# catie-aq/flashT5

Hardware: AMD Instinct MI355X
Metric: FA2+T5-bias fwd+bwd TFLOP/s (bf16, d_head=64) (higher is better)
Workload: dtype bf16; 1 GPU; encoder self-attn fwd+bwd, (B,H,S,d)=(4,12,512,64) per GPU, non-causal, 32-bucket T5 RPE bias (rpe mode), sm_scale 0.125, (B,S,H,D)-strided inputs; global_batch=4, seq_len=512, parallelism=dp1, bias_mode=rpe, launch=hipGraph replay, 16 step(s) per replay

## Files before the change

### flasht5_amd/_lib.py

```python
import ctypes
import os

import torch

_HERE = os.path.dirname(os.path.abspath(__file__))
_VAR = os.environ.get("FAT5_LIB_VARIANT", "")
LIB_PATH = os.path.join(_HERE, "lib", "libfat5" + ("_" + _VAR if _VAR else "") + ".so")

FAT5_F32, FAT5_F16, FAT5_BF16 = 0, 1, 2
FAT5_FORCED_BOS, FAT5_FORCED_EOS = 1, 2
BIAS_NONE, BIAS_DENSE, BIAS_RPE1D = 0, 1, 2
KV_NATIVE, KV_FP8_E4M3 = 0, 1
MAX_RPE_RADIUS = 1024

_DT = {torch.float32: FAT5_F32, torch.float16: FAT5_F16, torch.bfloat16: FAT5_BF16}

c_i64x3 = ctypes.c_int64 * 3


class AttnParams(ctypes.Structure):
    _fields_ = [
        ("B", ctypes.c_int32), ("H", ctypes.c_int32), ("M", ctypes.c_int32), ("N", ctypes.c_int32),
        ("D", ctypes.c_int32), ("dtype", ctypes.c_int32), ("causal", ctypes.c_int32),
        ("bias_mode", ctypes.c_int32), ("sm_scale", ctypes.c_float), ("rpe_radius", ctypes.c_int32),
# ... 82 lines not shown
    _fields_ = [
        ("B", ctypes.c_int32), ("L", ctypes.c_int32), ("H", ctypes.c_int32), ("D", ctypes.c_int32), ("dtype", ctypes.c_int32),
        ("x", ctypes.c_void_p), ("out", ctypes.c_void_p), ("scale", ctypes.c_void_p),
        ("x_stride", c_i64x3), ("out_stride", c_i64x3), ("scale_stride", c_i64x3),
    ]


class SampleParams(ctypes.Structure):
    _fields_ = [
        ("B", ctypes.c_int32), ("V", ctypes.c_int32), ("dtype", ctypes.c_int32), ("top_k", ctypes.c_int32),
        ("logits", ctypes.c_void_p), ("row_stride", ctypes.c_int64), ("temperature", ctypes.c_float), ("top_p", ctypes.c_float),
        ("seed", ctypes.c_uint64), ("offset", ctypes.c_int64), ("offsets", ctypes.c_void_p), ("uniforms", ctypes.c_void_p),
        ("tokens", ctypes.c_void_p), ("aux", ctypes.c_void_p),
    ]


class BeamParams(ctypes.Structure):
    _fields_ = [
        ("B", ctypes.c_int32), ("k", ctypes.c_int32), ("V", ctypes.c_int32), ("dtype", ctypes.c_int32),
        ("logits", ctypes.c_void_p), ("row_stride", ctypes.c_int64), ("running_scores", ctypes.c_void_p),
        ("running_seqs", ctypes.c_void_p), ("cache_row_batch", ctypes.c_void_p), ("finished_seqs", ctypes.c_void_p),
        ("finished_scores", ctypes.c_void_p), ("finished_flags", ctypes.c_void_p), ("finished_lens", ctypes.c_void_p),
        ("heuristic", ctypes.c_void_p), ("status", ctypes.c_void_p), ("tokens", ctypes.c_void_p), ("step", ctypes.c_void_p),
        ("seq_len", ctypes.c_int32), ("capacity", ctypes.c_int32), ("max_length", ctypes.c_int32), ("early_stopping", ctypes.c_int32),
        ("length_penalty", ctypes.c_float), ("workspace", ctypes.c_void_p), ("workspace_bytes", ctypes.c_size_t),
        ("logits_normalized", ctypes.c_int32),
    ]


class LogitsParams(ctypes.Structure):
    _fields_ = [
        ("rows", ctypes.c_int32), ("V", ctypes.c_int32), ("dtype", ctypes.c_int32), ("log_softmax", ctypes.c_int32),
        ("logits", ctypes.c_void_p), ("row_stride", ctypes.c_int64), ("out", ctypes.c_void_p), ("out_stride", ctypes.c_int64),
        ("sequences", ctypes.c_void_p), ("seq_stride", ctypes.c_int64), ("lengths", ctypes.c_void_p), ("seq_len", ctypes.c_int32),
        ("repetition_penalty", ctypes.c_float), ("no_repeat_ngram_size", ctypes.c_int32), ("min_length", ctypes.c_int32),
        ("eos_token_id", ctypes.c_int32), ("n_suppress", ctypes.c_int32), ("suppress_tokens", ctypes.c_void_p),
        ("encoder_repetition_penalty", ctypes.c_double), ("encoder_input_ids", ctypes.c_void_p), ("encoder_stride", ctypes.c_int64),
        ("encoder_lengths", ctypes.c_void_p), ("encoder_rows", ctypes.c_int32), ("encoder_len", ctypes.c_int32),
        ("rows_per_encoder_row", ctypes.c_int32), ("encoder_no_repeat_ngram_size", ctypes.c_int32),
        ("bad_words_ids", ctypes.c_void_p), ("bad_words_offsets", ctypes.c_void_p), ("bad_words_offsets_host", ctypes.c_void_p),
        ("n_bad_words", ctypes.c_int32), ("n_bad_word_ids", ctypes.c_int32), ("min_new_tokens", ctypes.c_int32),
        ("prompt_length", ctypes.c_int32), ("prompt_lengths", ctypes.c_void_p), ("max_new_tokens", ctypes.c_int32),
        ("forced_tokens", ctypes.c_int32), ("forced_bos_token_id", ctypes.c_int32), ("forced_eos_token_id", ctypes.c_int32),
    ]


class SpecParams(ctypes.Structure):
    _fields_ = [
        ("B", ctypes.c_int32), ("M", ctypes.c_int32), ("V", ctypes.c_int32), ("dtype", ctypes.c_int32),
        ("logits", ctypes.c_void_p), ("batch_stride", ctypes.c_int64), ("row_stride", ctypes.c_int64),
        ("draft", ctypes.c_void_p), ("draft_stride", ctypes.c_int64), ("cache_seqlens", ctypes.c_void_p),
        ("draft_seqlens", ctypes.c_void_p), ("labels", ctypes.c_void_p), ("labels_stride", ctypes.c_int64),
        ("ncols", ctypes.c_int32), ("eos_token_id", ctypes.c_int32), ("tok", ctypes.c_void_p), ("seen_eos", ctypes.c_void_p),
        ("limit", ctypes.c_void_p), ("limit_scalar", ctypes.c_int32), ("n_accepted", ctypes.c_void_p), ("n_new", ctypes.c_void_p),
        ("workspace", ctypes.c_void_p), ("workspace_bytes", ctypes.c_size_t),
    ]


class SpecSampleParams(ctypes.Structure):
    _fields_ = [
        ("spec", SpecParams), ("draft_logits", ctypes.c_void_p), ("draft_batch_stride", ctypes.c_int64),
        ("draft_row_stride", ctypes.c_int64), ("temperature", ctypes.c_float), ("top_p", ctypes.c_float),
        ("top_k", ctypes.c_int32), ("reserved", ctypes.c_int32), ("seed", ctypes.c_uint64), ("offset", ctypes.c_int64),
        ("uniforms", ctypes.c_void_p), ("sampled", ctypes.c_void_p), ("aux", ctypes.c_void_p),
    ]


class LookupParams(ctypes.Structure):
    _fields_ = [
        ("B", ctypes.c_int32), ("L_src", ctypes.c_int32), ("ncols", ctypes.c_int32), ("gamma", ctypes.c_int32),
        ("max_ngram", ctypes.c_int32), ("V", ctypes.c_int32),
        ("source", ctypes.c_void_p), ("source_stride", ctypes.c_int64), ("src_seqlens", ctypes.c_void_p),
        ("labels", ctypes.c_void_p), ("labels_stride", ctypes.c_int64), ("cache_seqlens", ctypes.c_void_p),
        ("tok", ctypes.c_void_p), ("seen_eos", ctypes.c_void_p), ("draft", ctypes.c_void_p), ("draft_stride", ctypes.c_int64),
        ("n_proposed", ctypes.c_void_p),
    ]


class PackParams(ctypes.Structure):
    _fields_ = [
        ("B", ctypes.c_int32), ("L", ctypes.c_int32), ("seg_cap", ctypes.c_int32), ("reserved", ctypes.c_int32),
        ("seg", ctypes.c_void_p), ("cu_seqlens", ctypes.c_void_p), ("index", ctypes.c_void_p), ("seg_count", ctypes.c_void_p),
        ("status", ctypes.c_void_p),
    ]


class Ul2Params(ctypes.Structure):
    _fields_ = [
        ("B", ctypes.c_int32), ("L", ctypes.c_int32), ("max_length", ctypes.c_int32), ("max_labels_length", ctypes.c_int32),
        ("num_denoisers", ctypes.c_int32), ("num_sentinels", ctypes.c_int32), ("random_chunk", ctypes.c_int32), ("reserved", ctypes.c_int32),
        ("sentinel_first_id", ctypes.c_int64), ("eos_token_id", ctypes.c_int64), ("pad_token_id", ctypes.c_int64), ("seed", ctypes.c_uint64),
        ("tokens", ctypes.c_void_p), ("tokens_stride", ctypes.c_int64), ("lengths", ctypes.c_void_p), ("step", ctypes.c_void_p),
        ("mu", ctypes.c_void_p), ("r", ctypes.c_void_p), ("max_spans", ctypes.c_void_p), ("tokens_len", ctypes.c_void_p),
        ("prefix_off", ctypes.c_void_p), ("prefix_ids", ctypes.c_void_p), ("cum_prop", ctypes.c_void_p),
        ("noise_mask", ctypes.c_void_p), ("noise_mask_stride", ctypes.c_int64), ("denoiser_in", ctypes.c_void_p),
        ("input_ids", ctypes.c_void_p), ("labels", ctypes.c_void_p), ("attention_mask", ctypes.c_void_p),
        ("decoder_attention_mask", ctypes.c_void_p), ("enc_len", ctypes.c_void_p), ("dec_len", ctypes.c_void_p),
        ("denoiser", ctypes.c_void_p), ("status", ctypes.c_void_p),
    ]


class W8QuantParams(ctypes.Structure):
    _fields_ = [
        ("N", ctypes.c_int64), ("K", ctypes.c_int32), ("dtype", ctypes.c_int32), ("w", ctypes.c_void_p), ("w_stride", ctypes.c_int64),
        ("out", ctypes.c_void_p), ("out_stride", ctypes.c_int64), ("scale", ctypes.c_void_p),
    ]


class W8LinearParams(ctypes.Structure):
    _fields_ = [
        ("R", ctypes.c_int64), ("N", ctypes.c_int64), ("K", ctypes.c_int32), ("dtype", ctypes.c_int32),
        ("x", ctypes.c_void_p), ("x_stride", ctypes.c_int64), ("w8", ctypes.c_void_p), ("w_stride", ctypes.c_int64),
        ("scale", ctypes.c_void_p), ("norm_weight", ctypes.c_void_p), ("eps", ctypes.c_float), ("reserved", ctypes.c_int32),
        ("residual", ctypes.c_void_p), ("residual_stride", ctypes.c_int64), ("y", ctypes.c_void_p), ("y_stride", ctypes.c_int64),
    ]


POOL_EOS, POOL_FIRST, POOL_LAST, POOL_MEAN = 0, 1, 2, 3


class SeqPoolParams(ctypes.Structure):
    _fields_ = [
        ("mode", ctypes.c_int32), ("dtype", ctypes.c_int32), ("nseq", ctypes.c_int32), ("L", ctypes.c_int32),
        ("total", ctypes.c_int64), ("d", ctypes.c_int64), ("eos_token_id", ctypes.c_int64),
        ("hidden", ctypes.c_void_p), ("hidden_row_stride", ctypes.c_int64), ("hidden_batch_stride", ctypes.c_int64),
        ("cu_seqlens", ctypes.c_void_p), ("seqlens", ctypes.c_void_p), ("input_ids", ctypes.c_void_p),
        ("ids_batch_stride", ctypes.c_int64), ("pooled", ctypes.c_void_p), ("pooled_stride", ctypes.c_int64),
        ("position", ctypes.c_void_p), ("found", ctypes.c_void_p), ("dpooled", ctypes.c_void_p), ("dpooled_stride", ctypes.c_int64),
        ("dhidden", ctypes.c_void_p), ("dhidden_row_stride", ctypes.c_int64), ("dhidden_batch_stride", ctypes.c_int64),
    ]


class KdParams(ctypes.Structure):
    _fields_ = [
        ("dtype", ctypes.c_int32), ("reserved", ctypes.c_int32), ("rows", ctypes.c_int64), ("n_cols", ctypes.c_int64),
        ("logits", ctypes.c_void_p), ("row_stride", ctypes.c_int64), ("teacher_logits", ctypes.c_void_p),
        ("teacher_row_stride", ctypes.c_int64), ("labels", ctypes.c_void_p), ("dlosses", ctypes.c_void_p), ("dloss_stride", ctypes.c_int64),
        ("losses", ctypes.c_void_p), ("kd_losses", ctypes.c_void_p), ("z_losses", ctypes.c_void_p), ("ce_losses", ctypes.c_void_p),
        ("lse", ctypes.c_void_p), ("lse_student_t", ctypes.c_void_p), ("lse_teacher_t", ctypes.c_void_p),
        ("dlogits", ctypes.c_void_p), ("dlogits_row_stride", ctypes.c_int64), ("ignore_index", ctypes.c_int64),
        ("alpha", ctypes.c_float), ("temperature", ctypes.c_float), ("label_smoothing", ctypes.c_float), ("logit_scale", ctypes.c_float),
        ("lse_square_scale", ctypes.c_float), ("reserved2", ctypes.c_int32),
    ]


class DropoutDesc(ctypes.Structure):
    _fields_ = [
        ("seed", ctypes.c_uint64), ("step", ctypes.c_void_p), ("elem_offset", ctypes.c_uint64), ("site", ctypes.c_uint32),
        ("p", ctypes.c_float),
    ]


EXPORTS = (
    "fat5_version", "fat5_chip_cus", "fat5_last_error", "fat5_sizeof_attn_params", "fat5_attn_fwd", "fat5_attn_bwd_workspace_bytes", "fat5_attn_bwd", "fat5_attn_bwd_launches",
    "fat5_attn_bwd_stages", "fat5_attn_describe", "fat5_rpe1d_from_table",
    "fat5_rmsnorm_fwd", "fat5_rmsnorm_bwd_workspace_bytes", "fat5_rmsnorm_bwd", "fat5_add_rmsnorm_fwd", "fat5_add_rmsnorm_bwd",
    "fat5_ce_fwd", "fat5_ce_bwd", "fat5_ce_fwd_bwd", "fat5_fold_weights", "fat5_fold_weights_bwd", "fat5_fold_weights_bwd_scratch_bytes", "fat5_rmsnorm_unit_bwd", "fat5_gated_act_fwd", "fat5_gated_act_bwd",
    "fat5_adamw_scale_step", "fat5_adamw_scale_step_clipped", "fat5_adamw_scale_step_dev", "fat5_adamw_grad_sumsq", "fat5_sizeof_adamw_tensor",
    "fat5_rope_apply", "fat5_sizeof_rope_params",
    "fat5_fire_fwd", "fat5_fire_bwd", "fat5_fire_bwd_workspace_bytes", "fat5_sizeof_fire_params",
    "fat5_attn_decode", "fat5_attn_decode_workspace_bytes", "fat5_sizeof_decode_params",
    "fat5_attn_decode_kv8", "fat5_sizeof_decode_kv8_params",
    "fat5_attn_decode_chunk", "fat5_attn_decode_chunk_workspace_bytes", "fat5_sizeof_decode_chunk_params",
    "fat5_sample_logits", "fat5_sizeof_sample_params",
    "fat5_beam_step", "fat5_beam_step_workspace_bytes", "fat5_sizeof_beam_params",
    "fat5_process_logits", "fat5_sizeof_logits_params",
    "fat5_spec_accept", "fat5_spec_accept_workspace_bytes", "fat5_sizeof_spec_params",
    "fat5_spec_accept_sampled", "fat5_spec_accept_sampled_workspace_bytes", "fat5_sizeof_spec_sample_params",
    "fat5_kv_quantize", "fat5_sizeof_kv_quant_params",
    "fat5_lookup_draft", "fat5_sizeof_lookup_params",
    "fat5_pack_plan", "fat5_sizeof_pack_params",
    "fat5_ul2_collate", "fat5_sizeof_ul2_params",
    "fat5_w8_quantize", "fat5_sizeof_w8_quant_params", "fat5_w8_linear", "fat5_sizeof_w8_linear_params",
    "fat5_dropout", "fat5_dropout_add_rmsnorm_fwd", "fat5_dropout_add_rmsnorm_bwd", "fat5_sizeof_dropout_desc",
    "fat5_seq_pool_fwd", "fat5_seq_pool_bwd", "fat5_sizeof_seq_pool_params",
    "fat5_kd_fwd", "fat5_kd_bwd", "fat5_kd_fwd_bwd", "fat5_sizeof_kd_params",
)

_lib = None


def load():
    global _lib
    if _lib is not None:
        return _lib
    if not os.path.exists(LIB_PATH):
        raise ImportError(
            f"{LIB_PATH} not found: build it with `python flasht5_amd/build.py` (hipcc, gfx950). "
            "flasht5_amd has no non-HIP fallback.")
    lib = ctypes.CDLL(LIB_PATH)
    lib.fat5_version.restype = ctypes.c_int
    lib.fat5_last_error.restype = ctypes.c_char_p
    lib.fat5_attn_fwd.restype = ctypes.c_int
    lib.fat5_attn_fwd.argtypes = [ctypes.POINTER(AttnParams), ctypes.c_void_p]
    lib.fat5_attn_bwd.restype = ctypes.c_int
    lib.fat5_attn_bwd.argtypes = [ctypes.POINTER(AttnParams), ctypes.c_void_p]
    lib.fat5_attn_bwd_stages.restype = ctypes.c_int
    lib.fat5_attn_bwd_stages.argtypes = [ctypes.POINTER(AttnParams), ctypes.c_int, ctypes.c_void_p]
    lib.fat5_attn_bwd_launches.restype = ctypes.c_int
    lib.fat5_attn_bwd_launches.argtypes = [ctypes.POINTER(AttnParams)]
    lib.fat5_attn_describe.restype = ctypes.c_int
    lib.fat5_attn_describe.argtypes = [ctypes.POINTER(AttnParams), ctypes.c_char_p, ctypes.c_size_t]
    lib.fat5_attn_bwd_workspace_bytes.restype = ctypes.c_size_t
    lib.fat5_attn_bwd_workspace_bytes.argtypes = [ctypes.POINTER(AttnParams)]
    lib.fat5_rpe1d_from_table.restype = ctypes.c_int
    lib.fat5_rpe1d_from_table.argtypes = [ctypes.c_void_p, ctypes.c_int, ctypes.c_void_p, ctypes.c_void_p, ctypes.c_int32, ctypes.c_int32,
                                          ctypes.c_int32, ctypes.c_void_p]
    i64, f32, vp, i32 = ctypes.c_int64, ctypes.c_float, ctypes.c_void_p, ctypes.c_int
    lib.fat5_rmsnorm_fwd.restype = ctypes.c_int
    lib.fat5_rmsnorm_fwd.argtypes = [vp, vp, vp, vp, i64, i64, i64, i64, f32, i32, i32, vp]
    lib.fat5_rmsnorm_bwd_workspace_bytes.restype = ctypes.c_size_t
    lib.fat5_rmsnorm_bwd_workspace_bytes.argtypes = [i64, i64]
    lib.fat5_rmsnorm_bwd.restype = ctypes.c_int
    lib.fat5_rmsnorm_bwd.argtypes = [vp, vp, vp, vp, vp, vp, i64, i64, i64, i64, i64, i32, i32, vp, ctypes.c_size_t, vp]
    lib.fat5_add_rmsnorm_fwd.restype = ctypes.c_int
    lib.fat5_add_rmsnorm_fwd.argtypes = [vp, vp, vp, vp, vp, vp, i64, i64, i64, i64, i64, i64, f32, i32, i32, vp]
    lib.fat5_add_rmsnorm_bwd.restype = ctypes.c_int
    lib.fat5_add_rmsnorm_bwd.argtypes = [vp, vp, vp, vp, vp, vp, vp, i64, i64, i64, i64, i64, i64, i32, i32, vp, ctypes.c_size_t, vp]
    lib.fat5_ce_fwd.restype = ctypes.c_int
    lib.fat5_ce_fwd.argtypes = [vp, vp, vp, vp, vp, i64, i64, i64, f32, f32, f32, i64, i32, i32, vp]
    lib.fat5_fold_weights_bwd.restype = ctypes.c_int
    lib.fat5_fold_weights_bwd.argtypes = [vp, vp, vp, vp, i64, i64, i64, i64, i64, i64, vp, vp, vp, vp, vp, i64, i32, vp, ctypes.c_size_t, vp]
    lib.fat5_fold_weights_bwd_scratch_bytes.restype = ctypes.c_size_t
    lib.fat5_gated_act_fwd.restype = ctypes.c_int
    lib.fat5_gated_act_fwd.argtypes = [vp, vp, vp, i64, i64, i64, i64, i64, i32, i32, vp]
    lib.fat5_gated_act_bwd.restype = ctypes.c_int
    lib.fat5_gated_act_bwd.argtypes = [vp, vp, vp, vp, vp, i64, i64, i64, i64, i64, i64, i64, i32, i32, vp]
    lib.fat5_fold_weights_bwd_scratch_bytes.argtypes = [i64, i64]
    lib.fat5_rmsnorm_unit_bwd.restype = ctypes.c_int
    lib.fat5_rmsnorm_unit_bwd.argtypes = [vp, vp, vp, vp, vp, i64, i64, i64, i64, i64, i64, vp, i64, i32, vp]
    lib.fat5_fold_weights.restype = ctypes.c_int
    lib.fat5_fold_weights.argtypes = [vp, vp, vp, i64, i64, i64, i64, i64, i64, vp, vp, i64, i32, vp]
    lib.fat5_ce_bwd.restype = ctypes.c_int
    lib.fat5_ce_bwd.argtypes = [vp, i64, vp, vp, vp, vp, i64, i64, i64, i64, f32, f32, f32, i64, i32, vp]
    lib.fat5_ce_fwd_bwd.restype = ctypes.c_int
    lib.fat5_ce_fwd_bwd.argtypes = [vp, vp, vp, i64, vp, vp, vp, vp, i64, i64, i64, i64, f32, f32, f32, i64, i32, vp]
    lib.fat5_adamw_scale_step.restype = ctypes.c_int
    f64 = ctypes.c_double
    lib.fat5_adamw_scale_step.argtypes = [vp, i32, i32, vp, f64, f64, f64, f64, f64, i32, i32, i32, vp]
    lib.fat5_adamw_scale_step_clipped.restype = ctypes.c_int
    lib.fat5_adamw_scale_step_dev.restype = ctypes.c_int
    lib.fat5_adamw_scale_step_dev.argtypes = [vp, i32, i32, vp, vp, f64, f64, f64, i32, i32, i32, vp, vp]
    lib.fat5_adamw_scale_step_clipped.argtypes = [vp, i32, i32, vp, f64, f64, f64, f64, f64, i32, i32, i32, vp, vp]
    lib.fat5_adamw_grad_sumsq.restype = ctypes.c_int
    lib.fat5_adamw_grad_sumsq.argtypes = [vp, i32, i32, vp, i32, vp]
    lib.fat5_sizeof_adamw_tensor.restype = ctypes.c_size_t
    lib.fat5_rope_apply.restype = ctypes.c_int
    lib.fat5_rope_apply.argtypes = [ctypes.POINTER(RopeParams), ctypes.c_void_p]
    lib.fat5_sizeof_rope_params.restype = ctypes.c_size_t
    if lib.fat5_sizeof_rope_params() != ctypes.sizeof(RopeParams):
        raise ImportError(f"fat5_rope_params layout mismatch: library {lib.fat5_sizeof_rope_params()} B, "
                          f"binding {ctypes.sizeof(RopeParams)} B")
    lib.fat5_fire_fwd.restype = ctypes.c_int
    lib.fat5_fire_fwd.argtypes = [ctypes.POINTER(FireParams), ctypes.c_void_p]
    lib.fat5_fire_bwd.restype = ctypes.c_int
    lib.fat5_fire_bwd.argtypes = [ctypes.POINTER(FireParams), ctypes.c_void_p, ctypes.c_size_t, ctypes.c_void_p]
    lib.fat5_fire_bwd_workspace_bytes.restype = ctypes.c_size_t
    lib.fat5_fire_bwd_workspace_bytes.argtypes = [ctypes.POINTER(FireParams)]
    lib.fat5_sizeof_fire_params.restype = ctypes.c_size_t
    if lib.fat5_sizeof_fire_params() != ctypes.sizeof(FireParams):
        raise ImportError(f"fat5_fire_params layout mismatch: library {lib.fat5_sizeof_fire_params()} B, "
                          f"binding {ctypes.sizeof(FireParams)} B")
    lib.fat5_attn_decode.restype = ctypes.c_int
    lib.fat5_attn_decode.argtypes = [ctypes.POINTER(DecodeParams), ctypes.c_void_p]
    lib.fat5_attn_decode_workspace_bytes.restype = ctypes.c_size_t
    lib.fat5_attn_decode_workspace_bytes.argtypes = [ctypes.POINTER(DecodeParams)]
    lib.fat5_sizeof_decode_params.restype = ctypes.c_size_t
    if lib.fat5_sizeof_decode_params() != ctypes.sizeof(DecodeParams):
        raise ImportError(f"fat5_decode_params layout mismatch: library {lib.fat5_sizeof_decode_params()} B, "
                          f"binding {ctypes.sizeof(DecodeParams)} B")
    lib.fat5_attn_decode_kv8.restype = ctypes.c_int
    lib.fat5_attn_decode_kv8.argtypes = [ctypes.POINTER(DecodeKV8Params), ctypes.c_void_p]
    lib.fat5_sizeof_decode_kv8_params.restype = ctypes.c_size_t
    if lib.fat5_sizeof_decode_kv8_params() != ctypes.sizeof(DecodeKV8Params):
        raise ImportError(f"fat5_decode_kv8_params layout mismatch: library {lib.fat5_sizeof_decode_kv8_params()} B, "
                          f"binding {ctypes.sizeof(DecodeKV8Params)} B")
    lib.fat5_attn_decode_chunk.restype = ctypes.c_int
    lib.fat5_attn_decode_chunk.argtypes = [ctypes.POINTER(DecodeChunkParams), ctypes.c_void_p]
    lib.fat5_attn_decode_chunk_workspace_bytes.restype = ctypes.c_size_t
    lib.fat5_attn_decode_chunk_workspace_bytes.argtypes = [ctypes.POINTER(DecodeChunkParams)]
    lib.fat5_sizeof_decode_chunk_params.restype = ctypes.c_size_t
    if lib.fat5_sizeof_decode_chunk_params() != ctypes.sizeof(DecodeChunkParams):
        raise ImportError(f"fat5_decode_chunk_params layout mismatch: library {lib.fat5_sizeof_decode_chunk_params()} B, "
                          f"binding {ctypes.sizeof(DecodeChunkParams)} B")
    lib.fat5_sample_logits.restype = ctypes.c_int
    lib.fat5_sample_logits.argtypes = [ctypes.POINTER(SampleParams), ctypes.c_void_p]
    lib.fat5_sizeof_sample_params.restype = ctypes.c_size_t
    if lib.fat5_sizeof_sample_params() != ctypes.sizeof(SampleParams):
        raise ImportError(f"fat5_sample_params layout mismatch: library {lib.fat5_sizeof_sample_params()} B, "
                          f"binding {ctypes.sizeof(SampleParams)} B")
    lib.fat5_beam_step.restype = ctypes.c_int
    lib.fat5_beam_step.argtypes = [ctypes.POINTER(BeamParams), ctypes.c_void_p]
    lib.fat5_beam_step_workspace_bytes.restype = ctypes.c_size_t
    lib.fat5_beam_step_workspace_bytes.argtypes = [ctypes.POINTER(BeamParams)]
    lib.fat5_sizeof_beam_params.restype = ctypes.c_size_t
    if lib.fat5_sizeof_beam_params() != ctypes.sizeof(BeamParams):
        raise ImportError(f"fat5_beam_params layout mismatch: library {lib.fat5_sizeof_beam_params()} B, "
                          f"binding {ctypes.sizeof(BeamParams)} B")
    lib.fat5_process_logits.restype = ctypes.c_int
    lib.fat5_process_logits.argtypes = [ctypes.POINTER(LogitsParams), ctypes.c_void_p]
    lib.fat5_sizeof_logits_params.restype = ctypes.c_size_t
    if lib.fat5_sizeof_logits_params() != ctypes.sizeof(LogitsParams):
        raise ImportError(f"fat5_logits_params layout mismatch: library {lib.fat5_sizeof_logits_params()} B, "
                          f"binding {ctypes.sizeof(LogitsParams)} B")
    lib.fat5_spec_accept.restype = ctypes.c_int
    lib.fat5_spec_accept.argtypes = [ctypes.POINTER(SpecParams), ctypes.c_void_p]
    lib.fat5_spec_accept_workspace_bytes.restype = ctypes.c_size_t
    lib.fat5_spec_accept_workspace_bytes.argtypes = [ctypes.POINTER(SpecParams)]
    lib.fat5_sizeof_spec_params.restype = ctypes.c_size_t
    if lib.fat5_sizeof_spec_params() != ctypes.sizeof(SpecParams):
        raise ImportError(f"fat5_spec_params layout mismatch: library {lib.fat5_sizeof_spec_params()} B, "
                          f"binding {ctypes.sizeof(SpecParams)} B")
    lib.fat5_spec_accept_sampled.restype = ctypes.c_int
    lib.fat5_spec_accept_sampled.argtypes = [ctypes.POINTER(SpecSampleParams), ctypes.c_void_p]
    lib.fat5_spec_accept_sampled_workspace_bytes.restype = ctypes.c_size_t
    lib.fat5_spec_accept_sampled_workspace_bytes.argtypes = [ctypes.POINTER(SpecSampleParams)]
    lib.fat5_sizeof_spec_sample_params.restype = ctypes.c_size_t
    if lib.fat5_sizeof_spec_sample_params() != ctypes.sizeof(SpecSampleParams):
        raise ImportError(f"fat5_spec_sample_params layout mismatch: library {lib.fat5_sizeof_spec_sample_params()} B, "
                          f"binding {ctypes.sizeof(SpecSampleParams)} B")
    lib.fat5_kv_quantize.restype = ctypes.c_int
    lib.fat5_kv_quantize.argtypes = [ctypes.POINTER(KvQuantParams), ctypes.c_void_p]
    lib.fat5_sizeof_kv_quant_params.restype = ctypes.c_size_t
    if lib.fat5_sizeof_kv_quant_params() != ctypes.sizeof(KvQuantParams):
        raise ImportError(f"fat5_kv_quant_params layout mismatch: library {lib.fat5_sizeof_kv_quant_params()} B, "
                          f"binding {ctypes.sizeof(KvQuantParams)} B")
    lib.fat5_lookup_draft.restype = ctypes.c_int
    lib.fat5_lookup_draft.argtypes = [ctypes.POINTER(LookupParams), ctypes.c_void_p]
    lib.fat5_sizeof_lookup_params.restype = ctypes.c_size_t
    if lib.fat5_sizeof_lookup_params() != ctypes.sizeof(LookupParams):
        raise ImportError(f"fat5_lookup_params layout mismatch: library {lib.fat5_sizeof_lookup_params()} B, "
                          f"binding {ctypes.sizeof(LookupParams)} B")
    lib.fat5_pack_plan.restype = ctypes.c_int
    lib.fat5_pack_plan.argtypes = [ctypes.POINTER(PackParams), ctypes.c_void_p]
    lib.fat5_sizeof_pack_params.restype = ctypes.c_size_t
    if lib.fat5_sizeof_pack_params() != ctypes.sizeof(PackParams):
        raise ImportError(f"fat5_pack_params layout mismatch: library {lib.fat5_sizeof_pack_params()} B, "
                          f"binding {ctypes.sizeof(PackParams)} B")
    lib.fat5_ul2_collate.restype = ctypes.c_int
    lib.fat5_ul2_collate.argtypes = [ctypes.POINTER(Ul2Params), ctypes.c_void_p]
    lib.fat5_sizeof_ul2_params.restype = ctypes.c_size_t
    if lib.fat5_sizeof_ul2_params() != ctypes.sizeof(Ul2Params):
        raise ImportError(f"fat5_ul2_params layout mismatch: library {lib.fat5_sizeof_ul2_params()} B, "
                          f"binding {ctypes.sizeof(Ul2Params)} B")
    for fn, size_fn, struct, name in ((lib.fat5_w8_quantize, lib.fat5_sizeof_w8_quant_params, W8QuantParams, "fat5_w8_quant_params"),
                                      (lib.fat5_w8_linear, lib.fat5_sizeof_w8_linear_params, W8LinearParams, "fat5_w8_linear_params")):
        fn.restype = ctypes.c_int
        fn.argtypes = [ctypes.POINTER(struct), ctypes.c_void_p]
        size_fn.restype = ctypes.c_size_t
        if size_fn() != ctypes.sizeof(struct):
            raise ImportError(f"{name} layout mismatch: library {size_fn()} B, binding {ctypes.sizeof(struct)} B")
    for fn in (lib.fat5_seq_pool_fwd, lib.fat5_seq_pool_bwd):
        fn.restype = ctypes.c_int
        fn.argtypes = [ctypes.POINTER(SeqPoolParams), ctypes.c_void_p]
    lib.fat5_sizeof_seq_pool_params.restype = ctypes.c_size_t
    if lib.fat5_sizeof_seq_pool_params() != ctypes.sizeof(SeqPoolParams):
        raise ImportError(f"fat5_seq_pool_params layout mismatch: library {lib.fat5_sizeof_seq_pool_params()} B, "
                          f"binding {ctypes.sizeof(SeqPoolParams)} B")
    for fn in (lib.fat5_kd_fwd, lib.fat5_kd_bwd, lib.fat5_kd_fwd_bwd):
        fn.restype = ctypes.c_int
        fn.argtypes = [ctypes.POINTER(KdParams), ctypes.c_void_p]
    lib.fat5_sizeof_kd_params.restype = ctypes.c_size_t
    if lib.fat5_sizeof_kd_params() != ctypes.sizeof(KdParams):
        raise ImportError(f"fat5_kd_params layout mismatch: library {lib.fat5_sizeof_kd_params()} B, "
                          f"binding {ctypes.sizeof(KdParams)} B")
    dd = ctypes.POINTER(DropoutDesc)
    lib.fat5_dropout.restype = ctypes.c_int
    lib.fat5_dropout.argtypes = [vp, vp, vp, i64, i64, i64, i64, i64, dd, i32, vp]
    lib.fat5_dropout_add_rmsnorm_fwd.restype = ctypes.c_int
    lib.fat5_dropout_add_rmsnorm_fwd.argtypes = [vp, vp, vp, vp, vp, vp, i64, i64, i64, i64, i64, i64, f32, dd, i32, i32, vp]
    lib.fat5_dropout_add_rmsnorm_bwd.restype = ctypes.c_int
    lib.fat5_dropout_add_rmsnorm_bwd.argtypes = [vp, vp, vp, vp, vp, vp, vp, vp, i64, i64, i64, i64, i64, i64, i64, dd, i32, i32, vp,
                                                 ctypes.c_size_t, vp]
    lib.fat5_sizeof_dropout_desc.restype = ctypes.c_size_t
    if lib.fat5_sizeof_dropout_desc() != ctypes.sizeof(DropoutDesc):
        raise ImportError(f"fat5_dropout_desc layout mismatch: library {lib.fat5_sizeof_dropout_desc()} B, "
                          f"binding {ctypes.sizeof(DropoutDesc)} B")
    lib.fat5_sizeof_attn_params.restype = ctypes.c_size_t
    if lib.fat5_sizeof_attn_params() != ctypes.sizeof(AttnParams):
        raise ImportError(f"fat5_attn_params layout mismatch: library {lib.fat5_sizeof_attn_params()} B, "
                          f"binding {ctypes.sizeof(AttnParams)} B")
    _lib = lib
    return lib


V_FWD64_ON, V_FWD64_OFF, V_KV64_ON, V_KV64_OFF, V_Q64_ON, V_Q64_OFF = 1, 2, 4, 8, 16, 32
V_DBIAS_STAGED, V_DBIAS_INKERNEL, V_NO_FUSE, V_NO_SPLIT = 64, 128, 256, 512
V_FWD64_KSPLIT_ON, V_FWD64_KSPLIT_OFF = 1024, 2048
V_KV64_HALF_ON, V_KV64_HALF_OFF = 4096, 8192
V_KV64_MIX_ON, V_KV64_MIX_OFF = 16384, 32768
V_FWD64_MIX_ON, V_FWD64_MIX_OFF = 524288, 1048576
V_FUSED64_ON, V_FUSED64_OFF = 65536, 131072
V_DBIAS_NOSPLIT = 262144
V_QDB64_ON, V_QDB64_OFF = 2097152, 4194304
V_QDIAG_ON, V_QDIAG_OFF = 8388608, 16777216
V_DTABLE_RUNS_ON, V_DTABLE_RUNS_OFF = 33554432, 67108864
_variant = 0


def set_variant(bits):
    global _variant
    prev, _variant = _variant, int(bits)
    nat = native()
    if nat is not None:
        nat.set_variant(int(bits))
    return prev


class variant:

    def __init__(self, bits):
        self.bits = bits

    def __enter__(self):
        self.prev = set_variant(self.bits)

    def __exit__(self, *exc):
        set_variant(self.prev)
        return False


_native = False


def native():
    global _native
    if _native is False:
        _native = None
        if os.environ.get("FAT5_TORCH_BINDING", "1") != "0" and not _VAR:
            path = os.path.join(_HERE, "lib", "_fat5_torch.so")
            if os.path.exists(path):
                import importlib.util
                load()
                spec = importlib.util.spec_from_file_location("_fat5_torch", path)
                mod = importlib.util.module_from_spec(spec)
                spec.loader.exec_module(mod)
                if mod.sizeof_attn_params() != ctypes.sizeof(AttnParams):
                    raise ImportError("lib/_fat5_torch.so was built against another include/fat5.h: rebuild (python flasht5_amd/build.py)")
                _native = mod
    return _native


def check(rc, what):
    if rc != 0:
        msg = load().fat5_last_error().decode("utf-8", "replace")
        raise RuntimeError(f"{what} failed (fat5 status {rc}): {msg}")


def dtype_code(dt):
    try:
        return _DT[dt]
    except KeyError:
        raise TypeError(f"unsupported dtype {dt}") from None


def stream_ptr(device):
    idx = device.index if device.index is not None else torch.cuda.current_device()
    return ctypes.c_void_p(torch._C._cuda_getCurrentRawStream(idx))


class on_device:
    __slots__ = ("idx", "prev")

    def __init__(self, device):
        self.idx = device.index if device.index is not None else -1
        self.prev = -1

    def __enter__(self):
        if self.idx >= 0:
            cur = torch.cuda.current_device()
            if cur != self.idx:
                self.prev = cur
                torch.cuda.set_device(self.idx)

    def __exit__(self, *exc):
        if self.prev >= 0:
            torch.cuda.set_device(self.prev)
        return False


def strides3(t):
    return c_i64x3(t.stride(0), t.stride(1), t.stride(2))


def kernel_ready(t):
    return (t.stride(-1) == 1 and t.data_ptr() % 16 == 0 and all(s % 8 == 0 for s in t.stride()[:-1]))


def describe(B, H, M, N, D=64, dtype=FAT5_BF16, causal=False, bias_mode=0, radius=0, need_dbias=False, variant=0, sm_scale=None,
             bucket=None, num_buckets=32, packed=False, total_q=0, total_k=None):
    p = AttnParams()
    p.B, p.H, p.M, p.N, p.D = B, H, M, N, D
    p.dtype, p.causal, p.bias_mode, p.rpe_radius, p.variant = dtype, int(causal), bias_mode, radius, variant
    p.sm_scale = float(D) ** -0.5 if sm_scale is None else float(sm_scale)
    if packed:
        p.cu_seqlens_q = p.cu_seqlens_k = 16
        p.total_q, p.total_k = int(total_q), int(total_q if total_k is None else total_k)
    if bias_mode == BIAS_DENSE:
        p.bias = 16
        p.bias_stride[0], p.bias_stride[1], p.bias_stride[2] = 0, M * N, N
        if need_dbias:
            p.dbias, p.dbias_batch, p.dbias_heads = 16, 1, H
    elif bias_mode == BIAS_RPE1D:
        p.rpe1d = 16
        if need_dbias and bucket is not None:
            host = (ctypes.c_int32 * len(bucket))(*[int(x) for x in bucket])
            p.rpe_bucket, p.drpe_table, p.rpe_num_buckets = 16, 16, int(num_buckets)
            p.rpe_bucket_host = ctypes.addressof(host)
        elif need_dbias:
            p.drpe1d = 16
    buf = ctypes.create_string_buffer(256)
    check(load().fat5_attn_describe(ctypes.byref(p), buf, 256), "fat5_attn_describe")
    return dict(kv.split("=") for kv in buf.value.decode().split())
```

### flasht5_amd/csrc/api_attn.hip

```cpp
#include <cstdio>

#include "api_common.h"
#include "attn_dispatch.h"
#include "reduce_kernels.h"

using namespace fat5;

namespace {

inline int effD(const fat5_attn_params* p) { return p->D == 16 ? 32 : p->D; }

int check_common(const fat5_attn_params* p) {
  if (!p) return fail(FAT5_EINVAL, "params is NULL");
  if (p->D != 16 && p->D != 32 && p->D != 64 && p->D != 128) return fail(FAT5_EINVAL, "head_dim %d unsupported (16, 32, 64, 128)", p->D);
  if (p->dtype != FAT5_F16 && p->dtype != FAT5_BF16) return fail(FAT5_EINVAL, "dtype %d unsupported (f16, bf16)", p->dtype);
  if (p->B <= 0 || p->H <= 0 || p->M <= 0 || p->N <= 0) return fail(FAT5_EINVAL, "empty problem B=%d H=%d M=%d N=%d", p->B, p->H, p->M, p->N);
  if (p->bias_mode < 0 || p->bias_mode > 2) return fail(FAT5_EINVAL, "bias_mode %d", p->bias_mode);
  if (p->bias_mode == FAT5_BIAS_DENSE && !p->bias) return fail(FAT5_EINVAL, "dense bias mode without bias pointer");
  if (p->bias_mode == FAT5_BIAS_RPE1D) {
    if (!p->rpe1d) return fail(FAT5_EINVAL, "rpe1d mode without table");
    if (p->rpe_radius < 1 || p->rpe_radius > 2048) return fail(FAT5_EINVAL, "rpe_radius %d out of range [1, 2048]", p->rpe_radius);
  }
  if (p->unit_count < 0 || p->unit_begin < 0 || (p->unit_count > 0 && (long)p->unit_begin + p->unit_count > (long)p->B * p->H))
    return fail(FAT5_EINVAL, "unit range [%d, +%d) outside the %ld units of the problem", p->unit_begin, p->unit_count, (long)p->B * p->H);
  if (p->unit_count > 0 && p->cu_seqlens_q) return fail(FAT5_EINVAL, "unit ranges are not available for packed (cu_seqlens) batches");
  return FAT5_OK;
}
inline DispatchKey key_of(const fat5_attn_params* p) { return dispatch_key(p, chip_cus()); }
inline long n_units(const fat5_attn_params* p) { return p->unit_count > 0 ? p->unit_count : (long)p->B * p->H; }

bool strides_ok(const void* ptr, const int64_t* s) {
  return aligned16(ptr) && (s[0] % 8 == 0) && (s[1] % 8 == 0) && (s[2] % 8 == 0) && s[2] > 0;
}
bool slice_fits(int64_t rows, int64_t row_stride, int D) {
  return ((rows - 1) * row_stride + D) * 2 < (int64_t(1) << 31);
}

void fill_common(const fat5_attn_params* p, AttnArgs& a) {
  memset(&a, 0, sizeof(a));
  a.q = (const uint16_t*)p->q; a.k = (const uint16_t*)p->k; a.v = (const uint16_t*)p->v;
  a.o = (uint16_t*)p->o; a.lse = p->lse;
  for (int i = 0; i < 3; ++i) {
    a.qs[i] = p->q_stride[i]; a.ks[i] = p->k_stride[i]; a.vs[i] = p->v_stride[i]; a.os[i] = p->o_stride[i];
    a.bs[i] = p->bias_stride[i];
  }
  a.B = p->B; a.H = p->H; a.M = p->M; a.N = p->N;
  a.dvalid = p->D;
  a.ref_first = std::fabs(p->sm_scale) * std::sqrt((float)p->D) >= 8.f;
  a.causal = p->causal; a.scale = p->sm_scale; a.R = p->rpe_radius;
  a.bias = (const uint16_t*)p->bias; a.rpe1d = p->rpe1d;
  a.cu_q = p->cu_seqlens_q; a.cu_k = p->cu_seqlens_k;
  a.total_q = p->total_q; a.total_k = p->total_k;
  a.unit_begin = p->unit_begin; a.unit_count = p->unit_count;
  a.batch_inner = p->bias_mode == FAT5_BIAS_DENSE && p->bias_stride[0] == 0 && p->B > 1 && p->unit_count == 0 &&
                  !p->cu_seqlens_q &&
                  (int64_t)(p->bias_stride[1] ? p->H : 1) * p->M * p->N * 2 > (int64_t(256) << 20);
  if (p->bias_mode == FAT5_BIAS_DENSE) {
    a.bias_vec4 = ((reinterpret_cast<uintptr_t>(p->bias) & 7) == 0) && (p->bias_stride[0] % 4 == 0) &&
                  (p->bias_stride[1] % 4 == 0) && (p->bias_stride[2] % 4 == 0);
    a.bias_dma = bias_dma_ok((int)(reinterpret_cast<uintptr_t>(p->bias) & 15), p->bias_stride);
  }
}

typedef hipError_t (*launch_fn)(const AttnArgs&, int, int, int, int, hipStream_t);

bool table_runs(const fat5_attn_params* p, BucketRuns* out) {
  if (p->bias_mode != FAT5_BIAS_RPE1D || !p->drpe_table || p->drpe1d || !p->rpe_bucket_host || (p->variant & FAT5_V_DTABLE_RUNS_OFF)) return false;
  const int nb = p->rpe_num_buckets, n1 = 2 * p->rpe_radius + 1;
  if (nb <= 0 || nb > kMaxRunBuckets || p->rpe_radius < 0) return false;
  BucketRuns r;
  for (int b = 0; b < kMaxRunBuckets; ++b) r.lo[b] = r.len[b] = 0;
  for (int i = 0; i < n1; ++i) {
    const int b = p->rpe_bucket_host[i];
    if (b < 0 || b >= nb) continue;
    if (r.len[b] == 0) r.lo[b] = i;
    else if (r.lo[b] + r.len[b] != i) return false;
    ++r.len[b];
  }
  if (out) *out = r;
  return true;
}

}

extern "C" {

size_t fat5_sizeof_attn_params(void) { return sizeof(fat5_attn_params); }

int fat5_attn_fwd(const fat5_attn_params* p, void* stream_) {
  int rc = check_common(p);
  if (rc) return rc;
  hipStream_t stream = (hipStream_t)stream_;
  if (!p->q || !p->k || !p->v || !p->o || !p->lse) return fail(FAT5_EINVAL, "fwd: null tensor pointer");
  if (!strides_ok(p->q, p->q_stride) || !strides_ok(p->k, p->k_stride) || !strides_ok(p->v, p->v_stride) ||
      !strides_ok(p->o, p->o_stride))
    return fail(FAT5_EINVAL, "fwd: q/k/v/o must be 16-byte aligned with strides that are multiples of 8 elements");
  if (!slice_fits(p->N, p->k_stride[2], p->D) || !slice_fits(p->N, p->v_stride[2], p->D) || !slice_fits(p->M, p->q_stride[2], p->D))
    return fail(FAT5_EINVAL, "fwd: one (batch, head) slice must span less than 2 GiB");
  if ((p->cu_seqlens_q == nullptr) != (p->cu_seqlens_k == nullptr)) return fail(FAT5_EINVAL, "cu_seqlens_q/k must both be set");
  if (p->cu_seqlens_q && p->bias_mode == FAT5_BIAS_DENSE) return fail(FAT5_EINVAL, "varlen: dense bias unsupported (none or rpe1d)");

  AttnArgs a;
  fill_common(p, a);
  const FwdChoice fc = fwd_choice(key_of(p));
  int nw = fc.nw;
  a.n_mblk = fc.n_mblk;
  a.mix_na = fc.mix_na; a.mix_a_lo = fc.mix_a_lo; a.mix_k_hi = fc.mix_k_hi;
  launch_fn fn = fc.fwd64 ? (p->D == 128 ? launch_fwd64_d128 : launch_fwd64_d64) : (effD(p) == 32 ? launch_fwd_d32 : (p->D == 64 ? launch_fwd_d64 : launch_fwd_d128));
  const long grid = fc.mixed ? fc.mix_grid : n_units(p) * a.n_mblk;
  if (grid > 0x7fffffffL) return fail(FAT5_EINVAL, "grid too large");
  hipError_t e = fn(a, p->dtype == FAT5_BF16, p->bias_mode, nw, (int)grid, stream);
  if (e != hipSuccess) return hip_fail(e, "attn_fwd launch");
  return FAT5_OK;
}

size_t fat5_attn_bwd_workspace_bytes(const fat5_attn_params* p) {
  if (check_common(p)) return 0;
  BwdLayout L;
  bwd_layout(key_of(p), L);
  return L.total;
}

int fat5_attn_bwd_launches(const fat5_attn_params* p) {
  if (check_common(p)) return 0;
  BwdLayout L;
  bwd_layout(key_of(p), L);
  return L.form == kSeparate ? 2 : 1;
}

int fat5_attn_describe(const fat5_attn_params* p, char* out, size_t n) {
  int rc = check_common(p);
  if (rc) return rc;
  if (!out || n == 0) return fail(FAT5_EINVAL, "describe: no buffer");
  const DispatchKey key = key_of(p);
  const FwdChoice fc = fwd_choice(key);
  BwdLayout L;
  bwd_layout(key, L);
  char kv[48];
  if (L.kv64 && L.kv64_mix_pf > 0) snprintf(kv, sizeof kv, "64key-mixed:%d", L.kv64_mix_pf);
  else snprintf(kv, sizeof kv, "%s", L.kv64 ? (L.kv64_half ? "64key-half" : "64key") : "32key");
  snprintf(out, n, "fwd=%s dq=%s dkdv=%s fused=%d dbias=%s qdiag=%d", fc.fwd64 ? (fc.mixed ? "64row-mixed" : (fc.ksplit ? "64row-ksplit" : "64row")) : (fc.nw == kFwdSplit ? "32row-split" : "32row"),
           L.qdb64 ? "64row-batch4" : (L.q64 ? "64row" : "32row"), kv, L.form != kSeparate ? 1 : 0,
           L.qdb64 ? (L.qdb_groups > 1 ? "dq-kernel+partials" : "dq-kernel") : (L.dbias_inkernel ? "inkernel" : (L.ds_staged ? "staged" : "direct")),
           L.diag_q ? 1 : 0);
  if (p->bias_mode == FAT5_BIAS_RPE1D && p->drpe_table && !p->drpe1d) {
    const size_t used = strlen(out);
    if (used < n) snprintf(out + used, n - used, " dtable=%s", table_runs(p, nullptr) ? "runs" : "scan");
  }
  return FAT5_OK;
}

int fat5_attn_bwd(const fat5_attn_params* p, void* stream_) { return fat5_attn_bwd_stages(p, FAT5_BWD_ALL, stream_); }

int fat5_attn_bwd_stages(const fat5_attn_params* p, int stages, void* stream_) {
  int rc = check_common(p);
  if (rc) return rc;
  hipStream_t stream = (hipStream_t)stream_;
  if ((p->cu_seqlens_q == nullptr) != (p->cu_seqlens_k == nullptr)) return fail(FAT5_EINVAL, "cu_seqlens_q/k must both be set");
  if (p->cu_seqlens_q && p->bias_mode == FAT5_BIAS_DENSE) return fail(FAT5_EINVAL, "varlen: dense bias unsupported (none or rpe1d)");
  if (!p->q || !p->k || !p->v || !p->o || !p->lse || !p->dout || !p->dq || !p->dk || !p->dv)
    return fail(FAT5_EINVAL, "bwd: null tensor pointer");
  if (!strides_ok(p->q, p->q_stride) || !strides_ok(p->k, p->k_stride) || !strides_ok(p->v, p->v_stride) ||
      !strides_ok(p->o, p->o_stride) || !strides_ok(p->dout, p->do_stride) || !strides_ok(p->dq, p->dq_stride) ||
      !strides_ok(p->dk, p->dk_stride) || !strides_ok(p->dv, p->dv_stride))
    return fail(FAT5_EINVAL, "bwd: tensors must be 16-byte aligned with strides that are multiples of 8 elements");
  if (p->bias_mode == FAT5_BIAS_DENSE && p->dbias) {
    if (!((p->dbias_batch == 1 || p->dbias_batch == p->B) && (p->dbias_heads == 1 || p->dbias_heads == p->H)))
      return fail(FAT5_EINVAL, "bwd: dbias batch/heads (%d,%d) must be 1 or (B,H)", p->dbias_batch, p->dbias_heads);
    if (!aligned16(p->dbias)) return fail(FAT5_EINVAL, "bwd: dbias must be 16-byte aligned");
    if (p->unit_count > 0 && (p->dbias_batch != p->B || p->dbias_heads != p->H))
      return fail(FAT5_EINVAL, "bwd: a unit range writes dense dbias only in its unreduced (B, H, M, N) form");
  }
  if (!slice_fits(p->M, p->q_stride[2], p->D) || !slice_fits(p->N, p->k_stride[2], p->D) || !slice_fits(p->N, p->v_stride[2], p->D) ||
      !slice_fits(p->M, p->o_stride[2], p->D) || !slice_fits(p->M, p->do_stride[2], p->D) || !slice_fits(p->M, p->dq_stride[2], p->D) ||
      !slice_fits(p->N, p->dk_stride[2], p->D) || !slice_fits(p->N, p->dv_stride[2], p->D))
    return fail(FAT5_EINVAL, "bwd: one (batch, head) slice must span less than 2 GiB");
  const DispatchKey key = key_of(p);
  BwdLayout L;
  bwd_layout(key, L);
  if (p->bias_mode == FAT5_BIAS_RPE1D) {
    const size_t lds = L.kv64 ? (L.kv64_half ? smem_bwd_kv64h_d64(p->rpe_radius, p->bias_mode) : smem_bwd_kv64_d64(p->rpe_radius, p->bias_mode))
                     : effD(p) == 32 ? smem_bwd_kv_d32(L.nw_kv, p->rpe_radius, p->bias_mode)
                                  : (p->D == 64 ? smem_bwd_kv_d64(L.nw_kv, p->rpe_radius, p->bias_mode) : smem_bwd_kv_d128(L.nw_kv, p->rpe_radius, p->bias_mode));
    if (lds > 160 * 1024)
      return fail(FAT5_EINVAL, "bwd: rpe_radius %d needs %zu bytes of LDS (160 KiB per workgroup; radius <= 1024 fits every head_dim)", p->rpe_radius, lds);
  }
  if (L.total > 0 && (!p->workspace || p->workspace_bytes < L.total))
    return fail(FAT5_EWORKSPACE, "bwd: workspace of %zu bytes required, got %zu", L.total, p->workspace_bytes);
  if ((reinterpret_cast<uintptr_t>(p->workspace) & 255) != 0) return fail(FAT5_EINVAL, "bwd: workspace must be 256-byte aligned");
  char* ws = (char*)p->workspace;

  AttnArgs a;
  fill_common(p, a);
  a.dout = (const uint16_t*)p->dout; a.dq = (uint16_t*)p->dq; a.dk = (uint16_t*)p->dk; a.dv = (uint16_t*)p->dv;
  for (int i = 0; i < 3; ++i) {
    a.dos[i] = p->do_stride[i]; a.dqs[i] = p->dq_stride[i]; a.dks[i] = p->dk_stride[i]; a.dvs[i] = p->dv_stride[i];
  }
  a.delta = (float*)(ws + L.delta_off);
  a.stat2 = L.kv64 ? (float*)(ws + L.stat2_off) : nullptr;
  if (a.scale == 0.f) a.scale = 1e-30f;
  const int64_t MN = (int64_t)p->M * p->N;
  const long bh = (long)p->B * p->H;
  const bool bf16 = p->dtype == FAT5_BF16;
  if (p->bias_mode == FAT5_BIAS_DENSE && p->dbias && L.qdb64) {
  } else if (p->bias_mode == FAT5_BIAS_DENSE && p->dbias && !L.dbias_inkernel) {
    if (L.ds_staged) {
      a.ds_out = (uint16_t*)(ws + L.ds_off);
    } else {
      a.ds_out = (uint16_t*)p->dbias;
    }
    a.dss[0] = (int64_t)p->H * MN; a.dss[1] = MN; a.dss[2] = p->N;
    a.ds_vec4 = (p->N % 4 == 0) && ((reinterpret_cast<uintptr_t>(a.ds_out) & 7) == 0);
    a.ds_vec8 = (p->N % 8 == 0) && ((reinterpret_cast<uintptr_t>(a.ds_out) & 15) == 0);
    if (p->causal && (stages & FAT5_BWD_DQ) && !L.ds_staged) {
      if (p->unit_count > 0) {
        for (int u = p->unit_begin; u < p->unit_begin + p->unit_count; ++u) {
          const int hh = u / p->B, bb = u - hh * p->B;
          hipError_t e = hipMemsetAsync(a.ds_out + ((size_t)bb * p->H + hh) * MN, 0, (size_t)MN * 2, stream);
          if (e != hipSuccess) return hip_fail(e, "memset ds");
        }
      } else {
        hipError_t e = hipMemsetAsync(a.ds_out, 0, (size_t)bh * MN * 2, stream);
        if (e != hipSuccess) return hip_fail(e, "memset ds");
      }
    }
  }
  if (p->bias_mode == FAT5_BIAS_RPE1D && (p->drpe1d || p->drpe_table)) {
    if (p->drpe_table && (!p->rpe_bucket || p->rpe_num_buckets <= 0))
      return fail(FAT5_EINVAL, "bwd: drpe_table needs rpe_bucket and rpe_num_buckets");
    a.drpe_part = (float*)(ws + L.drpe_off);
  }

  a.n_mblk = L.n_mblk;
  a.n_nblk = L.n_nblk;
  a.n_kv_blocks = 0;
  a.diag_q = L.diag_q ? 1 : 0;
  a.part_stride = L.part_rows;
  const long grid_q = n_units(p) * a.n_mblk, grid_kv = n_units(p) * a.n_nblk;
  const BwdForm form = ((stages & FAT5_BWD_DQ) && (stages & FAT5_BWD_DKDV)) ? L.form : kSeparate;
  if (form == kFused32) {
    a.n_kv_blocks = (int)grid_kv;
    launch_fn fn = effD(p) == 32 ? launch_bwd_fused_d32 : (p->D == 64 ? launch_bwd_fused_d64 : launch_bwd_fused_d128);
    hipError_t e = fn(a, bf16, p->bias_mode, 4, (int)(grid_q + grid_kv), stream);
    if (e != hipSuccess) return hip_fail(e, "attn_bwd_fused launch");
  } else if (form == kFused64) {
    a.n_kv_blocks = (int)grid_kv;
    a.stat2 = nullptr;
    hipError_t e = launch_bwd_fused64_d64(a, bf16, p->bias_mode, 4, (int)(grid_q + grid_kv), stream);
    if (e != hipSuccess) return hip_fail(e, "attn_bwd_fused64 launch");
  } else if (form == kDenseFused64) {
    a.n_kv_blocks = (int)grid_kv;
    a.part_stride = a.n_nblk;
    const long g = (long)p->H * L.qdb_groups * ((p->M + 63) / 64);
    if (g + grid_kv + 16 > 0x7fffffffL) return fail(FAT5_EINVAL, "grid too large");
    hipError_t e = launch_bwd_dfused64_d64(a, bf16, L.qdb_groups > 1 ? (void*)(ws + L.scratch_off) : p->dbias, L.qdb_groups > 1, (int)g, stream);
    if (e != hipSuccess) return hip_fail(e, "attn_bwd_dfused64 launch");
  } else {
    if ((stages & FAT5_BWD_DQ) && L.qdb64) {
      const long g = (long)p->H * L.qdb_groups * ((p->M + 63) / 64);
      if (g > 0x7fffffffL) return fail(FAT5_EINVAL, "grid too large");
      hipError_t e = launch_bwd_qdb64_d64(a, bf16, L.qdb_groups > 1 ? (void*)(ws + L.scratch_off) : p->dbias, L.qdb_groups > 1, (int)g, stream);
      if (e != hipSuccess) return hip_fail(e, "attn_bwd_qdb64 launch");
    } else if (stages & FAT5_BWD_DQ) {
      launch_fn fn = effD(p) == 32 ? launch_bwd_q_d32 : (p->D == 64 ? launch_bwd_q_d64 : launch_bwd_q_d128);
      if (L.q64) fn = launch_bwd_q64_d64;
      hipError_t e = fn(a, bf16, p->bias_mode, L.nw_q, (int)grid_q, stream);
      if (e != hipSuccess) return hip_fail(e, "attn_bwd_q launch");
    }
    if (stages & FAT5_BWD_DKDV) {
      launch_fn fn = effD(p) == 32 ? launch_bwd_kv_d32 : (p->D == 64 ? launch_bwd_kv_d64 : launch_bwd_kv_d128);
      if (L.kv64) fn = launch_bwd_kv64_d64;
      hipError_t e = hipSuccess;
      if (L.kv64 && L.kv64_mix_pf > 0 && p->unit_count == 0) {
        a.mix_full = L.kv64_mix_pf;
        const long gkv = 8L * ((long)L.kv64_mix_pf * ((p->N + 255) / 256) + (bh / 8 - L.kv64_mix_pf) * (long)a.n_nblk);
        e = fn(a, bf16, p->bias_mode, kKv64Mixed, (int)gkv, stream);
      } else if (L.kv64 && L.kv64_mix_pf > 0) {
        const int split = 8 * L.kv64_mix_pf, ub = p->unit_begin, ue = p->unit_begin + p->unit_count;
        AttnArgs af = a;
        if (ub < std::min(ue, split)) {
          af.unit_begin = ub; af.unit_count = std::min(ue, split) - ub;
          af.n_nblk = (p->N + 255) / 256; af.part_rows2 = 1;
          e = fn(af, bf16, p->bias_mode, kKv64Full, (int)((long)af.unit_count * af.n_nblk), stream);
        }
        if (e == hipSuccess && std::max(ub, split) < ue) {
          af = a;
          af.unit_begin = std::max(ub, split); af.unit_count = ue - af.unit_begin;
          e = fn(af, bf16, p->bias_mode, kKv64Half, (int)((long)af.unit_count * af.n_nblk), stream);
        }
      } else {
        e = fn(a, bf16, p->bias_mode, L.nw_kv, (int)grid_kv, stream);
      }
      if (e != hipSuccess) return hip_fail(e, "attn_bwd_kv launch");
    }
  }
  if (L.dbias_inkernel && (stages & FAT5_BWD_REDUCE)) {
    AttnArgs ab = a;
    ab.n_mblk = (p->M + 127) / 128;
    ab.batch_inner = 0;
    ab.lds_stage = (p->D <= 64 && !(p->variant & FAT5_V_DBIAS_NOSPLIT)) ? 1 : 0;
    const long strips = (long)p->H * ab.n_mblk, ntile = (p->N + 63) / 64;
    long nsplit = 1;
    while (strips * nsplit < cu_scaled(512, key.ncus) && nsplit * 2 <= ntile) nsplit *= 2;
    ab.n_nblk = (int)nsplit;
    const long grid = strips * nsplit;
    typedef hipError_t (*dbias_fn)(const AttnArgs&, int, void*, float*, int, hipStream_t);
    dbias_fn fn = effD(p) == 32 ? launch_bwd_dbias_d32 : (p->D == 64 ? launch_bwd_dbias_d64 : launch_bwd_dbias_d128);
    hipError_t e = fn(ab, bf16, p->dbias, p->B > 4 ? (float*)(ws + L.scratch_off) : nullptr, (int)grid, stream);
    if (e != hipSuccess) return hip_fail(e, "attn_bwd_dbias launch");
  }
  if (L.qdb64 && L.qdb_groups > 1 && (stages & FAT5_BWD_REDUCE)) {
    hipError_t e = launch_dbias_partial_reduce((const float*)(ws + L.scratch_off), p->dbias, bf16, L.qdb_groups, p->H, p->M, p->N, p->causal, stream);
    if (e != hipSuccess) return hip_fail(e, "dbias_partial_reduce launch");
  }
  if (L.ds_staged && (stages & FAT5_BWD_REDUCE)) {
    const int64_t chunks = (MN + 7) / 8 * p->dbias_batch * p->dbias_heads;
    const int grid = (int)((chunks + 255) / 256);
    if (bf16)
      hipLaunchKernelGGL(dbias_reduce_kernel<true>, dim3(grid), dim3(256), 0, stream, a.ds_out, (uint16_t*)p->dbias, p->B,
                         p->H, p->dbias_batch, p->dbias_heads, MN, p->causal ? p->N : 0, p->N - p->M);
    else
      hipLaunchKernelGGL(dbias_reduce_kernel<false>, dim3(grid), dim3(256), 0, stream, a.ds_out, (uint16_t*)p->dbias, p->B,
                         p->H, p->dbias_batch, p->dbias_heads, MN, p->causal ? p->N : 0, p->N - p->M);
    if (int rc = launched("dbias_reduce launch")) return rc;
  }
  BucketRuns runs;
  if (a.drpe_part && (stages & FAT5_BWD_REDUCE) && table_runs(p, &runs)) {
    const long parts = (long)p->B * L.part_rows;
    hipLaunchKernelGGL(drpe_runs_reduce_kernel, dim3(p->rpe_num_buckets, p->H), dim3(kRunsNT), 0, stream, a.drpe_part, p->drpe_table, runs, p->B,
                       p->H, L.part_rows, 2 * p->rpe_radius + 1, p->unit_begin, p->unit_count, div_magic(L.part_rows, parts));
    if (int rc = launched("drpe_runs_reduce launch")) return rc;
  } else if (a.drpe_part && (stages & FAT5_BWD_REDUCE)) {
    const int n1 = 2 * p->rpe_radius + 1;
    const size_t smem = (size_t)n1 * 24;
    if (smem > 48 * 1024) {
      hipError_t ea = hipFuncSetAttribute(reinterpret_cast<const void*>(drpe_reduce_kernel), hipFuncAttributeMaxDynamicSharedMemorySize, (int)smem);
      if (ea != hipSuccess) return hip_fail(ea, "drpe_reduce attribute");
    }
    hipLaunchKernelGGL(drpe_reduce_kernel, dim3(p->H), dim3(1024), smem, stream, a.drpe_part, p->drpe1d, p->rpe_bucket,
                       p->drpe_table, p->B, p->H, L.part_rows, n1, p->rpe_num_buckets, p->unit_begin, p->unit_count, div_magic(n1, 4L * n1),
                       div_magic(L.part_rows, (long)p->B * L.part_rows));
    if (int rc = launched("drpe_reduce launch")) return rc;
  }
  return FAT5_OK;
}

int fat5_rpe1d_from_table(const void* table, int table_dtype, const int32_t* rpe_bucket, float* rpe1d, int32_t H, int32_t rpe_radius,
                          int32_t num_buckets, void* stream_) {
  if (!table || !rpe_bucket || !rpe1d) return fail(FAT5_EINVAL, "rpe1d_from_table: null pointer");
  if (table_dtype != FAT5_F32 && table_dtype != FAT5_F16 && table_dtype != FAT5_BF16) return fail(FAT5_EINVAL, "rpe1d_from_table: bad dtype");
  if (H <= 0 || num_buckets <= 0 || rpe_radius < 1 || rpe_radius > 2048) return fail(FAT5_EINVAL, "rpe1d_from_table: bad shape");
  const int n1 = 2 * rpe_radius + 1;
  const int grid = (H * n1 + 255) / 256;
  hipStream_t stream = (hipStream_t)stream_;
  dispatch_dtype(table_dtype, [&](auto dt_) {
    constexpr int DT = decltype(dt_)::value;
    hipLaunchKernelGGL(rpe1d_gather_kernel<DT>, dim3(grid), dim3(256), 0, stream, table, rpe_bucket, rpe1d, H, n1, num_buckets);
  });
  return launched("rpe1d_gather launch");
}

}
```

### flasht5_amd/csrc/attn_bwd64.h

```cpp
#pragma once
#include "attn_common.h"
#include "attn_fwd64.h"
#include "diag_sum.h"

#ifndef FAT5_ABL
#define FAT5_ABL 0
#endif

#ifndef FAT5_DMA_SPREAD
#define FAT5_DMA_SPREAD 0
#endif
#ifndef FAT5_TRACE
#define FAT5_TRACE 0
#endif

namespace fat5 {

#if FAT5_TRACE
#define FAT5_STAMP(slot) do { if (threadIdx.x == 0) reinterpret_cast<long long*>(a.delta)[(int64_t)blockIdx.x * 16 + (slot)] = __builtin_readcyclecounter(); } while (0)
#else
#define FAT5_STAMP(slot) do { } while (0)
#endif

template <int D, bool HALF = false, bool SELF = false, bool DENSE = false>
// ... 760 lines not shown
          tadr0 = tab_addr(0, (mt0 + j) * 32);
          TN0 = lds_rd128(tadr0);
          static_for<4>([&](auto si) { fast_iter.template operator()<decltype(si)::value, true>(j + decltype(si)::value, 0.f); });
          j += 4;
        }
      }
      if constexpr (BIAS == FAT5_BIAS_RPE1D) {
        if (j < nsteps && !(j + 4 <= nsteps && (j & 3) == 0 && classify(j, side) && classify(j + 3, side3) && side3 == side)) {
          generic_iter(j);
          ++j;
        }
      } else {
        if (j < nsteps) {
          generic_iter(j);
          ++j;
        }
      }
    }
    FAT5_STAMP(3);
    product_step((uint32_t)(((nsteps - 1) & 3) * SLOT));
  }

  asm volatile("s_nop 15\n\ts_nop 15" ::: "memory");
  FAT5_STAMP(4);
  auto partial_rows = [&]() {
    if constexpr (DG && !(FAT5_ABL & 16)) {
      if (want_drpe) {
        diag_flush();
        far_neg = wave_sum(far_neg);
        far_pos = wave_sum(far_pos);
        if (l == 0) {
          sD0[(2 * w) * n1] += far_neg;
          sD0[(2 * w) * n1 + 2 * a.R] += far_pos;
        }
        asm volatile("s_waitcnt lgkmcnt(0)" ::: "memory");
        __builtin_amdgcn_s_barrier();
        float* out = a.drpe_part + ((int64_t)bh * a.part_stride + part_row) * n1;
        for (int i2 = tid; i2 < n1; i2 += NT) {
          float acc = 0.f;
#pragma unroll
          for (int ww = 0; ww < 2 * Cfg::NW; ++ww) acc += sD0[ww * n1 + i2];
          out[i2] = acc;
          if (part_zero_next) out[n1 + i2] = 0.f;
        }
      }
    }
  };
  const bool stores_first = stg && !HALF;
  if (!stores_first) partial_rows();

  FAT5_STAMP(5);
  if constexpr (HALF) {
    __syncthreads();
    char* mg = smem + wp * (128 * 64 * 4);
    if (pr == 1) {
#pragma unroll
      for (int kb = 0; kb < 2; ++kb)
#pragma unroll
        for (int db = 0; db < DB; ++db)
#pragma unroll
          for (int g = 0; g < 4; ++g) {
            const int i = ((kb * DB + db) * 4 + g) * 2;
            *reinterpret_cast<f32x4*>(mg + (i * 64 + l) * 16) = f32x4{dk[kb][db][4 * g], dk[kb][db][4 * g + 1], dk[kb][db][4 * g + 2], dk[kb][db][4 * g + 3]};
            *reinterpret_cast<f32x4*>(mg + ((i + 1) * 64 + l) * 16) = f32x4{dv[kb][db][4 * g], dv[kb][db][4 * g + 1], dv[kb][db][4 * g + 2], dv[kb][db][4 * g + 3]};
          }
    }
    __syncthreads();
    if (pr == 1) return;
#pragma unroll
    for (int kb = 0; kb < 2; ++kb)
#pragma unroll
      for (int db = 0; db < DB; ++db)
#pragma unroll
        for (int g = 0; g < 4; ++g) {
          const int i = ((kb * DB + db) * 4 + g) * 2;
          const f32x4 xk = *reinterpret_cast<const f32x4*>(mg + (i * 64 + l) * 16), xv = *reinterpret_cast<const f32x4*>(mg + ((i + 1) * 64 + l) * 16);
#pragma unroll
          for (int e = 0; e < 4; ++e) {
            dk[kb][db][4 * g + e] += xk[e];
            dv[kb][db][4 * g + e] += xv[e];
          }
        }
  }
  const float scale = a.scale;
  const bool stg_out = stg || DENSE;
  if (DENSE && !stg) {
    asm volatile("s_waitcnt lgkmcnt(0)" ::: "memory");
    __builtin_amdgcn_s_barrier();
  }
  if (stg_out) {
    char* img = smem + (stg ? Cfg::RINGB : 0) + wp * 2 * Cfg::STG_T;
    static_assert(!DENSE || Cfg::NW * 2 * Cfg::STG_T <= Cfg::RING, "the output images fit the ring");
#pragma unroll
    for (int kb = 0; kb < 2; ++kb) {
      const int row = 32 * kb + lq;
#pragma unroll
      for (int db = 0; db < DB; ++db)
#pragma unroll
        for (int g = 0; g < 4; ++g) {
          u32x2 wk, wv;
          wk[0] = pack2<BF16>(dk[kb][db][4 * g + 0] * scale, dk[kb][db][4 * g + 1] * scale);
          wk[1] = pack2<BF16>(dk[kb][db][4 * g + 2] * scale, dk[kb][db][4 * g + 3] * scale);
          wv[0] = pack2<BF16>(dv[kb][db][4 * g + 0], dv[kb][db][4 * g + 1]);
          wv[1] = pack2<BF16>(dv[kb][db][4 * g + 2], dv[kb][db][4 * g + 3]);
          *reinterpret_cast<u32x2*>(img + rm_off<D>(row, 4 * db + g) + 8 * hi) = wk;
          *reinterpret_cast<u32x2*>(img + Cfg::STG_T + rm_off<D>(row, 4 * db + g) + 8 * hi) = wv;
        }
    }
#pragma unroll
    for (int i = 0; i < 8; ++i) {
      const int row = 8 * i + (l >> 3), slot = l & 7;
      const u32x4 k4 = *reinterpret_cast<const u32x4*>(img + row * (2 * D) + slot * 16);
      const u32x4 v4 = *reinterpret_cast<const u32x4*>(img + Cfg::STG_T + row * (2 * D) + slot * 16);
      if (kw0 + row < N) {
        *reinterpret_cast<u32x4*>(dkb + (int64_t)(kw0 + row) * a.dks[2] + ((slot ^ swz<D>(row)) << 3)) = k4;
        *reinterpret_cast<u32x4*>(dvb + (int64_t)(kw0 + row) * a.dvs[2] + ((slot ^ swz<D>(row)) << 3)) = v4;
      }
    }
    if (stores_first) partial_rows();
    FAT5_STAMP(6);
    return;
  }
#pragma unroll
  for (int kb = 0; kb < 2; ++kb) {
    const int krow = kw0 + 32 * kb + lq;
    if (krow < N) {
      uint16_t* dkrow = dkb + (int64_t)krow * a.dks[2];
      uint16_t* dvrow = dvb + (int64_t)krow * a.dvs[2];
#pragma unroll
      for (int db = 0; db < DB; ++db)
#pragma unroll
        for (int g = 0; g < 4; ++g) {
          u32x2 wk, wv;
          wk[0] = pack2<BF16>(dk[kb][db][4 * g + 0] * scale, dk[kb][db][4 * g + 1] * scale);
          wk[1] = pack2<BF16>(dk[kb][db][4 * g + 2] * scale, dk[kb][db][4 * g + 3] * scale);
          wv[0] = pack2<BF16>(dv[kb][db][4 * g + 0], dv[kb][db][4 * g + 1]);
          wv[1] = pack2<BF16>(dv[kb][db][4 * g + 2], dv[kb][db][4 * g + 3]);
          *reinterpret_cast<u32x2*>(dkrow + 32 * db + 8 * g + 4 * hi) = wk;
          *reinterpret_cast<u32x2*>(dvrow + 32 * db + 8 * g + 4 * hi) = wv;
        }
    }
  }
  FAT5_STAMP(6);
}

template <int D>
struct BwdQ64Cfg {
  static constexpr int NW = 4, BM = 64 * NW, KT = 32, NT = 64 * NW, NS = 4;
  static constexpr int IMG = rm_bytes<D, KT>();
  static constexpr int SLOT = 2 * IMG;
  static constexpr int RING = NS * SLOT;
  static constexpr int STG_T = 64 * 2 * D;
  static constexpr int STG = NW * 3 * STG_T;
  static size_t smem(int R, int bias_mode, bool stage = false, bool qdg = false) {
    return RING + (stage ? STG : 0) + (bias_mode == FAT5_BIAS_RPE1D ? rpe_table_bytes(R) + 16 : 0) +
           (qdg && bias_mode == FAT5_BIAS_RPE1D ? ((size_t)(2 * R + 1) * 4 * 2 * NW + NT * 4 + 63) / 64 * 64 : 0);
  }
};

template <int D, bool BF16, int BIAS, bool QDG = false>
FAT5_DEV void attn_bwd_q64_body(const AttnArgs& a, const int bid) {
  static_assert(D == 64 && BIAS != FAT5_BIAS_DENSE, "gap schedule written for D = 64, bias none / rpe1d");
  static_assert(!QDG || BIAS == FAT5_BIAS_RPE1D, "the diagonal sums belong to the T5 bias");
  FAT5_STAMP(0);
  using Cfg = BwdQ64Cfg<D>;
  constexpr int BM = Cfg::BM, NT = Cfg::NT, IMG = Cfg::IMG, SLOT = Cfg::SLOT;
  constexpr int KK = D / 16, DB = D / 32;
  extern __shared__ __attribute__((aligned(16))) char smem[];
  const bool stg = a.lds_stage != 0;
  float* sT = reinterpret_cast<float*>(smem + Cfg::RING + (stg ? Cfg::STG : 0)) + kRpePad;

  const int tid = threadIdx.x, w = __builtin_amdgcn_readfirstlane(tid >> 6), l = tid & 63, lq = l & 31, hi = l >> 5;
  int b, h, mblk;
  decode_unit(a, bid, a.n_mblk, b, h, mblk, (FAT5_CAUSAL_ORDER && a.causal) ? 1 : 0);
  const int M = a.M, N = a.N;
  const int m0 = mblk * BM;
  if (m0 >= M) return;
  [[maybe_unused]] RpeTableRegs tabr;
  if constexpr (BIAS == FAT5_BIAS_RPE1D) tabr = rpe_table_load_first(a.rpe1d + (int64_t)h * (2 * a.R + 1), a.R, tid, NT);
  const uint16_t* qb_ = a.q + (int64_t)b * a.qs[0] + (int64_t)h * a.qs[1];
  const uint16_t* kb_ = a.k + (int64_t)b * a.ks[0] + (int64_t)h * a.ks[1];
  const uint16_t* vb_ = a.v + (int64_t)b * a.vs[0] + (int64_t)h * a.vs[1];
  const uint16_t* ob_ = a.o + (int64_t)b * a.os[0] + (int64_t)h * a.os[1];
  const uint16_t* dob_ = a.dout + (int64_t)b * a.dos[0] + (int64_t)h * a.dos[1];
  uint16_t* dqb_ = a.dq + (int64_t)b * a.dqs[0] + (int64_t)h * a.dqs[1];
  const int64_t stat_off = ((int64_t)b * a.H + h) * a.M;
  const int P = N - M;
  [[maybe_unused]] const bool ctab = BIAS == FAT5_BIAS_RPE1D && a.causal && P < a.R && P >= -a.R;
  int n_end = N;
  if (a.causal) n_end = min(N, m0 + BM + P);
  const int nt = n_end > 0 ? (n_end + 31) / 32 : 0;
  const int qw0 = m0 + 64 * w;
  FAT5_STAMP(10);

  u32x4 qf[2][KK], dof[2][KK], off_[2][KK];
  float nL2[2];
  u32x4 d3[2];
  [[maybe_unused]] f32x16 nd16[2];
  const uint32_t lds0 = (uint32_t)(uintptr_t)smem;
  float Lq_[2];
#pragma unroll
  for (int qb = 0; qb < 2; ++qb) Lq_[qb] = a.lse[stat_off + min(qw0 + 32 * qb + lq, M - 1)];
  const uint32_t stg_w = lds0 + (uint32_t)(Cfg::RING + w * 3 * Cfg::STG_T);
  using SDma = DmaStage<D, 64, 64>;
  static_assert(SDma::PER == 8 && SDma::NV == 2, "eight 1-KiB pieces of 8 rows per tensor");
  if (stg) {
    SDma sq, sdo, so;
    sq.init(a.qs[2], l);
    sdo.init(a.dos[2], l);
    so.init(a.os[2], l);
    const __amdgpu_buffer_rsrc_t qrs = make_rows_rsrc(qb_, a.qs[2], M, D), dors = make_rows_rsrc(dob_, a.dos[2], M, D), ors = make_rows_rsrc(ob_, a.os[2], M, D);
    const uint32_t dst = (uint32_t)__builtin_amdgcn_readfirstlane((int)stg_w);
    const uint32_t q0 = (uint32_t)qw0 * (uint32_t)a.qs[2] * 2u, do0 = (uint32_t)qw0 * (uint32_t)a.dos[2] * 2u, o0 = (uint32_t)qw0 * (uint32_t)a.os[2] * 2u;
#pragma unroll
    for (int i = 0; i < SDma::PER; ++i) {
      dma16_asm(qrs, dst + (uint32_t)(i * 1024), sq.voff[i % 2], q0 + sq.piece_step * (i / 2));
      dma16_asm(dors, dst + (uint32_t)(Cfg::STG_T + i * 1024), sdo.voff[i % 2], do0 + sdo.piece_step * (i / 2));
      dma16_asm(ors, dst + (uint32_t)(2 * Cfg::STG_T + i * 1024), so.voff[i % 2], o0 + so.piece_step * (i / 2));
    }
  } else {
#pragma unroll
    for (int qb = 0; qb < 2; ++qb) {
      const int qrow_c = min(qw0 + 32 * qb + lq, M - 1);
#pragma unroll
      for (int kk = 0; kk < KK; ++kk) {
        qf[qb][kk] = *reinterpret_cast<const u32x4*>(qb_ + (int64_t)qrow_c * a.qs[2] + 16 * kk + 8 * hi);
        dof[qb][kk] = *reinterpret_cast<const u32x4*>(dob_ + (int64_t)qrow_c * a.dos[2] + 16 * kk + 8 * hi);
        off_[qb][kk] = *reinterpret_cast<const u32x4*>(ob_ + (int64_t)qrow_c * a.os[2] + 16 * kk + 8 * hi);
        if constexpr (QDG) {
          if (qw0 + 32 * qb + lq >= M) {
            dof[qb][kk] = u32x4{0u, 0u, 0u, 0u};
            off_[qb][kk] = u32x4{0u, 0u, 0u, 0u};
          }
        }
      }
    }
  }
  FAT5_STAMP(11);
  auto derive_rows = [&]() {
#pragma unroll
    for (int qb = 0; qb < 2; ++qb) {
      const int qrow = qw0 + 32 * qb + lq;
      float dsum = 0.f;
#pragma unroll
      for (int kk = 0; kk < KK; ++kk) {
        const u32x4 of = off_[qb][kk];
#pragma unroll
        for (int j = 0; j < 4; ++j) {
          dsum = fmaf(cvt_lo<BF16>(of[j]), cvt_lo<BF16>(dof[qb][kk][j]), dsum);
          dsum = fmaf(cvt_hi<BF16>(of[j]), cvt_hi<BF16>(dof[qb][kk][j]), dsum);
        }
      }
      const float delta = pair_sum(dsum);
      if (!FAT5_TRACE && a.delta && qrow < M && hi == 0) a.delta[stat_off + qrow] = delta;
      const float Lq = Lq_[qb];
      nL2[qb] = (Lq < kDeadRowLse) ? -INFINITY : -Lq * kLog2e;
      if (a.stat2 && hi == 0 && qrow < (M + 31) / 32 * 32) {
        float* st = a.stat2 + (((int64_t)b * a.H + h) * ((M + 31) / 32) + (qrow >> 5)) * 64 + (qrow & 31);
        const bool live = qrow < M && !(Lq < kDeadRowLse);
        st[0] = live ? -Lq / a.scale : (a.scale > 0.f ? -INFINITY : INFINITY);
        st[32] = qrow < M ? -delta : 0.f;
      }
      {
        const float nd = -delta;
        const uint32_t p0 = to16<BF16>(nd);
        const float r1 = nd - cvt16<BF16>((uint16_t)p0);
        const uint32_t p1 = to16<BF16>(r1);
        const float r2 = r1 - cvt16<BF16>((uint16_t)p1);
        const uint32_t p2 = to16<BF16>(r2);
        d3[qb] = hi == 0 ? u32x4{p0 | (p1 << 16), p2, 0u, 0u} : u32x4{0u, 0u, 0u, 0u};
#pragma unroll
        for (int r = 0; r < 16; ++r) nd16[qb][r] = nd;
      }
    }
  };
  if (!stg) derive_rows();
  const uint32_t one2 = pack2<BF16>(1.f, 1.f);
  u32x4 ones4 = {one2, one2, one2, one2};
  const float* sTa[2] = {sT, sT};
  if constexpr (BIAS == FAT5_BIAS_RPE1D) {
#pragma unroll
    for (int qb = 0; qb < 2; ++qb) sTa[qb] = sT + ((a.R - (qw0 + 32 * qb + lq)) & 3) * rpe_n1p(a.R);
  }

  [[maybe_unused]] const int n1 = 2 * a.R + 1;
  [[maybe_unused]] float* const sD0 = sT - kRpePad + 4 * rpe_n1p(a.R);
  [[maybe_unused]] DiagCarry dcar[2];
  diag_carry_zero(dcar[0]);
  diag_carry_zero(dcar[1]);
  [[maybe_unused]] float dprev0 = 0.f;
  [[maybe_unused]] bool diag_run = false;
  [[maybe_unused]] int diag_nb = 0;
  [[maybe_unused]] float dmask[7] = {0.f, 0.f, 0.f, 0.f, 0.f, 0.f, 0.f};
  if constexpr (QDG) {
#pragma unroll
    for (int i = 0; i < 7; ++i) {
      const int ql0 = i < 3 ? i + 1 : i + 5;
      dmask[i] = ((l & 15) + ql0 >= 16) ? 1.f : 0.f;
      asm volatile("" : "+v"(dmask[i]));
    }
  }
  [[maybe_unused]] float far_neg = 0.f, far_pos = 0.f;
  [[maybe_unused]] const bool want_drpe = QDG && (a.drpe_part != nullptr);
  [[maybe_unused]] float* const dsum = sD0 + (2 * w + hi) * n1 + a.R + 4 * hi - lq;
  [[maybe_unused]] float* const dtrash = sD0 + 2 * Cfg::NW * n1 + tid;
  [[maybe_unused]] auto diag_store = [&](const float E, const int base) {
    const int dm = base + lq - 4 * hi;
    far_neg += dm >= a.R ? E : 0.f;
    far_pos += dm <= -a.R ? E : 0.f;
    *((dm > -a.R && dm < a.R) ? dsum - base : dtrash) = E;
  };
  [[maybe_unused]] auto diag_step_end = [&](const DiagStep (&st)[2], const int nb) {
    const float F0 = diag_finish_halves(dcar[0], st[0], l), F1 = diag_finish_halves(dcar[1], st[1], l);
    diag_store(F1 + dprev0, qw0 + 32 - nb);
    dprev0 = F0;
    diag_run = true;
    diag_nb = nb;
  };
  [[maybe_unused]] auto diag_flush = [&]() {
    if (diag_run) {
      diag_store(dcar[1].cur + dprev0, qw0 - diag_nb);
      diag_store(dcar[0].cur, qw0 - diag_nb - 32);
      diag_carry_zero(dcar[0]);
      diag_carry_zero(dcar[1]);
      dprev0 = 0.f;
      diag_run = false;
    }
  };
  [[maybe_unused]] f32x4 facc4 = {0.f, 0.f, 0.f, 0.f};
  if constexpr (QDG) {
    f32x4* z = reinterpret_cast<f32x4*>(sD0);
    for (int i = tid; i < (n1 * 2 * Cfg::NW + 3) / 4; i += NT) z[i] = f32x4{0.f, 0.f, 0.f, 0.f};
  }

  f32x16 dq[2][DB];
#pragma unroll
  for (int qb = 0; qb < 2; ++qb)
#pragma unroll
    for (int i = 0; i < DB; ++i)
#pragma unroll
      for (int r = 0; r < 16; ++r) dq[qb][i][r] = 0.f;

  using Dma = DmaStage<D, Cfg::KT, NT>;
  static_assert(Dma::PER == 1 && Dma::NV == 1, "one 16-byte piece per thread and image");
  Dma kst, vst;
  kst.init(a.ks[2], tid);
  vst.init(a.vs[2], tid);
  const __amdgpu_buffer_rsrc_t krs = make_rows_rsrc(kb_, a.ks[2], N, D);
  const __amdgpu_buffer_rsrc_t vrs = make_rows_rsrc(vb_, a.vs[2], N, D);
  const uint32_t kstride_b = (uint32_t)a.ks[2] * 2u, vstride_b = (uint32_t)a.vs[2] * 2u;
  const uint32_t wave_lds = __builtin_amdgcn_readfirstlane(lds0 + (uint32_t)(tid >> 6) * 1024u);
  auto dma_step = [&](int t, uint32_t slot_off) {
    const uint32_t tt = (uint32_t)__builtin_amdgcn_readfirstlane(t);
    const uint32_t dst = (uint32_t)__builtin_amdgcn_readfirstlane((int)(wave_lds + slot_off));
    dma16_asm(krs, dst, kst.voff[0], tt * 32u * kstride_b);
    dma16_asm(vrs, dst + (uint32_t)IMG, vst.voff[0], tt * 32u * vstride_b);
  };
  auto sync_wait = [&](int t) {
    if (t + 2 < nt) asm volatile("s_waitcnt vmcnt(2)" ::: "memory");
    else wait_dma_all();
    __syncthreads();
  };
  auto sync_step = [&](int t, uint32_t slot3_off) {
    sync_wait(t);
    if (t + 3 < nt) dma_step(t + 3, slot3_off);
  };
#pragma unroll
  for (int i = 0; i < 3; ++i)
    if (i < nt) dma_step(i, (uint32_t)(i * SLOT));
  for (int i = tid; i < SLOT / 16; i += NT) reinterpret_cast<u32x4*>(smem + 3 * SLOT)[i] = u32x4{0u, 0u, 0u, 0u};
  FAT5_STAMP(7);
  if constexpr (BIAS == FAT5_BIAS_RPE1D) rpe_table_fill_rest(sT - kRpePad, a.rpe1d + (int64_t)h * (2 * a.R + 1), a.R, tid, NT, tabr, ctab ? P : 0x7fffffff);
  FAT5_STAMP(8);
  wait_dma_all();
  __syncthreads();
  FAT5_STAMP(9);
  FragAddr<D> fa;
  fa.init(l);
  if (stg) {
#pragma unroll
    for (int qb = 0; qb < 2; ++qb)
#pragma unroll
      for (int kk = 0; kk < KK; ++kk) {
        const uint32_t ad = stg_w + (uint32_t)(fa.rm[kk] + qb * 32 * 2 * D);
        qf[qb][kk] = lds_rd128(ad);
        dof[qb][kk] = lds_rd128(ad + (uint32_t)Cfg::STG_T);
        off_[qb][kk] = lds_rd128(ad + (uint32_t)(2 * Cfg::STG_T));
      }
    derive_rows();
  }
  FAT5_STAMP(1);
#pragma unroll
  for (int qb = 0; qb < 2; ++qb)
#pragma unroll
    for (int kk = 0; kk < KK; ++kk) asm volatile("" : "+a"(qf[qb][kk]), "+a"(dof[qb][kk]));
  asm volatile("" : "+a"(d3[0]), "+a"(d3[1]), "+a"(ones4));

  uint32_t rmA[KK], trA[2][DB];
#pragma unroll
  for (int kk = 0; kk < KK; ++kk) rmA[kk] = lds0 + (uint32_t)fa.rm[kk];
#pragma unroll
  for (int j2 = 0; j2 < 2; ++j2)
#pragma unroll
    for (int db = 0; db < DB; ++db) trA[j2][db] = lds0 + (uint32_t)fa.tr[j2][db];

  const float c2 = a.scale * kLog2e;
  float cst_neg = 0.f, cst_pos = 0.f;
  if constexpr (BIAS == FAT5_BIAS_RPE1D) {
    cst_neg = sT[0];
    cst_pos = sT[2 * a.R];
  }
  const f32x16 zero16 = {0.f, 0.f, 0.f, 0.f, 0.f, 0.f, 0.f, 0.f, 0.f, 0.f, 0.f, 0.f, 0.f, 0.f, 0.f, 0.f};
  const u32x4 zero4 = {0u, 0u, 0u, 0u};
  uint32_t tabA[2] = {0u, 0u};
  int posb[2] = {0, 0};
  u32x4 TN0;
  uint32_t tadr0 = 0u;
  if constexpr (BIAS == FAT5_BIAS_RPE1D) {
#pragma unroll
    for (int qb = 0; qb < 2; ++qb) {
      const int qrow = qw0 + 32 * qb + lq;
      tabA[qb] = (uint32_t)(uintptr_t)sTa[qb];
      posb[qb] = a.R + 4 * hi - qrow - ((a.R - qrow) & 3);
    }
  }
  const int tclamp_hi = rpe_n1p(a.R) - kRpePad - 28;
  auto tab_addr = [&](int qb, int nb) { return tabA[qb] + 4u * (uint32_t)min(max(posb[qb] + nb, -kRpePad), tclamp_hi); };

  f32x16 S[2], DP[2];
  u32x4 DSB[2][2], TRK[2];

  auto rd_tr = [&](uint32_t off, int t2, int db) {
    const uint32_t o = off + (uint32_t)(16 * t2 * 2 * D);
    return lds_rd_tr(trA[0][db] + o, trA[1][db] + o);
  };
  auto score_step = [&](const uint32_t so, f32x16 (&Sx)[2], f32x16 (&DPx)[2]) {
    u32x4 kf[KK], vf[KK];
#pragma unroll
    for (int kk = 0; kk < KK; ++kk) {
      kf[kk] = lds_rd128(rmA[kk] + so);
      vf[kk] = lds_rd128(rmA[kk] + so + (uint32_t)IMG);
    }
#pragma unroll
    for (int kk = 0; kk < KK; ++kk)
#pragma unroll
      for (int qb = 0; qb < 2; ++qb) Sx[qb] = mfma32<BF16>(kf[kk], qf[qb][kk], kk == 0 ? zero16 : Sx[qb]);
#pragma unroll
    for (int qb = 0; qb < 2; ++qb) DPx[qb] = mfma32<BF16>(ones4, d3[qb], zero16);
#pragma unroll
    for (int kk = 0; kk < KK; ++kk)
#pragma unroll
      for (int qb = 0; qb < 2; ++qb) DPx[qb] = mfma32<BF16>(vf[kk], dof[qb][kk], DPx[qb]);
  };
  auto product_step = [&](const uint32_t so) {
#pragma unroll
    for (int t2 = 0; t2 < 2; ++t2)
#pragma unroll
      for (int db = 0; db < DB; ++db) {
        const u32x4 kt = rd_tr(so, t2, db);
#pragma unroll
        for (int qb = 0; qb < 2; ++qb) mfma_acc_agpr<BF16>(dq[qb][db], kt, DSB[qb][t2]);
      }
  };
  auto softmax_generic = [&](const int nb) {
    [[maybe_unused]] DiagStep gst[2];
#pragma unroll
    for (int qb = 0; qb < 2; ++qb) {
      f32x16& s = S[qb];
      const f32x16& dp = DP[qb];
      const int qr0 = qw0 + 32 * qb, qrow = qr0 + lq;
      const float nl = nL2[qb];
      if constexpr (BIAS == FAT5_BIAS_RPE1D) {
        const int R = a.R;
        const float4* tp4 = reinterpret_cast<const float4*>(sTa[qb] + rpe_clamp_asc(R + nb + 4 * hi - qrow - ((R - qrow) & 3), R));
#pragma unroll
        for (int g = 0; g < 4; ++g) {
          const float4 bq = tp4[2 * g];
          s[4 * g + 0] = fmaf(s[4 * g + 0], c2, bq.x + nl);
          s[4 * g + 1] = fmaf(s[4 * g + 1], c2, bq.y + nl);
          s[4 * g + 2] = fmaf(s[4 * g + 2], c2, bq.z + nl);
          s[4 * g + 3] = fmaf(s[4 * g + 3], c2, bq.w + nl);
        }
      } else {
#pragma unroll
        for (int r = 0; r < 16; ++r) s[r] = fmaf(s[r], c2, nl);
      }
#pragma unroll
      for (int r = 0; r < 16; ++r) s[r] = fast_exp2(s[r]) * dp[r];
      const bool nmask = nb + 32 > N;
      const bool cmask = a.causal && (nb + 31 > qr0 + P);
      if (nmask || cmask) {
        const int lim = a.causal ? min(N - 1, qrow + P) : N - 1;
#pragma unroll
        for (int r = 0; r < 16; ++r)
          if (nb + crow(r, hi) > lim) s[r] = 0.f;
      }
#pragma unroll
      for (int t2 = 0; t2 < 2; ++t2) DSB[qb][t2] = pack8<BF16>(s, t2);
      if constexpr (QDG) {
        diag_step_zero(gst[qb]);
        static_for<16>([&](auto ri) { diag_elem<decltype(ri)::value>(gst[qb], s[decltype(ri)::value], l & 15); });
      }
    }
    if constexpr (QDG) diag_step_end(gst, nb);
  };
  auto generic_iter = [&](const int t) {
    const uint32_t o_prev = (uint32_t)(((t + 3) & 3) * SLOT), o_cur = (uint32_t)((t & 3) * SLOT), o_next = (uint32_t)(((t + 1) & 3) * SLOT);
    product_step(o_prev);
    sync_step(t, o_prev);
    f32x16 Sn[2], DPn[2];
    score_step(o_next, Sn, DPn);
    softmax_generic(t * 32);
#pragma unroll
    for (int qb = 0; qb < 2; ++qb) {
      S[qb] = Sn[qb];
      DP[qb] = DPn[qb];
    }
    TRK[0] = rd_tr(o_cur, 0, 0);
    TRK[1] = rd_tr(o_cur, 0, 1);
  };

  constexpr int NG = 24, G_DP = 16;
  auto fast_iter = [&]<int SL, bool BAND>(const int t, const float ad0, const float ad1) {
    constexpr uint32_t o_prev = (uint32_t)(((SL + 3) & 3) * SLOT), o_cur = (uint32_t)(SL * SLOT), o_next = (uint32_t)(((SL + 1) & 3) * SLOT);
    f32x16 Sn[2], DPn[2];
    u32x4 DSn[2][2], kf[KK], vf[KK];
    u32x2 th[2][2], tn[2][2];
    float X[32], Pv[32], Dv[32];
    u32x4 T[2][4];
    uint32_t tadr1 = 0u;
    if constexpr (BAND) T[0][0] = TN0;
    [[maybe_unused]] DiagStep dst[2];
    if constexpr (BAND && QDG) {
      diag_step_zero(dst[0]);
      diag_step_zero(dst[1]);
    }
    [[maybe_unused]] auto stE_ = [&]<int E>() {
      constexpr int r = E & 15, ql0 = diag_ql0(r);
      diag_elem_u<r>(dst[E >> 4], Dv[E]);
      if constexpr (ql0 != 0) diag_elem_bm<r>(dst[E >> 4], Dv[E], dmask[ql0 < 8 ? ql0 - 1 : ql0 - 5]);
    };
    auto stA_ = [&]<int E>() {
      if constexpr (BAND) {
        float tn_ = __uint_as_float(T[E >> 4][(E & 15) >> 2][E & 3]);
        asm_add(tn_, (E >> 4) == 0 ? ad0 : ad1);
        X[E] = asm_fma(S[E >> 4][E & 15], c2, tn_);
      } else {
        X[E] = asm_fma(S[E >> 4][E & 15], c2, (E >> 4) == 0 ? ad0 : ad1);
      }
    };
    auto stB_ = [&]<int E>() { Pv[E] = asm_exp2(X[E]); };
    auto stC_ = [&]<int E>() { Dv[E] = asm_mul(Pv[E], DP[E >> 4][E & 15]); };
    auto stD_ = [&]<int E0>() {
      constexpr int qb = E0 >> 4, r0 = E0 & 15;
      DSn[qb][r0 >> 3][(r0 & 7) >> 1] = asm_cvt_pk<BF16>(Dv[E0], Dv[E0 + 1]);
    };
    static_for<NG>([&](auto gi) {
      constexpr int g = decltype(gi)::value;
      if constexpr (g < 8) {
        constexpr int p = g >> 1, t2 = p >> 1, db = p & 1, qb = g & 1;
        u32x4 fr;
        if constexpr (t2 == 0) fr = TRK[db];
        else fr = u32x4{th[db][0][0], th[db][0][1], th[db][1][0], th[db][1][1]};
        mfma_acc_agpr<BF16>(dq[qb][db], fr, DSB[qb][t2]);
      } else if constexpr (g < 16) {
        constexpr int kk = (g - 8) >> 1, qb = g & 1;
        if constexpr (kk == 0) Sn[qb] = mfma32<BF16>(kf[kk], qf[qb][kk], zero16);
        else Sn[qb] = mfma32<BF16>(kf[kk], qf[qb][kk], Sn[qb]);
      } else if constexpr (g < G_DP) {
        DPn[g - 16] = mfma32<BF16>(ones4, d3[g - 16], zero16);
      } else {
        constexpr int kk = (g - G_DP) >> 1, qb = g & 1;
        if constexpr (kk == 0) DPn[qb] = mfma32<BF16>(vf[kk], dof[qb][kk], nd16[qb]);
        else DPn[qb] = mfma32<BF16>(vf[kk], dof[qb][kk], DPn[qb]);
      }
      __builtin_amdgcn_sched_barrier(0);
      if constexpr (g == 4) {
        if constexpr (FAT5_DMA_SPREAD) sync_wait(t);
        else sync_step(t, o_prev);
      }
      if constexpr (FAT5_DMA_SPREAD && (g == 5 || g == 6)) {
        if (t + 3 < nt) {
          const uint32_t tt = (uint32_t)__builtin_amdgcn_readfirstlane(t + 3);
          const uint32_t dst = (uint32_t)__builtin_amdgcn_readfirstlane((int)(wave_lds + o_prev));
          if constexpr (g == 5) dma16_asm(krs, dst, kst.voff[0], tt * 32u * kstride_b);
          else dma16_asm(vrs, dst + (uint32_t)IMG, vst.voff[0], tt * 32u * vstride_b);
        }
      }
      if constexpr (g < 4) {
        constexpr int db = g >> 1, half = g & 1;
        th[db][half] = lds_rd_tr_half(trA[half][db] + o_prev + (uint32_t)(16 * 2 * D));
      } else if constexpr (g < 8) {
        kf[g - 4] = lds_rd128(rmA[g - 4] + o_next);
      } else if constexpr (g >= 12 && g < 16) {
        vf[g - 12] = lds_rd128(rmA[g - 12] + o_next + (uint32_t)IMG);
      } else if constexpr (g >= NG - 4) {
        constexpr int db = (g - (NG - 4)) >> 1, half = g & 1;
        tn[db][half] = lds_rd_tr_half(trA[half][db] + o_cur);
      }
      if constexpr (BAND) {
        if constexpr (g == 0) T[0][1] = lds_rd128(tadr0 + 32u);
        else if constexpr (g == 2) T[0][2] = lds_rd128(tadr0 + 64u);
        else if constexpr (g == 5) T[0][3] = lds_rd128(tadr0 + 96u);
        else if constexpr (g == 6) tadr1 = tab_addr(1, t * 32);
        else if constexpr (g == 8) T[1][0] = lds_rd128(tadr1);
        else if constexpr (g == 9) T[1][1] = lds_rd128(tadr1 + 32u);
        else if constexpr (g == 11) T[1][2] = lds_rd128(tadr1 + 64u);
        else if constexpr (g == 16) T[1][3] = lds_rd128(tadr1 + 96u);
        else if constexpr (g == 17) tadr0 = tab_addr(0, (t + 1) * 32);
        else if constexpr (g == 18) TN0 = lds_rd128(tadr0);
      }
      {
        constexpr auto lo = [](int gg) { return gg <= 0 ? 0 : (gg >= NG - 3 ? 32 : (32 * gg) / (NG - 3)); };
        static_for<lo(g - 2) - lo(g - 3)>([&](auto ei) {
          constexpr int e = lo(g - 3) + decltype(ei)::value;
          if constexpr ((e & 1) == 1) stD_.template operator()<e - 1>();
          if constexpr (BAND && QDG) stE_.template operator()<e>();
        });
        static_for<lo(g - 1) - lo(g - 2)>([&](auto ei) { stC_.template operator()<lo(g - 2) + decltype(ei)::value>(); });
        static_for<lo(g) - lo(g - 1)>([&](auto ei) { stB_.template operator()<lo(g - 1) + decltype(ei)::value>(); });
        static_for<lo(g + 1) - lo(g)>([&](auto ei) { stA_.template operator()<lo(g) + decltype(ei)::value>(); });
        if constexpr (g == NG - 1) {
          static_for<32 - lo(NG - 1)>([&](auto ei) { stB_.template operator()<lo(NG - 1) + decltype(ei)::value>(); });
          static_for<32 - lo(NG - 2)>([&](auto ei) { stC_.template operator()<lo(NG - 2) + decltype(ei)::value>(); });
          static_for<32 - lo(NG - 3)>([&](auto ei) {
            constexpr int e = lo(NG - 3) + decltype(ei)::value;
            if constexpr ((e & 1) == 1) stD_.template operator()<e - 1>();
          });
        }
      }
      if constexpr (QDG && !BAND && (g == 9 || g == 14 || g == 19)) {
        constexpr int grp = (g - 9) / 5;
        if constexpr (BF16) asm volatile("v_mfma_f32_16x16x32_bf16 %0, %1, %2, %0" : "+v"(facc4) : "a"(ones4), "v"(DSn[grp >> 1][grp & 1]));
        else asm volatile("v_mfma_f32_16x16x32_f16 %0, %1, %2, %0" : "+v"(facc4) : "a"(ones4), "v"(DSn[grp >> 1][grp & 1]));
      }
      __builtin_amdgcn_sched_barrier(0);
    });
    if constexpr (QDG && !BAND) {
      asm volatile("s_nop 1" ::: "memory");
      if constexpr (BF16) asm volatile("v_mfma_f32_16x16x32_bf16 %0, %1, %2, %0" : "+v"(facc4) : "a"(ones4), "v"(DSn[1][1]));
      else asm volatile("v_mfma_f32_16x16x32_f16 %0, %1, %2, %0" : "+v"(facc4) : "a"(ones4), "v"(DSn[1][1]));
    }
#pragma unroll
    for (int qb = 0; qb < 2; ++qb) {
      S[qb] = Sn[qb];
      DP[qb] = DPn[qb];
#pragma unroll
      for (int t2 = 0; t2 < 2; ++t2) DSB[qb][t2] = DSn[qb][t2];
    }
#pragma unroll
    for (int db = 0; db < DB; ++db) TRK[db] = u32x4{tn[db][0][0], tn[db][0][1], tn[db][1][0], tn[db][1][1]};
    if constexpr (BAND && QDG) {
      asm volatile("s_nop 1" : "+v"(dst[1].u1), "+v"(dst[1].b1));
      diag_step_end(dst, t * 32);
    }
  };

  if (nt > 0) {
    score_step(0u, S, DP);
#pragma unroll
    for (int qb = 0; qb < 2; ++qb)
#pragma unroll
      for (int t2 = 0; t2 < 2; ++t2) DSB[qb][t2] = zero4;
    TRK[0] = zero4;
    TRK[1] = zero4;
    FAT5_STAMP(2);
    auto classify = [&](const int t, int& side) {
      const int nb = t * 32;
      bool fast = nb + 32 <= N && (!a.causal || nb + 31 <= qw0 + P);
      side = -1;
      if constexpr (BIAS == FAT5_BIAS_RPE1D) {
        const bool fneg = nb + 31 - qw0 <= -a.R, fpos = nb - (qw0 + 63) >= a.R;
        fast = fast && (fneg || fpos);
        side = fneg ? -1 : 1;
      }
      return fast;
    };
    auto all_visible = [&](const int t) { return t * 32 + 32 <= N && (!a.causal || ctab || t * 32 + 31 <= qw0 + P); };
    int t = 0;
    while (t < nt) {
      int side, side3;
      while (t + 4 <= nt && (t & 3) == 0 && classify(t, side) && classify(t + 3, side3) && side3 == side) {
        const float cst = BIAS == FAT5_BIAS_RPE1D ? (side > 0 ? cst_pos : cst_neg) : 0.f;
        const float ad0 = cst + nL2[0], ad1 = cst + nL2[1];
        if constexpr (QDG) diag_flush();
        static_for<4>([&](auto si) { fast_iter.template operator()<decltype(si)::value, false>(t + decltype(si)::value, ad0, ad1); });
        t += 4;
        if constexpr (QDG) {
          asm volatile("s_nop 15" : "+v"(facc4));
          const float fsum = ((facc4[0] + facc4[1]) + (facc4[2] + facc4[3])) * 0.0625f;
          facc4 = f32x4{0.f, 0.f, 0.f, 0.f};
          if (side > 0) far_pos += fsum; else far_neg += fsum;
        }
      }
      if constexpr (BIAS == FAT5_BIAS_RPE1D) {
        while (t + 4 <= nt && (t & 3) == 0 && all_visible(t + 3) && !(classify(t, side) && classify(t + 3, side3) && side3 == side)) {
          tadr0 = tab_addr(0, t * 32);
          TN0 = lds_rd128(tadr0);
          static_for<4>([&](auto si) { fast_iter.template operator()<decltype(si)::value, true>(t + decltype(si)::value, nL2[0], nL2[1]); });
          t += 4;
        }
        if (t < nt && !(t + 4 <= nt && (t & 3) == 0 && classify(t, side) && classify(t + 3, side3) && side3 == side)) {
          generic_iter(t);
          ++t;
        }
      } else {
        if (t < nt) {
          generic_iter(t);
          ++t;
        }
      }
    }
    FAT5_STAMP(3);
    product_step((uint32_t)(((nt - 1) & 3) * SLOT));
  }
  asm volatile("s_nop 15\n\ts_nop 15" ::: "memory");
  FAT5_STAMP(4);

  const float scale = a.scale;
  if (stg) {
    char* img = smem + Cfg::RING + w * 3 * Cfg::STG_T;
#pragma unroll
    for (int qb = 0; qb < 2; ++qb) {
      const int row = 32 * qb + lq;
#pragma unroll
      for (int db = 0; db < DB; ++db)
#pragma unroll
        for (int g = 0; g < 4; ++g) {
          u32x2 wv;
          wv[0] = pack2<BF16>(dq[qb][db][4 * g + 0] * scale, dq[qb][db][4 * g + 1] * scale);
          wv[1] = pack2<BF16>(dq[qb][db][4 * g + 2] * scale, dq[qb][db][4 * g + 3] * scale);
          *reinterpret_cast<u32x2*>(img + rm_off<D>(row, 4 * db + g) + 8 * hi) = wv;
        }
    }
#pragma unroll
    for (int i = 0; i < 8; ++i) {
      const int row = 8 * i + (l >> 3), slot = l & 7;
      const u32x4 v4 = *reinterpret_cast<const u32x4*>(img + row * (2 * D) + slot * 16);
      if (qw0 + row < M) *reinterpret_cast<u32x4*>(dqb_ + (int64_t)(qw0 + row) * a.dqs[2] + ((slot ^ swz<D>(row)) << 3)) = v4;
    }
  } else {
#pragma unroll
    for (int qb = 0; qb < 2; ++qb) {
      const int qrow = qw0 + 32 * qb + lq;
      if (qrow < M) {
        uint16_t* drow = dqb_ + (int64_t)qrow * a.dqs[2];
#pragma unroll
        for (int db = 0; db < DB; ++db)
#pragma unroll
          for (int g = 0; g < 4; ++g) {
            u32x2 wv;
            wv[0] = pack2<BF16>(dq[qb][db][4 * g + 0] * scale, dq[qb][db][4 * g + 1] * scale);
            wv[1] = pack2<BF16>(dq[qb][db][4 * g + 2] * scale, dq[qb][db][4 * g + 3] * scale);
            *reinterpret_cast<u32x2*>(drow + 32 * db + 8 * g + 4 * hi) = wv;
          }
      }
    }
  }
  FAT5_STAMP(12);
  if constexpr (QDG) {
    if (want_drpe) {
      diag_flush();
      far_neg = wave_sum(far_neg);
      far_pos = wave_sum(far_pos);
      if (l == 0) {
        sD0[(2 * w) * n1] += far_neg;
        sD0[(2 * w) * n1 + 2 * a.R] += far_pos;
      }
      asm volatile("s_waitcnt lgkmcnt(0)" ::: "memory");
      __builtin_amdgcn_s_barrier();
      FAT5_STAMP(13);
      float* out = a.drpe_part + ((int64_t)(b * a.H + h) * a.part_stride + mblk) * n1;
      for (int i2 = tid; i2 < n1; i2 += NT) {
        float acc = 0.f;
#pragma unroll
        for (int ww = 0; ww < 2 * Cfg::NW; ++ww) acc += sD0[ww * n1 + i2];
        out[i2] = acc;
      }
    }
  }
  FAT5_STAMP(6);
}

template <int D, bool BF16, int BIAS, bool QDG = false>
__global__ __launch_bounds__(256) __attribute__((amdgpu_waves_per_eu(1, 1)))
void attn_bwd_q64_kernel(const AttnArgs a) {
  attn_bwd_q64_body<D, BF16, BIAS, QDG>(a, blockIdx.x);
}

template <int D, bool BF16, int BIAS, bool QDG = false>
__global__ __launch_bounds__(256) __attribute__((amdgpu_waves_per_eu(1, 1)))
void attn_bwd_fused64_kernel(const AttnArgs a) {
  if ((int)blockIdx.x < a.n_kv_blocks) {
    int b, h, nblk;
    decode_unit(a, blockIdx.x, a.n_nblk, b, h, nblk, (FAT5_CAUSAL_ORDER && a.causal) ? 2 : 0);
    attn_bwd_kv64_body<D, BF16, BIAS, false, true, false, QDG>(a, b, h, nblk, nblk, false);
  } else {
    attn_bwd_q64_body<D, BF16, BIAS, QDG>(a, blockIdx.x - a.n_kv_blocks);
  }
}

template <int D, bool BF16, int BIAS, bool HALF, bool ONE = false, bool NODIAG = false>
__global__ __launch_bounds__(256) __attribute__((amdgpu_waves_per_eu(1, 1)))
void attn_bwd_kv64_kernel(const AttnArgs a) {
  int b, h, nblk;
  decode_unit(a, blockIdx.x, a.n_nblk, b, h, nblk, (FAT5_CAUSAL_ORDER && a.causal) ? 2 : 0);
  const bool two = !HALF && a.part_rows2;
  attn_bwd_kv64_body<D, BF16, BIAS, HALF, false, ONE, NODIAG>(a, b, h, nblk, two ? 2 * nblk : nblk, two && 2 * nblk + 1 < a.part_stride);
}

template <int D, bool BF16, int BIAS>
__global__ __launch_bounds__(256) __attribute__((amdgpu_waves_per_eu(1, 1)))
void attn_bwd_kv64_mixed_kernel(const AttnArgs a) {
  const int xcd = blockIdx.x & 7, idx = blockIdx.x >> 3;
  const int nth = a.part_stride, ntf = (a.N + 255) / 256;
  const int nfull = a.mix_full * ntf;
  int pair, tile;
  const bool full = idx < nfull;
  if (full) {
    pair = idx / ntf;
    tile = idx - pair * ntf;
  } else {
    const int i2 = idx - nfull;
    pair = a.mix_full + i2 / nth;
    tile = i2 - (i2 / nth) * nth;
  }
  const int ui = pair * 8 + xcd;
  const int h = ui / a.B, b = ui - h * a.B;
  if (full) attn_bwd_kv64_body<D, BF16, BIAS, false>(a, b, h, tile, 2 * tile, 2 * tile + 1 < nth);
  else attn_bwd_kv64_body<D, BF16, BIAS, true>(a, b, h, tile, tile, false);
}

}
```

### flasht5_amd/csrc/attn_bwd64_inst.hip

```cpp
#include "attn_bwd64.h"
#include "attn_launch.h"
#include <algorithm>
#include <cstring>

#ifndef FAT5_INST_D
#error "FAT5_INST_D must be defined"
#endif
#define CAT_(a, b) a##b
#define CAT(a, b) CAT_(a, b)

namespace fat5 {

static inline bool inv_scale_is_16bit(float scale, bool bf16) { return bf16 ? is_one16<true>(1.f / scale) : is_one16<false>(1.f / scale); }
template <int D, bool BF16, int BIAS, bool HALF, bool ONE = false, bool NODIAG = false>
static hipError_t launch_kv64(const AttnArgs& a, int grid, hipStream_t s) {
  AttnArgs as = a;
  fill_div_magic(as, grid);
  using Cfg = Bwd64Cfg<D, HALF, false, BIAS == FAT5_BIAS_DENSE>;
  as.lds_stage = Cfg::smem(a.R, BIAS, true) <= 160 * 1024;
  const size_t smem = Cfg::smem(a.R, BIAS, as.lds_stage != 0);
  auto kern = attn_bwd_kv64_kernel<D, BF16, BIAS, HALF, ONE, NODIAG>;
  if (smem > 48 * 1024) {
    hipError_t e = hipFuncSetAttribute(reinterpret_cast<const void*>(kern), hipFuncAttributeMaxDynamicSharedMemorySize, (int)smem);
    if (e != hipSuccess) return e;
  }
  hipLaunchKernelGGL(kern, dim3(grid), dim3(256), smem, s, as);
  return hipGetLastError();
}

template <int D, bool BF16, int BIAS, bool QDG = false>
static hipError_t launch_q64(const AttnArgs& a, int grid, hipStream_t s) {
  AttnArgs as = a;
  fill_div_magic(as, grid);
  as.lds_stage = BwdQ64Cfg<D>::smem(a.R, BIAS, true, QDG) <= 160 * 1024;
  const size_t smem = BwdQ64Cfg<D>::smem(a.R, BIAS, as.lds_stage != 0, QDG);
  auto kern = attn_bwd_q64_kernel<D, BF16, BIAS, QDG>;
  if (smem > 48 * 1024) {
    hipError_t e = hipFuncSetAttribute(reinterpret_cast<const void*>(kern), hipFuncAttributeMaxDynamicSharedMemorySize, (int)smem);
    if (e != hipSuccess) return e;
  }
  hipLaunchKernelGGL(kern, dim3(grid), dim3(256), smem, s, as);
  return hipGetLastError();
}
hipError_t CAT(launch_bwd_q64_d, FAT5_INST_D)(const AttnArgs& a, int bf16, int bias, int , int grid, hipStream_t s) {
  if (bias == FAT5_BIAS_RPE1D) {
    if (a.diag_q) return bf16 ? launch_q64<FAT5_INST_D, true, FAT5_BIAS_RPE1D, true>(a, grid, s) : launch_q64<FAT5_INST_D, false, FAT5_BIAS_RPE1D, true>(a, grid, s);
    return bf16 ? launch_q64<FAT5_INST_D, true, FAT5_BIAS_RPE1D>(a, grid, s) : launch_q64<FAT5_INST_D, false, FAT5_BIAS_RPE1D>(a, grid, s);
  }
  return bf16 ? launch_q64<FAT5_INST_D, true, FAT5_BIAS_NONE>(a, grid, s) : launch_q64<FAT5_INST_D, false, FAT5_BIAS_NONE>(a, grid, s);
}

template <bool HALF>
static hipError_t launch_kv64_bias(const AttnArgs& a, int bf16, int bias, int grid, hipStream_t s) {
  if constexpr (!HALF) {
    if (bias == FAT5_BIAS_DENSE) {
      const bool one = inv_scale_is_16bit(a.scale, bf16 != 0);
      if (bf16) return one ? launch_kv64<FAT5_INST_D, true, FAT5_BIAS_DENSE, false, true>(a, grid, s) : launch_kv64<FAT5_INST_D, true, FAT5_BIAS_DENSE, false, false>(a, grid, s);
      return one ? launch_kv64<FAT5_INST_D, false, FAT5_BIAS_DENSE, false, true>(a, grid, s) : launch_kv64<FAT5_INST_D, false, FAT5_BIAS_DENSE, false, false>(a, grid, s);
    }
  }
  if (bias == FAT5_BIAS_RPE1D) {
    if constexpr (!HALF) {
      if (a.diag_q)
        return bf16 ? launch_kv64<FAT5_INST_D, true, FAT5_BIAS_RPE1D, false, false, true>(a, grid, s) : launch_kv64<FAT5_INST_D, false, FAT5_BIAS_RPE1D, false, false, true>(a, grid, s);
    }
    return bf16 ? launch_kv64<FAT5_INST_D, true, FAT5_BIAS_RPE1D, HALF>(a, grid, s) : launch_kv64<FAT5_INST_D, false, FAT5_BIAS_RPE1D, HALF>(a, grid, s);
  }
  return bf16 ? launch_kv64<FAT5_INST_D, true, FAT5_BIAS_NONE, HALF>(a, grid, s) : launch_kv64<FAT5_INST_D, false, FAT5_BIAS_NONE, HALF>(a, grid, s);
}
template <int D, bool BF16, int BIAS>
static hipError_t launch_kv64_mixed(const AttnArgs& a, int grid, hipStream_t s) {
  AttnArgs as = a;
  fill_div_magic(as, grid);
  as.lds_stage = std::max(Bwd64Cfg<D, false>::smem(a.R, BIAS, true), Bwd64Cfg<D, true>::smem(a.R, BIAS, true)) <= 160 * 1024;
  const bool st = as.lds_stage != 0;
  const size_t smem = std::max(Bwd64Cfg<D, false>::smem(a.R, BIAS, st), Bwd64Cfg<D, true>::smem(a.R, BIAS, st));
  auto kern = attn_bwd_kv64_mixed_kernel<D, BF16, BIAS>;
  if (smem > 48 * 1024) {
    hipError_t e = hipFuncSetAttribute(reinterpret_cast<const void*>(kern), hipFuncAttributeMaxDynamicSharedMemorySize, (int)smem);
    if (e != hipSuccess) return e;
  }
  hipLaunchKernelGGL(kern, dim3(grid), dim3(256), smem, s, as);
  return hipGetLastError();
}
hipError_t CAT(launch_bwd_kv64_d, FAT5_INST_D)(const AttnArgs& a, int bf16, int bias, int nw, int grid, hipStream_t s) {
  if (nw == kKv64Mixed) {
    if (bias == FAT5_BIAS_RPE1D)
      return bf16 ? launch_kv64_mixed<FAT5_INST_D, true, FAT5_BIAS_RPE1D>(a, grid, s) : launch_kv64_mixed<FAT5_INST_D, false, FAT5_BIAS_RPE1D>(a, grid, s);
    return bf16 ? launch_kv64_mixed<FAT5_INST_D, true, FAT5_BIAS_NONE>(a, grid, s) : launch_kv64_mixed<FAT5_INST_D, false, FAT5_BIAS_NONE>(a, grid, s);
  }
  return nw == kKv64Half ? launch_kv64_bias<true>(a, bf16, bias, grid, s) : launch_kv64_bias<false>(a, bf16, bias, grid, s);
}
template <int D, bool BF16, int BIAS, bool QDG = false>
static hipError_t launch_fused64(const AttnArgs& a, int grid, hipStream_t s) {
  AttnArgs as = a;
  fill_div_magic(as, grid);
  as.lds_stage = std::max(Bwd64Cfg<D, false, true>::smem(a.R, BIAS, true), BwdQ64Cfg<D>::smem(a.R, BIAS, true, QDG)) <= 160 * 1024;
  const bool st = as.lds_stage != 0;
  const size_t smem = std::max(Bwd64Cfg<D, false, true>::smem(a.R, BIAS, st), BwdQ64Cfg<D>::smem(a.R, BIAS, st, QDG));
  auto kern = attn_bwd_fused64_kernel<D, BF16, BIAS, QDG>;
  if (smem > 48 * 1024) {
    hipError_t e = hipFuncSetAttribute(reinterpret_cast<const void*>(kern), hipFuncAttributeMaxDynamicSharedMemorySize, (int)smem);
    if (e != hipSuccess) return e;
  }
  hipLaunchKernelGGL(kern, dim3(grid), dim3(256), smem, s, as);
  return hipGetLastError();
}
hipError_t CAT(launch_bwd_fused64_d, FAT5_INST_D)(const AttnArgs& a, int bf16, int bias, int , int grid, hipStream_t s) {
  if (bias == FAT5_BIAS_RPE1D) {
    if (a.diag_q)
      return bf16 ? launch_fused64<FAT5_INST_D, true, FAT5_BIAS_RPE1D, true>(a, grid, s) : launch_fused64<FAT5_INST_D, false, FAT5_BIAS_RPE1D, true>(a, grid, s);
    return bf16 ? launch_fused64<FAT5_INST_D, true, FAT5_BIAS_RPE1D>(a, grid, s) : launch_fused64<FAT5_INST_D, false, FAT5_BIAS_RPE1D>(a, grid, s);
  }
  return bf16 ? launch_fused64<FAT5_INST_D, true, FAT5_BIAS_NONE>(a, grid, s) : launch_fused64<FAT5_INST_D, false, FAT5_BIAS_NONE>(a, grid, s);
}
size_t CAT(smem_bwd_fused64_d, FAT5_INST_D)(int R, int bias) {
  return std::max(Bwd64Cfg<FAT5_INST_D, false, true>::smem(R, bias), BwdQ64Cfg<FAT5_INST_D>::smem(R, bias, false, true));
}
size_t CAT(smem_bwd_kv64_d, FAT5_INST_D)(int R, int bias) {
  return bias == FAT5_BIAS_DENSE ? Bwd64Cfg<FAT5_INST_D, false, false, true>::smem(R, bias) : Bwd64Cfg<FAT5_INST_D>::smem(R, bias);
}
size_t CAT(smem_bwd_kv64h_d, FAT5_INST_D)(int R, int bias) { return Bwd64Cfg<FAT5_INST_D, true>::smem(R, bias); }

}
```

### flasht5_amd/csrc/attn_common.h

```cpp
#pragma once
#include <hip/hip_runtime.h>
#include <stdint.h>
#include <utility>
#include "../../include/fat5.h"

namespace fat5 {

typedef __attribute__((ext_vector_type(8))) __bf16 bf16x8_t;
typedef __attribute__((ext_vector_type(8))) _Float16 f16x8_t;
typedef __attribute__((ext_vector_type(2))) __bf16 bf16x2_t;
typedef __attribute__((ext_vector_type(2))) _Float16 f16x2_t;
typedef __attribute__((ext_vector_type(16))) float f32x16;
typedef __attribute__((ext_vector_type(2))) float f32x2;
typedef __attribute__((ext_vector_type(4))) uint32_t u32x4;
typedef __attribute__((ext_vector_type(2))) uint32_t u32x2;
typedef __attribute__((ext_vector_type(4))) short s16x4_t;

#define FAT5_DEV __device__ __forceinline__

template <int N, typename F>
FAT5_DEV void static_for(F&& f) {
  [&]<int... I>(std::integer_sequence<int, I...>) { (f(std::integral_constant<int, I>{}), ...); }(std::make_integer_sequence<int, N>{});
}

// ... 151 lines not shown
  return pair_sum(v);
}

template <int D>
FAT5_DEV constexpr int swz(int row) {
  constexpr int C = D / 8;
  if constexpr (C == 16) return ((row & 3) << 2) | ((row >> 2) & 3);
  else if constexpr (C == 8) return (((row >> 1) & 1) << 2) | ((row >> 2) & 3);
  else return (row * C / 16) & (C - 1);
}
template <int D>
FAT5_DEV int rm_off(int row, int chunk) {
  return row * (2 * D) + ((chunk ^ swz<D>(row)) << 4);
}

FAT5_DEV u32x4 gload16(const uint16_t* p, bool valid) {
  u32x4 z = {0, 0, 0, 0};
  return valid ? *reinterpret_cast<const u32x4*>(p) : z;
}

FAT5_DEV int fast_div(int n, int d, uint32_t mg) { return mg ? (int)__umulhi((uint32_t)n, mg) : n / d; }
__host__ inline uint32_t div_magic(long d, long n_max) {
  if (d <= 1 || d >= (1L << 31) || n_max < 0 || (unsigned long long)n_max * (unsigned long long)d >= (1ull << 32)) return 0u;
  return (uint32_t)(((1ull << 32) + (unsigned long long)d - 1) / (unsigned long long)d);
}
FAT5_DEV void decode_block(int bid, int nbh, int ntile, int& bh, int& tile, uint32_t mg_tile = 0, int order = 0) {
  const int nx = 8;
  if ((nbh % nx) == 0) {
    const int xcd = bid % nx;
    const int idx = bid / nx;
    const int per = nbh / nx;
    int pair;
    if (order) {
      const int tq = idx / per;
      pair = idx - tq * per;
      tile = order == 1 ? ntile - 1 - tq : tq;
    } else {
      pair = fast_div(idx, ntile, mg_tile);
      tile = idx - pair * ntile;
    }
    bh = pair * nx + xcd;
  } else if (order) {
    const int tq = bid / nbh;
    bh = bid - tq * nbh;
    tile = order == 1 ? ntile - 1 - tq : tq;
  } else {
    bh = fast_div(bid, ntile, mg_tile);
    tile = bid - bh * ntile;
  }
}


constexpr int kRpePad = 96;
__host__ __device__ constexpr int rpe_n1p(int R) { return (2 * R + 1 + 2 * kRpePad + 3) & ~3; }
__host__ __device__ constexpr size_t rpe_table_bytes(int R) { return (size_t)4 * rpe_n1p(R) * 4; }
FAT5_DEV int rpe_clamp_asc(int pos, int R) { return min(max(pos, -kRpePad), rpe_n1p(R) - kRpePad - 28); }
FAT5_DEV int rpe_clamp_desc(int pos, int R) { return min(max(pos, -kRpePad + 24), rpe_n1p(R) - kRpePad - 4); }
FAT5_DEV void rpe_table_fill(float* sT_raw, const float* rpe1d_h, int R, int tid, int nthreads) {
  const int n1 = 2 * R + 1, n1p = rpe_n1p(R);
  for (int m0 = tid; m0 < n1p; m0 += 2 * nthreads) {
    float vv[8];
#pragma unroll
    for (int c = 0; c < 4; ++c)
#pragma unroll
      for (int u = 0; u < 2; ++u) {
        const int m = m0 + u * nthreads;
        vv[2 * c + u] = rpe1d_h[min(max(m + c - kRpePad, 0), n1 - 1)];
      }
#pragma unroll
    for (int c = 0; c < 4; ++c)
#pragma unroll
      for (int u = 0; u < 2; ++u) {
        const int m = m0 + u * nthreads;
        if (m < n1p) sT_raw[c * n1p + m] = vv[2 * c + u] * kLog2e;
      }
  }
}

struct RpeTableRegs { float vv[8]; };
FAT5_DEV RpeTableRegs rpe_table_load_first(const float* rpe1d_h, int R, int tid, int nthreads) {
  const int n1 = 2 * R + 1;
  RpeTableRegs r;
#pragma unroll
  for (int c = 0; c < 4; ++c)
#pragma unroll
    for (int u = 0; u < 2; ++u) r.vv[2 * c + u] = rpe1d_h[min(max(tid + u * nthreads + c - kRpePad, 0), n1 - 1)];
  return r;
}
FAT5_DEV void rpe_table_fill_rest(float* sT_raw, const float* rpe1d_h, int R, int tid, int nthreads, const RpeTableRegs& first, int dcut = 0x7fffffff) {
  const int n1 = 2 * R + 1, n1p = rpe_n1p(R);
  const int mcut = dcut == 0x7fffffff ? 0x7fffffff : dcut + R + kRpePad;
#pragma unroll
  for (int c = 0; c < 4; ++c)
#pragma unroll
    for (int u = 0; u < 2; ++u) {
      const int m = tid + u * nthreads;
      if (m < n1p) sT_raw[c * n1p + m] = (m + c > mcut) ? -INFINITY : first.vv[2 * c + u] * kLog2e;
    }
  for (int m0 = tid + 2 * nthreads; m0 < n1p; m0 += 2 * nthreads) {
    float vv[8];
#pragma unroll
    for (int c = 0; c < 4; ++c)
#pragma unroll
      for (int u = 0; u < 2; ++u) vv[2 * c + u] = rpe1d_h[min(max(m0 + u * nthreads + c - kRpePad, 0), n1 - 1)];
#pragma unroll
    for (int c = 0; c < 4; ++c)
#pragma unroll
      for (int u = 0; u < 2; ++u) {
        const int m = m0 + u * nthreads;
        if (m < n1p) sT_raw[c * n1p + m] = (m + c > mcut) ? -INFINITY : vv[2 * c + u] * kLog2e;
      }
  }
}

}

namespace fat5 {

struct AttnArgs {
  const uint16_t *q, *k, *v, *dout;
  uint16_t *o, *dq, *dk, *dv;
  float* lse;
  float* delta;
  float* stat2;
  const uint16_t* bias;
  uint16_t* ds_out;
  const float* rpe1d;
  float* drpe_part;
  const int32_t *cu_q, *cu_k;
  int64_t qs[3], ks[3], vs[3], os[3], dos[3], dqs[3], dks[3], dvs[3];
  int64_t bs[3];
  int64_t dss[3];
  int32_t B, H, M, N;
  int32_t total_q, total_k;
  int32_t causal, R;
  int32_t bias_vec4;
  int32_t ds_vec4;
  int32_t ds_vec8;
  int32_t bias_dma;
  int32_t n_mblk, n_nblk;
  int32_t n_kv_blocks;
  int32_t mix_full;
  int32_t part_stride;
  int32_t part_rows2;
  int32_t diag_q;
  int32_t unit_begin, unit_count;
  int32_t batch_inner;
  uint32_t mg_mblk, mg_nblk, mg_H;
  uint32_t mg_mix[4];
  int32_t mix_na, mix_a_lo, mix_k_hi;
  int32_t dvalid;
  int32_t ref_first;
  int32_t lds_stage;
  float scale;
};

#ifndef FAT5_CAUSAL_ORDER
#define FAT5_CAUSAL_ORDER 1
#endif
FAT5_DEV void decode_unit(const AttnArgs& a, int bid, int ntile, int& b, int& h, int& tile, int order = 0) {
  const uint32_t mg_tile = ntile == a.n_mblk ? a.mg_mblk : (ntile == a.n_nblk ? a.mg_nblk : 0u);
  if (a.batch_inner) {
    const int groups = a.H * ntile;
    int gid;
    if ((groups & 7) == 0) {
      const int xcd = bid & 7, idx = bid >> 3;
      b = idx % a.B;
      gid = (idx / a.B) * 8 + xcd;
    } else {
      b = bid % a.B;
      gid = bid / a.B;
    }
    if (order) {
      const int tq = gid / a.H;
      h = gid - tq * a.H;
      tile = order == 1 ? ntile - 1 - tq : tq;
      return;
    }
    h = gid / ntile;
    tile = gid - h * ntile;
    return;
  }
  int ui;
  decode_block(bid, a.unit_count > 0 ? a.unit_count : a.B * a.H, ntile, ui, tile, mg_tile, order);
  if (a.unit_count > 0) {
    const int u = a.unit_begin + ui;
    h = u / a.B;
    b = u - h * a.B;
  } else {
    b = fast_div(ui, a.H, a.mg_H);
    h = ui - b * a.H;
  }
}

FAT5_DEV __amdgpu_buffer_rsrc_t make_rows_rsrc(const uint16_t* base, int64_t row_stride, int nrows, int D) {
  const uint64_t a = reinterpret_cast<uint64_t>(base);
  const uint32_t lo = __builtin_amdgcn_readfirstlane((uint32_t)a);
  const uint32_t hi = __builtin_amdgcn_readfirstlane((uint32_t)(a >> 32));
  const int64_t bytes = nrows > 0 ? ((int64_t)(nrows - 1) * row_stride + D) * 2 : 0;
  return __builtin_amdgcn_make_buffer_rsrc(reinterpret_cast<void*>(((uint64_t)hi << 32) | lo), 0,
                                           __builtin_amdgcn_readfirstlane((int)bytes), 0x00020000);
}

FAT5_DEV u32x4 load_frag16(const uint16_t* row, int kk, int hi, int dvalid) {
  if (16 * kk + 8 * hi >= dvalid) return u32x4{0u, 0u, 0u, 0u};
  return *reinterpret_cast<const u32x4*>(row + 16 * kk + 8 * hi);
}

template <int D, int ROWS, int NT>
struct RowStage {
  static constexpr int C = D / 8;
  static constexpr int ITEMS = ROWS * C;
  static constexpr int PER = (ITEMS + NT - 1) / NT;
  u32x4 r[PER];
  FAT5_DEV void load(const uint16_t* base, int64_t row_stride, int row0, int limit, int tid) {
#pragma unroll
    for (int i = 0; i < PER; ++i) {
      const int id = tid + NT * i;
      const int c = id % C, row = row0 + id / C;
      const bool in = (ITEMS % NT == 0) || (id < ITEMS);
      r[i] = gload16(base + (int64_t)row * row_stride + c * 8, in && row < limit);
    }
  }
  FAT5_DEV void load_clamped(const uint16_t* base, int64_t row_stride, int row0, int limit, int tid) {
#pragma unroll
    for (int i = 0; i < PER; ++i) {
      const int id = tid + NT * i;
      if ((ITEMS % NT != 0) && id >= ITEMS) continue;
      const int row = min(row0 + id / C, limit - 1);
      r[i] = *reinterpret_cast<const u32x4*>(base + (int64_t)row * row_stride + (id % C) * 8);
    }
  }
  FAT5_DEV void load_buf(__amdgpu_buffer_rsrc_t rsrc, uint32_t tile_byte_off, int tid) {
#pragma unroll
    for (int i = 0; i < PER; ++i) {
      if ((ITEMS % NT != 0) && tid + NT * i >= ITEMS) continue;
      r[i] = __builtin_bit_cast(u32x4, __builtin_amdgcn_raw_buffer_load_b128(rsrc, goff[i] * 2u, tile_byte_off, 0));
    }
  }
  uint32_t goff[PER];
  int loff[PER];
  FAT5_DEV void init(int64_t row_stride, int tid) {
#pragma unroll
    for (int i = 0; i < PER; ++i) {
      const int id = tid + NT * i;
      goff[i] = (uint32_t)((id / C) * row_stride + (id % C) * 8);
      loff[i] = rm_off<D>(id / C, id % C);
    }
  }
  FAT5_DEV void load_full(const uint16_t* tile, int tid) {
#pragma unroll
    for (int i = 0; i < PER; ++i) {
      if ((ITEMS % NT != 0) && tid + NT * i >= ITEMS) continue;
      r[i] = *reinterpret_cast<const u32x4*>(tile + goff[i]);
    }
  }
  FAT5_DEV void store_rm(char* lds, int tid) const {
#pragma unroll
    for (int i = 0; i < PER; ++i) {
      if ((ITEMS % NT != 0) && tid + NT * i >= ITEMS) continue;
      *reinterpret_cast<u32x4*>(lds + loff[i]) = r[i];
    }
  }
};

template <int D, int ROWS, int NT, bool SWZ = true>
struct DmaStage {
  static constexpr int C = D / 8;
  static constexpr int ITEMS = ROWS * C;
  static constexpr int PER = ITEMS >= NT ? ITEMS / NT : 1;
  static constexpr int RP = NT / C;
  static constexpr int NV = (RP % 16 == 0 || !SWZ) ? 1 : 16 / RP;
  static_assert((ITEMS % NT == 0 || (NT % ITEMS == 0 && ITEMS % 64 == 0)) && NT % C == 0 && (16 % RP == 0 || RP % 16 == 0) &&
                    PER % NV == 0, "unsupported tile split");
  uint32_t voff[NV];
  uint32_t piece_step;
  FAT5_DEV void init(int64_t row_stride, int tid, int dvalid = D) {
#pragma unroll
    for (int v = 0; v < NV; ++v) {
      const int row = tid / C + RP * v, slot = tid % C;
      const int src = SWZ ? (slot ^ swz<D>(row)) : slot;
      voff[v] = (uint32_t)(row * row_stride * 2 + (src << 4));
      if (8 * src >= dvalid) voff[v] = 0x80000000u;
    }
    piece_step = (uint32_t)(RP * NV * row_stride * 2);
  }
  FAT5_DEV void issue(__amdgpu_buffer_rsrc_t rsrc, uint32_t tile_off, char* img, int tid) const {
#if defined(__HIP_DEVICE_COMPILE__)
    typedef __attribute__((address_space(3))) void* lds_t;
    const int wave = __builtin_amdgcn_readfirstlane(tid >> 6);
#pragma unroll
    for (int i = 0; i < PER; ++i) {
      if (ITEMS < NT && 64 * wave >= ITEMS) continue;
      __builtin_amdgcn_raw_ptr_buffer_load_lds(rsrc, (lds_t)(uintptr_t)(uint32_t)(uintptr_t)(img + (NT * i + 64 * wave) * 16), 16,
                                               voff[i % NV], tile_off + piece_step * (i / NV), 0, 0);
    }
#endif
  }
  FAT5_DEV u32x4 load_piece(__amdgpu_buffer_rsrc_t rsrc, uint32_t tile_off, int i) const {
    return __builtin_bit_cast(u32x4, __builtin_amdgcn_raw_buffer_load_b128(rsrc, voff[i % NV], tile_off + piece_step * (i / NV), 0));
  }
  FAT5_DEV static constexpr int own_off(int tid, int i) { return (tid + NT * i) * 16; }
};

struct BiasTileReader {
  int base[2];
// ... 80 lines not shown
```

### flasht5_amd/csrc/attn_dispatch.h

```cpp
#pragma once
#include <algorithm>
#include <cmath>
#include <cstdint>
#include <cstring>

#include "../../include/fat5.h"
#include "attn_launch.h"

namespace fat5 {

struct DispatchKey {
  int64_t bias_stride[3];
  int32_t B, H, M, N, D, dtype, bias_mode, causal, rpe_radius, variant;
  float sm_scale;
  int32_t dbias_batch, dbias_heads, unit_count, total_q;
  int32_t bias_mis16;
  int32_t packed;
  int32_t has_dbias, has_drpe1d, has_drpe_table;
  int32_t ncus;
};

inline DispatchKey dispatch_key(const fat5_attn_params* p, int ncus) {
  DispatchKey k;
  memset(&k, 0, sizeof(k));
  for (int i = 0; i < 3; ++i) k.bias_stride[i] = p->bias_stride[i];
  k.B = p->B; k.H = p->H; k.M = p->M; k.N = p->N; k.D = p->D;
  k.dtype = p->dtype; k.bias_mode = p->bias_mode; k.causal = p->causal; k.rpe_radius = p->rpe_radius; k.variant = p->variant;
  k.sm_scale = p->sm_scale;
  k.dbias_batch = p->dbias_batch; k.dbias_heads = p->dbias_heads; k.unit_count = p->unit_count; k.total_q = p->total_q;
  k.bias_mis16 = (int32_t)(reinterpret_cast<uintptr_t>(p->bias) & 15);
  k.packed = p->cu_seqlens_q != nullptr;
  k.has_dbias = p->dbias != nullptr; k.has_drpe1d = p->drpe1d != nullptr; k.has_drpe_table = p->drpe_table != nullptr;
  k.ncus = ncus;
  return k;
}

inline size_t align_up(size_t x, size_t a) { return (x + a - 1) / a * a; }

inline int vsel(int variant, int on_bit, int off_bit) { return (variant & on_bit) ? 1 : ((variant & off_bit) ? 0 : -1); }

struct Overrides {
  int fwd64, fwd64_ksplit, fwd64_mix;
  int kv64, kv64_half, kv64_mix, q64, fused64, qdb64, qdiag;
  bool dbias_staged, dbias_inkernel;
  bool no_split, no_fuse;
  explicit Overrides(int v)
      : fwd64(vsel(v, FAT5_V_FWD64_ON, FAT5_V_FWD64_OFF)), fwd64_ksplit(vsel(v, FAT5_V_FWD64_KSPLIT_ON, FAT5_V_FWD64_KSPLIT_OFF)),
        fwd64_mix(vsel(v, FAT5_V_FWD64_MIX_ON, FAT5_V_FWD64_MIX_OFF)), kv64(vsel(v, FAT5_V_KV64_ON, FAT5_V_KV64_OFF)),
        kv64_half(vsel(v, FAT5_V_KV64_HALF_ON, FAT5_V_KV64_HALF_OFF)), kv64_mix(vsel(v, FAT5_V_KV64_MIX_ON, FAT5_V_KV64_MIX_OFF)),
        q64(vsel(v, FAT5_V_Q64_ON, FAT5_V_Q64_OFF)), fused64(vsel(v, FAT5_V_FUSED64_ON, FAT5_V_FUSED64_OFF)),
        qdb64(vsel(v, FAT5_V_QDB64_ON, FAT5_V_QDB64_OFF)), qdiag(vsel(v, FAT5_V_QDIAG_ON, FAT5_V_QDIAG_OFF)),
        dbias_staged(v & FAT5_V_DBIAS_STAGED), dbias_inkernel(v & FAT5_V_DBIAS_INKERNEL), no_split(v & FAT5_V_NO_SPLIT),
        no_fuse(v & FAT5_V_NO_FUSE) {}
};


inline bool bias_dma_ok(int base_mis16, const int64_t* stride) {
  return base_mis16 == 0 && (stride[0] % 8 == 0) && (stride[1] % 8 == 0) && (stride[2] % 8 == 0);
}
inline bool bias_dma_ok(const DispatchKey& k) { return bias_dma_ok(k.bias_mis16, k.bias_stride); }
inline bool causal_in_band(const DispatchKey& k) {
  return k.causal && k.bias_mode == FAT5_BIAS_RPE1D && k.N - k.M < k.rpe_radius && k.N - k.M >= -k.rpe_radius;
}
inline bool batch_shared_dbias(const DispatchKey& k) {
  return k.dbias_batch == 1 && k.dbias_heads == k.H && k.bias_stride[0] == 0 && (k.bias_stride[1] != 0 || k.H == 1) && k.unit_count == 0 &&
         !k.packed;
}
inline bool bias_slice_fits(const DispatchKey& k) { return ((int64_t)(k.M - 1) * k.bias_stride[2] + k.N) * 2 < (int64_t(1) << 31); }

constexpr long kFwd64MinWaves = 384;

inline long cu_scaled(long wgs_at_256, int ncus) { return wgs_at_256 * ncus / 256; }

inline int pick_nw(long ctas_at_nw4, int ncus) {
  return ctas_at_nw4 < cu_scaled(160, ncus) ? 2 : 4;
}

enum BwdForm {
  kSeparate,
  kFused32,
  kFused64,
  kDenseFused64,
};

struct BwdLayout {
  size_t delta_off, stat2_off, ds_off, drpe_off, scratch_off, total;
  bool kv64;
  bool kv64_half;
  int kv64_mix_pf;
  bool q64;
  bool fused64;
  bool ds_staged;
  bool dbias_inkernel;
  bool dfused64;
  bool qdb64;
  int qdb_groups;
  int n_mblk, n_nblk;
  int nw_q, nw_kv;
  bool diag_q;
  int part_rows;
  long grid_q, grid_kv;
  BwdForm form;
};

struct FwdChoice {
  int nw;
  int n_mblk;
  bool fwd64;
  bool ksplit;
  bool mixed;
  int mix_na, mix_a_lo, mix_k_hi;
  long mix_grid;
};

inline FwdChoice fwd_choice(const DispatchKey& k) {
  const Overrides ov(k.variant);
  FwdChoice c;
  c.fwd64 = c.ksplit = c.mixed = false;
  c.mix_na = c.mix_a_lo = c.mix_k_hi = 0;
  c.mix_grid = 0;
  const long bh = (long)k.B * k.H;
  int nw = pick_nw(bh * ((k.M + 127) / 128), k.ncus);
  c.n_mblk = (k.M + 32 * nw - 1) / (32 * nw);
  const long ctas4 = bh * ((k.M + 127) / 128);
  if (!ov.no_split && ctas4 <= k.ncus && bh * ((k.M + 63) / 64) >= cu_scaled(96, k.ncus) && k.N >= 128) {
    nw = kFwdSplit;
    c.n_mblk = (k.M + 63) / 64;
  }
  const long waves64 = bh * ((k.M + 63) / 64);
  const bool ctab = causal_in_band(k);
  const bool dense_ok = k.bias_mode == FAT5_BIAS_DENSE && k.dtype == FAT5_BF16 && !k.packed && ov.fwd64 != 0 && bias_dma_ok(k);
  const bool dense64 = k.D == 64 && dense_ok && smem_fwd64_d64(0, FAT5_BIAS_DENSE) <= 160 * 1024 &&
                       (ov.fwd64 == 1 || (!k.causal && ((waves64 >= cu_scaled(3072, k.ncus) && k.N >= 4096) || (waves64 >= cu_scaled(6144, k.ncus) && k.N >= 2048))));
  const bool dense128 = k.D == 128 && dense_ok && smem_fwd64_d128(0, FAT5_BIAS_DENSE) <= 160 * 1024 &&
                        (ov.fwd64 == 1 || (waves64 >= cu_scaled(384, k.ncus) && k.N >= 512 && !(k.causal && waves64 < cu_scaled(768, k.ncus) && k.N < 2048)));
  if (dense64 || dense128) {
    c.fwd64 = true;
    c.nw = kFwd64Rows256;
    c.n_mblk = (k.M + 255) / 256;
    return c;
  }
  if (k.D == 128 && k.bias_mode != FAT5_BIAS_DENSE && !k.packed && ov.fwd64 != 0 &&
      smem_fwd64_d128(k.rpe_radius, k.bias_mode) <= 160 * 1024 &&
      (ov.fwd64 == 1 || (waves64 >= cu_scaled(768, k.ncus) && (k.N >= 1024 || (k.N >= 512 && waves64 <= 4L * k.ncus))))) {
    c.fwd64 = true;
    c.n_mblk = (k.M + 255) / 256;
    c.nw = bh * c.n_mblk <= k.ncus ? kFwd64Spread : kFwd64Rows256;
    return c;
  }
  if (k.D == 64 && k.bias_mode != FAT5_BIAS_DENSE && !k.packed && ov.fwd64 != 0 &&
      (ov.fwd64 == 1 || (waves64 >= cu_scaled(k.dtype == FAT5_BF16 ? kFwd64MinWaves : 1536, k.ncus) &&
                        !(k.N <= 512 && k.causal && !ctab) &&
                        !(k.causal && k.N > 512 && k.N < 2048 && waves64 < cu_scaled(512, k.ncus)) &&
                        smem_fwd64_d64(k.rpe_radius, k.bias_mode) <= 80 * 1024))) {
    c.fwd64 = true;
    const bool ksplit = ov.fwd64_ksplit == 1 || (ov.fwd64_ksplit != 0 && waves64 < cu_scaled(k.causal ? 2560 : 2048, k.ncus));
    c.ksplit = ksplit;
    nw = ksplit ? kFwd64KSplit : kFwd64Rows256;
    c.n_mblk = ksplit ? (k.M + 127) / 128 : (k.M + 255) / 256;
    if (ov.fwd64_mix != 0 && bh % 8 == 0 && k.M >= 384 && !k.causal && ov.fwd64_ksplit == -1 &&
        (ov.fwd64_mix == 1 || (waves64 * 10 >= 6L * k.ncus * 9 && waves64 * 10 <= 6L * k.ncus * 11 && k.N >= 1024))) {
      const long npx = bh / 8;
      long na_x = (waves64 + 24) / 48;
      na_x = std::max(na_x, npx);
      const long a_max = (k.M - 128) / 256;
      na_x = std::min(na_x, npx * a_max);
      if (a_max >= 1) {
        c.mixed = true;
        c.mix_a_lo = (int)(na_x / npx);
        c.mix_k_hi = (int)(na_x % npx);
        c.mix_na = (int)(8 * na_x);
        const long b_hi = (std::max<long>(k.M - 256L * (c.mix_a_lo + 1), 0) + 127) / 128, b_lo = (std::max<long>(k.M - 256L * c.mix_a_lo, 0) + 127) / 128;
        c.mix_grid = k.unit_count > 0 ? (long)k.unit_count * (c.mix_a_lo + 1 + b_lo)
                                       : 8 * (na_x + c.mix_k_hi * b_hi + (npx - c.mix_k_hi) * b_lo);
        nw = kFwd64Mixed;
      }
    }
  }
  c.nw = nw;
  return c;
}

inline void set_kv64_full(BwdLayout& L, const DispatchKey& k) {
  L.kv64 = true;
  L.kv64_half = false;
  L.kv64_mix_pf = -1;
  L.nw_kv = kKv64Full;
  L.n_nblk = (k.N + 255) / 256;
}

inline bool bwd_fusable(const BwdLayout& L, const Overrides& ov, const DispatchKey& k) {
  if (k.D > 64) return false;
  const long fuse_max = 4L * k.ncus;
  return !ov.no_fuse && !L.kv64 && !L.q64 && !L.qdb64 && L.nw_q == 4 && L.nw_kv == 4 && L.grid_q + L.grid_kv <= fuse_max;
}

inline int bwd_layout_compute(const DispatchKey& k, BwdLayout& L) {
  const Overrides ov(k.variant);
  const long bh = (long)k.B * k.H;
  L.nw_q = pick_nw(bh * ((k.M + 127) / 128), k.ncus);
  L.nw_kv = pick_nw(bh * ((k.N + 127) / 128), k.ncus);
  L.n_nblk = (k.N + 32 * L.nw_kv - 1) / (32 * L.nw_kv);
  const long wg256 = bh * ((k.N + 255) / 256);
  const long ncu = k.ncus;
  const double r_full = (double)((wg256 + ncu - 1) / ncu), r_half = 0.5 * 1.04 * (double)((2 * wg256 + ncu - 1) / ncu);
  const bool dense = k.bias_mode == FAT5_BIAS_DENSE;
  const bool scale_exact = k.sm_scale != 0.f && std::isfinite(1.f / k.sm_scale) && std::isfinite(k.sm_scale) && (k.dtype == FAT5_BF16 || std::fabs(1.f / k.sm_scale) <= 60000.f);
  const bool dense_kv_ok = dense && scale_exact && bias_dma_ok(k) && bias_slice_fits(k);
  const int qdb_ngrp = (k.B + 3) / 4;
  const bool qdb_legal = dense && k.has_dbias && k.D == 64 && scale_exact && batch_shared_dbias(k) && k.N % 8 == 0 && bias_dma_ok(k) &&
                         (int64_t)k.M * k.N * (qdb_ngrp > 1 ? 4 : 2) < (int64_t(1) << 31) &&
                         (qdb_ngrp == 1 || (int64_t)qdb_ngrp * k.H * k.M * k.N * 4 <= (int64_t(4) << 30)) && bias_slice_fits(k);
  const long qdb_nq = (long)k.H * qdb_ngrp * ((k.M + 63) / 64);
  const bool dense_causal_odd_round = dense && k.causal && k.N <= 512 && wg256 + qdb_nq > k.ncus && wg256 + qdb_nq < 2L * k.ncus;
  const int64_t dense_scores = (int64_t)k.B * k.H * k.M * k.N;
  const bool qdb_rule = k.B >= 2 && (dense_scores >= (int64_t(1) << 24) || (dense_scores >= (int64_t(1) << 23) && k.B >= 16)) && !dense_causal_odd_round;
  const bool qdb_pick = qdb_legal && dense_kv_ok && ov.qdb64 != 0 && qdb_rule && !(ov.dbias_staged || ov.dbias_inkernel);
  L.kv64_half = !dense && (ov.kv64_half == 1 || (ov.kv64_half != 0 && k.bias_mode == FAT5_BIAS_NONE && r_half < 0.9 * r_full && !k.causal));
  L.kv64_mix_pf = -1;
  double mix_gain = 1.0;
  if (bh % 8 == 0 && ov.kv64_mix != 0 && ov.kv64_half == -1 && !dense) {
    const int per = (int)(bh / 8), ntf = (k.N + 255) / 256, nth = (k.N + 127) / 128;
    const double rh = k.bias_mode == FAT5_BIAS_NONE ? 0.65 : 0.73;
    auto makespan = [&](int pf) {
      const long F = (long)pf * ntf, Hn = (long)(per - pf) * nth;
      const long cx = k.ncus / 8 > 0 ? k.ncus / 8 : 1;
      const long a = F / cx, rem = F % cx, n_lo = cx - rem, n_hi = rem;
      const double base = (double)(a + (rem ? 1 : 0));
      if (Hn == 0) return base;
      long jl = 0, jh = 0, count = 0;
      double t = 0;
      while (count < Hn) {
        const double tl = (double)a + jl * rh, th = (double)(a + 1) + jh * rh;
        if (n_hi == 0 || tl <= th) { t = tl; count += n_lo; ++jl; }
        else { t = th; count += n_hi; ++jh; }
      }
      return std::max(t + rh, base);
    };
    {
      const double pure = std::min(makespan(per), L.kv64_half || k.bias_mode == FAT5_BIAS_NONE ? makespan(0) : 1e30);
      double best = 1e30;
      int best_pf = -1;
      for (int pf = 1; pf < per; ++pf) {
        const double m = makespan(pf);
        if (m < best) { best = m; best_pf = pf; }
      }
      if (best_pf > 0 && (ov.kv64_mix == 1 || (best < 0.95 * pure && !k.causal))) {
        L.kv64_mix_pf = best_pf;
        mix_gain = best / makespan(per);
      }
    }
  }
  const size_t kv64_lds = L.kv64_mix_pf > 0 ? std::max(smem_bwd_kv64h_d64(k.rpe_radius, k.bias_mode), smem_bwd_kv64_d64(k.rpe_radius, k.bias_mode))
                                            : (L.kv64_half ? smem_bwd_kv64h_d64(k.rpe_radius, k.bias_mode) : smem_bwd_kv64_d64(k.rpe_radius, k.bias_mode));
  const bool fills = L.kv64_mix_pf > 0 ? mix_gain <= 0.9 : L.kv64_half;
  const bool ctab = causal_in_band(k);
  const bool kv64_causal_ok = !k.causal || k.N >= ((ctab || k.bias_mode == FAT5_BIAS_NONE) ? 1024 : 4096);
  const bool dense_rule = dense && ((wg256 >= cu_scaled(192, k.ncus) && (int64_t)bh * k.M * k.N >= (int64_t(1) << 25)) || qdb_pick);
  L.kv64 = k.D == 64 && (!dense || dense_kv_ok) && !k.packed && ov.kv64 != 0 &&
           (ov.kv64 == 1 || dense_rule || ((wg256 >= cu_scaled(k.causal ? 256 : (fills ? 320 : 512), k.ncus) ||
                              (wg256 >= cu_scaled(160, k.ncus) && k.M >= 4096 && !k.causal)) && kv64_causal_ok)) && kv64_lds <= 160 * 1024;
  if (L.kv64 && L.kv64_mix_pf > 0) {
    L.kv64_half = false;
    L.nw_kv = kKv64Mixed;
    L.n_nblk = (k.N + 127) / 128;
  } else if (L.kv64) {
    L.kv64_mix_pf = -1;
    L.nw_kv = L.kv64_half ? kKv64Half : kKv64Full;
    L.n_nblk = L.kv64_half ? (k.N + 127) / 128 : (k.N + 255) / 256;
  } else {
    L.kv64_half = false;
    L.kv64_mix_pf = -1;
  }
  L.q64 = k.D == 64 && k.bias_mode != FAT5_BIAS_DENSE && !k.packed && ov.q64 != 0 &&
          (ov.q64 == 1 || ((bh * ((k.M + 255) / 256) >= cu_scaled(512, k.ncus) || (bh * ((k.M + 255) / 256) >= cu_scaled(160, k.ncus) && k.N >= 8192)) &&
                            k.N >= ((k.bias_mode == FAT5_BIAS_RPE1D && bh * ((k.M + 255) / 256) < cu_scaled(1024, k.ncus)) ? 4096 : 2048) && (!k.causal || k.M >= 16384)));
  L.fused64 = false;
  if (k.D == 64 && k.bias_mode != FAT5_BIAS_DENSE && !k.packed && ov.fused64 != 0 &&
      smem_bwd_fused64_d64(k.rpe_radius, k.bias_mode) <= 160 * 1024) {
    const long wq = bh * ((k.M + 255) / 256), tot = wg256 + wq;
    const long FUSED64_MAX_WG = cu_scaled(1152, k.ncus);
    const bool squarish = 2 * (k.M < k.N ? k.M : k.N) >= (k.M < k.N ? k.N : k.M);
    const long max_wg = (k.causal && (ctab || k.bias_mode == FAT5_BIAS_NONE)) ? cu_scaled(896, k.ncus) : FUSED64_MAX_WG;
    const bool causal_ok = !k.causal || (ctab && squarish && (tot <= k.ncus || tot >= cu_scaled(512, k.ncus) || k.N >= 1024)) ||
                           (k.bias_mode == FAT5_BIAS_NONE && squarish && (tot <= k.ncus || (k.N <= 512 && tot >= cu_scaled(512, k.ncus)) || k.N >= 2048 ||
                                                                           (k.N <= 1024 && tot % k.ncus == 0 && tot <= 4L * k.ncus)));
    const long padM = ((k.M + 255) / 256) * 256, padN = ((k.N + 255) / 256) * 256;
    const bool padded = !k.causal && tot > k.ncus && ((k.M > 256 && padM * 5 >= (long)k.M * 6) || (k.N > 256 && padN * 5 >= (long)k.N * 6));
    const bool rule = causal_ok && !padded && (tot <= cu_scaled(384, k.ncus) || (tot <= max_wg && squarish)) && ov.kv64 != 0 && ov.q64 != 0 && ov.kv64_half != 1 && ov.kv64_mix != 1;
    L.fused64 = ov.fused64 == 1 || rule;
  }
  if (L.fused64) {
    set_kv64_full(L, k);
    L.q64 = true;
  }
  {
    const long wq = bh * ((k.M + 255) / 256);
    L.diag_q = L.fused64 && k.bias_mode == FAT5_BIAS_RPE1D && (k.has_drpe1d || k.has_drpe_table) && ov.qdiag != 0 &&
               smem_bwd_fused64_d64(k.rpe_radius, k.bias_mode) <= 160 * 1024 && (ov.qdiag == 1 || wg256 + wq <= k.ncus);
  }
  L.dfused64 = false;
  if (qdb_legal && dense_kv_ok && ov.fused64 != 0 && ov.qdb64 != 0 && ov.kv64 != 0 && ov.kv64_half != 1 && ov.kv64_mix != 1 &&
      !(ov.dbias_staged || ov.dbias_inkernel) && smem_bwd_kv64_d64(k.rpe_radius, k.bias_mode) <= 160 * 1024) {
    const long nq = (long)k.H * qdb_ngrp * ((k.M + 63) / 64), tot = wg256 + nq;
    const long r_one = (tot + ncu - 1) / ncu, r_two = (wg256 + ncu - 1) / ncu + (nq + ncu - 1) / ncu;
    const bool rule = k.B >= 2 && r_one < r_two && r_two <= 8;
    if (ov.fused64 == 1 || rule) {
      L.dfused64 = true;
      set_kv64_full(L, k);
    }
  }
  if (L.q64) L.nw_q = 8;
  size_t off = 0;
  L.delta_off = off;
  off = align_up(off + (k.packed ? (size_t)k.H * k.total_q : (size_t)bh * k.M) * sizeof(float), 256);
  L.stat2_off = off;
  if (L.kv64) off = align_up(off + (size_t)bh * ((k.M + 31) / 32) * 64 * sizeof(float), 256);
  L.ds_staged = false;
  L.dbias_inkernel = false;
  L.ds_off = off;
  L.scratch_off = off;
  L.qdb64 = false;
  L.qdb_groups = 0;
  if (qdb_legal) {
    if (ov.qdb64 != 0 && (ov.qdb64 == 1 || L.dfused64 || (qdb_rule && !(ov.dbias_staged || ov.dbias_inkernel)))) {
      L.qdb64 = true;
      L.qdb_groups = qdb_ngrp;
      L.q64 = false;
      L.fused64 = false;
      L.nw_q = 2;
      if (qdb_ngrp > 1) off = align_up(off + (size_t)qdb_ngrp * k.H * k.M * k.N * sizeof(float), 256);
    }
  }
  if (k.bias_mode == FAT5_BIAS_DENSE && k.has_dbias && !L.qdb64) {
    const bool reduced = (k.dbias_batch != k.B) || (k.dbias_heads != k.H);
    const int inker_env = ov.dbias_staged ? 0 : (ov.dbias_inkernel ? 2 : 1);
    const size_t staging = (size_t)bh * k.M * k.N * 2;
    const bool big = k.B <= 4 ? staging > (size_t(k.D == 128 ? 512 : 64) << 20) : staging > (size_t(2) << 30);
    if (reduced && inker_env && (big || inker_env > 1) && batch_shared_dbias(k)) {
      L.dbias_inkernel = true;
      if (k.B > 4) off = align_up(off + (size_t)k.H * k.M * k.N * sizeof(float), 256);
    } else if (reduced) {
      L.ds_staged = true;
      off = align_up(off + (size_t)bh * k.M * k.N * 2, 256);
    }
  }
  L.drpe_off = off;
  L.part_rows = L.diag_q ? (k.M + 255) / 256 : L.n_nblk;
  if (k.bias_mode == FAT5_BIAS_RPE1D && (k.has_drpe1d || k.has_drpe_table))
    off = align_up(off + (size_t)bh * L.part_rows * (2 * k.rpe_radius + 1) * sizeof(float), 256);
  L.total = off;
  L.n_mblk = (k.M + 32 * L.nw_q - 1) / (32 * L.nw_q);
  L.grid_q = bh * L.n_mblk;
  L.grid_kv = bh * L.n_nblk;
  L.form = bwd_fusable(L, ov, k) ? kFused32 : (L.fused64 ? kFused64 : (L.dfused64 ? kDenseFused64 : kSeparate));
  return FAT5_OK;
}

inline int bwd_layout(const DispatchKey& k, BwdLayout& L) {
  thread_local DispatchKey last_k;
  thread_local BwdLayout last_L;
  thread_local int last_rc = -1;
  if (last_rc == FAT5_OK && memcmp(&last_k, &k, sizeof(k)) == 0) {
    L = last_L;
    return FAT5_OK;
  }
  const int rc = bwd_layout_compute(k, L);
  memcpy(&last_k, &k, sizeof(k));
  last_L = L;
  last_rc = rc;
  return rc;
}

}
```

### flasht5_amd/csrc/attn_launch.h

```cpp
#pragma once
#include <hip/hip_runtime.h>
#include "attn_common.h"

namespace fat5 {
inline void fill_div_magic(AttnArgs& a, long grid) {
  a.mg_mblk = div_magic(a.n_mblk, grid);
  a.mg_nblk = div_magic(a.n_nblk, grid);
  a.mg_H = div_magic(a.H, grid);
}
enum FwdLaunch : int { kFwdSplit = -4 };
enum Fwd64Launch : int {
  kFwd64KSplit = 2,
  kFwd64Mixed = 3,
  kFwd64Rows256 = 4,
  kFwd64Spread = 5,
};
enum Kv64Launch : int {
  kKv64Half = 2,
  kKv64Mixed = 3,
  kKv64Full = 4,
};
#define FAT5_DECL_LAUNCH(D)                                                                           \
  hipError_t launch_fwd_d##D(const AttnArgs& a, int bf16, int bias, int nw, int grid, hipStream_t s); \
  hipError_t launch_bwd_q_d##D(const AttnArgs& a, int bf16, int bias, int nw, int grid, hipStream_t s); \
  hipError_t launch_bwd_kv_d##D(const AttnArgs& a, int bf16, int bias, int nw, int grid, hipStream_t s); \
  hipError_t launch_bwd_fused_d##D(const AttnArgs& a, int bf16, int bias, int nw, int grid, hipStream_t s); \
  hipError_t launch_bwd_dbias_d##D(const AttnArgs& a, int bf16, void* dbias, float* scratch, int grid, hipStream_t s); \
  size_t smem_fwd_d##D(int nw, int R, int bias);                                                      \
  size_t smem_bwd_q_d##D(int nw, int R, int bias);                                                    \
  size_t smem_bwd_kv_d##D(int nw, int R, int bias);
FAT5_DECL_LAUNCH(32)
FAT5_DECL_LAUNCH(64)
FAT5_DECL_LAUNCH(128)
#undef FAT5_DECL_LAUNCH
hipError_t launch_fwd64_d64(const AttnArgs& a, int bf16, int bias, int nw, int grid, hipStream_t s);
size_t smem_fwd64_d64(int R, int bias);
hipError_t launch_fwd64_d128(const AttnArgs& a, int bf16, int bias, int nw, int grid, hipStream_t s);
size_t smem_fwd64_d128(int R, int bias);
hipError_t launch_bwd_kv64_d64(const AttnArgs& a, int bf16, int bias, int nw, int grid, hipStream_t s);
size_t smem_bwd_kv64_d64(int R, int bias);
size_t smem_bwd_kv64h_d64(int R, int bias);
hipError_t launch_bwd_q64_d64(const AttnArgs& a, int bf16, int bias, int nw, int grid, hipStream_t s);
hipError_t launch_bwd_fused64_d64(const AttnArgs& a, int bf16, int bias, int nw, int grid, hipStream_t s);
size_t smem_bwd_fused64_d64(int R, int bias);
hipError_t launch_bwd_qdb64_d64(const AttnArgs& a, int bf16, void* dbias_out, int partial, int grid, hipStream_t s);
hipError_t launch_bwd_dfused64_d64(const AttnArgs& a, int bf16, void* dbias_out, int partial, int grid_qdb, hipStream_t s);
hipError_t launch_dbias_partial_reduce(const float* part, void* out, int bf16, int ngrp, int H, int M, int N, int causal, hipStream_t s);
}
```

### flasht5_amd/flash_attention_v2_bias.py

```python
import ctypes
import math
from typing import Optional, Tuple

import torch

from . import _lib
from . import positional_encoding as _pe

__all__ = ["flash_attention_v2_bias", "FlashAttentionAdditiveBias", "flash_attention_v2_rpe",
           "FlashAttentionRPE", "flash_attn_varlen_fwd"]


def _prep(t):
    return t if _lib.kernel_ready(t) else t.contiguous()


def _bias_strides(bias, B, H):
    sb = bias.stride(0) if bias.shape[0] == B and B != 1 else (0 if bias.shape[0] == 1 else bias.stride(0))
    sh = bias.stride(1) if bias.shape[1] == H and H != 1 else (0 if bias.shape[1] == 1 else bias.stride(1))
    if bias.shape[0] == 1:
        sb = 0
    if bias.shape[1] == 1:
        sh = 0
    return _lib.c_i64x3(sb, sh, bias.stride(2))
# ... 464 lines not shown


@torch.library.register_fake("fat5::flash_attn_varlen_fwd")
def _varlen_fwd_fake(q, k, v, cu_seqlens_q, cu_seqlens_k, max_seqlen_q, max_seqlen_k, causal, sm_scale, rpe1d, radius):
    Tq, H, D = q.shape
    return torch.empty((Tq, H, D), dtype=q.dtype, device=q.device), torch.empty((H, Tq), dtype=torch.float32, device=q.device)


@torch.library.custom_op("fat5::flash_attn_varlen_bwd", mutates_args=(), device_types="cuda")
def _varlen_bwd_op(do: torch.Tensor, q: torch.Tensor, k: torch.Tensor, v: torch.Tensor, o: torch.Tensor, lse: torch.Tensor,
                   cu_seqlens_q: torch.Tensor, cu_seqlens_k: torch.Tensor, max_seqlen_q: int, max_seqlen_k: int, causal: bool,
                   sm_scale: float, rpe1d: Optional[torch.Tensor], radius: int, need_drpe: bool
                   ) -> Tuple[torch.Tensor, torch.Tensor, torch.Tensor, torch.Tensor]:
    dq, dk, dv, d1 = _varlen_bwd_impl(do, q, k, v, o, lse, cu_seqlens_q, cu_seqlens_k, max_seqlen_q, max_seqlen_k, causal,
                                      sm_scale, rpe1d, radius, need_drpe)
    if d1 is None:
        d1 = torch.empty(0, dtype=torch.float32, device=q.device)
    return dq, dk, dv, d1


@torch.library.register_fake("fat5::flash_attn_varlen_bwd")
def _varlen_bwd_fake(do, q, k, v, o, lse, cu_seqlens_q, cu_seqlens_k, max_seqlen_q, max_seqlen_k, causal, sm_scale, rpe1d, radius,
                     need_drpe):
    d1 = torch.empty_like(rpe1d) if (need_drpe and rpe1d is not None) else torch.empty(0, dtype=torch.float32, device=q.device)
    return torch.empty_like(q), torch.empty_like(k), torch.empty_like(v), d1


def flash_attn_varlen_fwd(q, k, v, cu_seqlens_q, cu_seqlens_k, max_seqlen_q, max_seqlen_k, causal=False, sm_scale=None,
                          rpe1d=None, radius=0):
    if sm_scale is None:
        sm_scale = 1.0 / math.sqrt(q.shape[-1])
    cq, ck = _as_cu(cu_seqlens_q, q.device), _as_cu(cu_seqlens_k, q.device)
    if _tracing():
        return torch.ops.fat5.flash_attn_varlen_fwd(q, k, v, cq, ck, int(max_seqlen_q), int(max_seqlen_k), bool(causal), float(sm_scale),
                                                    rpe1d, int(radius))
    return _varlen_fwd_impl(q, k, v, cq, ck, int(max_seqlen_q), int(max_seqlen_k), bool(causal), float(sm_scale), rpe1d, int(radius))


def flash_attn_varlen_bwd(do, q, k, v, o, lse, cu_seqlens_q, cu_seqlens_k, max_seqlen_q, max_seqlen_k, causal=False,
                          sm_scale=None, rpe1d=None, radius=0, need_drpe=False):
    if sm_scale is None:
        sm_scale = 1.0 / math.sqrt(q.shape[-1])
    cq, ck = _as_cu(cu_seqlens_q, q.device), _as_cu(cu_seqlens_k, q.device)
    if _tracing():
        dq, dk, dv, d1 = torch.ops.fat5.flash_attn_varlen_bwd(do, q, k, v, o, lse, cq, ck, int(max_seqlen_q), int(max_seqlen_k), bool(causal),
                                                              float(sm_scale), rpe1d, int(radius), bool(need_drpe))
        d1 = d1 if (need_drpe and rpe1d is not None) else None
    else:
        dq, dk, dv, d1 = _varlen_bwd_impl(do, q, k, v, o, lse, cq, ck, int(max_seqlen_q), int(max_seqlen_k), bool(causal),
                                          float(sm_scale), rpe1d, int(radius), bool(need_drpe))
    return (dq, dk, dv, d1) if rpe1d is not None else (dq, dk, dv)


class FlashAttentionVarlen(torch.autograd.Function):

    @staticmethod
    def forward(ctx, q, k, v, cu_seqlens_q, cu_seqlens_k, max_seqlen_q, max_seqlen_k, causal, sm_scale, rpe1d, radius):
        r1 = rpe1d.detach().float().contiguous() if rpe1d is not None else None
        cq, ck = _as_cu(cu_seqlens_q, q.device), _as_cu(cu_seqlens_k, q.device)
        o, lse = flash_attn_varlen_fwd(q, k, v, cq, ck, max_seqlen_q, max_seqlen_k, causal, sm_scale, r1, radius)
        ctx.save_for_backward(q, k, v, o, lse, cq, ck, *([r1] if r1 is not None else []))
        ctx.meta = (int(max_seqlen_q), int(max_seqlen_k), bool(causal), sm_scale, int(radius),
                    rpe1d.dtype if rpe1d is not None else None)
        return o

    @staticmethod
    def backward(ctx, do):
        q, k, v, o, lse, cq, ck, *rest = ctx.saved_tensors
        mq, mk, causal, sm_scale, radius, rdtype = ctx.meta
        if rest:
            dq, dk, dv, d1 = flash_attn_varlen_bwd(do, q, k, v, o, lse, cq, ck, mq, mk, causal, sm_scale, rest[0], radius,
                                                   ctx.needs_input_grad[9])
            return dq, dk, dv, None, None, None, None, None, None, (d1.to(rdtype) if d1 is not None else None), None
        dq, dk, dv = flash_attn_varlen_bwd(do, q, k, v, o, lse, cq, ck, mq, mk, causal, sm_scale)
        return dq, dk, dv, None, None, None, None, None, None, None, None


def flash_attn_varlen_func(q, k, v, cu_seqlens_q, cu_seqlens_k, max_seqlen_q, max_seqlen_k, causal=False, sm_scale=None,
                           rpe1d=None, radius=0):
    return FlashAttentionVarlen.apply(q, k, v, cu_seqlens_q, cu_seqlens_k, max_seqlen_q, max_seqlen_k, causal, sm_scale,
                                      rpe1d, int(radius))


class AttentionPlan:

    def __init__(self, q, k, v, do, *, bias=None, rpe1d=None, radius=0, causal=False, sm_scale=None, need_dbias=True,
                 rpe_bucket=None, num_buckets=0, units=None, variant=None):
        _check_inputs(q, k, v)
        self.q, self.k, self.v, self.do = _prep(q), _prep(k), _prep(v), _prep(do)
        B, H, M, D = q.shape
        self.shape = (B, H, M, k.shape[2], D)
        sm_scale = (1.0 / math.sqrt(D)) if sm_scale is None else sm_scale
        dev = q.device
        self.o = torch.empty_like(self.q)
        self.lse = torch.empty((B, H, M), dtype=torch.float32, device=dev)
        self.dq, self.dk, self.dv = torch.empty_like(self.q), torch.empty_like(self.k), torch.empty_like(self.v)
        self.bias, self.rpe1d, self.dbias = bias, rpe1d, None
        p = _base_params(self.q, self.k, self.v, causal, sm_scale)
        p.o, p.lse, p.o_stride = self.o.data_ptr(), self.lse.data_ptr(), _lib.strides3(self.o)
        p.dout, p.dq, p.dk, p.dv = self.do.data_ptr(), self.dq.data_ptr(), self.dk.data_ptr(), self.dv.data_ptr()
        p.do_stride, p.dq_stride, p.dk_stride, p.dv_stride = (_lib.strides3(t) for t in (self.do, self.dq, self.dk, self.dv))
        if bias is not None:
            p.bias_mode, p.bias, p.bias_stride = _lib.BIAS_DENSE, bias.data_ptr(), _bias_strides(bias, B, H)
            if need_dbias:
                self.dbias = torch.empty_like(bias)
                p.dbias, p.dbias_batch, p.dbias_heads = self.dbias.data_ptr(), bias.shape[0], bias.shape[1]
        elif rpe1d is not None:
            p.bias_mode, p.rpe1d, p.rpe_radius = _lib.BIAS_RPE1D, rpe1d.data_ptr(), int(radius)
            if need_dbias and rpe_bucket is not None:
                self.rpe_bucket = rpe_bucket
                self.dbias = torch.empty((num_buckets, H), dtype=torch.float32, device=dev)
                p.rpe_bucket, p.drpe_table, p.rpe_num_buckets = rpe_bucket.data_ptr(), self.dbias.data_ptr(), num_buckets
                host = _pe.host_bucket_map(rpe_bucket)
                if host is None and not (rpe_bucket.is_cuda and torch.cuda.is_current_stream_capturing()):
                    host = rpe_bucket.detach().to("cpu", torch.int32).contiguous()
                self.rpe_bucket_host = host
                if host is not None:
                    p.rpe_bucket_host = host.data_ptr()
            elif need_dbias:
                self.dbias = torch.empty_like(rpe1d)
                p.drpe1d = self.dbias.data_ptr()
        self.empty = units is not None and int(units[1]) == 0
        if units is not None:
            if int(units[1]) < 0 or int(units[0]) < 0 or int(units[0]) + int(units[1]) > B * H:
                raise ValueError(f"unit range {tuple(units)} outside the {B * H} (batch, head) units")
            p.unit_begin, p.unit_count = int(units[0]), int(units[1])
        if self.empty and self.dbias is not None:
            self.dbias.zero_()
        if variant is not None:
            p.variant = int(variant)
        self.lib = _lib.load()
        nbytes = self.lib.fat5_attn_bwd_workspace_bytes(ctypes.byref(p))
        self.ws = torch.empty(max(nbytes, 256), dtype=torch.uint8, device=dev)
        p.workspace, p.workspace_bytes = self.ws.data_ptr(), self.ws.numel()
        self.p = p
        self.device = dev

    def set_variant(self, bits):
        self.p.variant = int(bits)
        nbytes = self.lib.fat5_attn_bwd_workspace_bytes(ctypes.byref(self.p))
        if nbytes > self.ws.numel():
            self.ws = torch.empty(nbytes, dtype=torch.uint8, device=self.device)
            self.p.workspace, self.p.workspace_bytes = self.ws.data_ptr(), self.ws.numel()

    def forward(self):
        if self.empty:
            return self.o
        _lib.check(self.lib.fat5_attn_fwd(ctypes.byref(self.p), _lib.stream_ptr(self.device)), "fat5_attn_fwd")
        return self.o

    def describe(self):
        buf = ctypes.create_string_buffer(256)
        _lib.check(self.lib.fat5_attn_describe(ctypes.byref(self.p), buf, 256), "fat5_attn_describe")
        return dict(kv.split("=") for kv in buf.value.decode().split())

    def bwd_launches(self):
        return int(self.lib.fat5_attn_bwd_launches(ctypes.byref(self.p)))

    def backward(self, stages=7):
        if self.empty:
            return self.dq, self.dk, self.dv, self.dbias
        _lib.check(self.lib.fat5_attn_bwd_stages(ctypes.byref(self.p), int(stages), _lib.stream_ptr(self.device)),
                   "fat5_attn_bwd")
        return self.dq, self.dk, self.dv, self.dbias
```

### include/fat5.h

```cpp
#ifndef FAT5_H
#define FAT5_H

#include <stddef.h>
#include <stdint.h>

#ifdef __cplusplus
extern "C" {
#endif

#define FAT5_VERSION 114

enum fat5_status {
  FAT5_OK = 0,
  FAT5_EINVAL = -1,
  FAT5_EHIP = -2,
  FAT5_EWORKSPACE = -3
};

enum fat5_dtype { FAT5_F16 = 1, FAT5_BF16 = 2, FAT5_F32 = 0 };

enum fat5_variant {
  FAT5_V_FWD64_ON = 1, FAT5_V_FWD64_OFF = 2,
  FAT5_V_KV64_ON = 4, FAT5_V_KV64_OFF = 8,
  FAT5_V_Q64_ON = 16, FAT5_V_Q64_OFF = 32,
  FAT5_V_DBIAS_STAGED = 64, FAT5_V_DBIAS_INKERNEL = 128,
  FAT5_V_NO_FUSE = 256,
  FAT5_V_NO_SPLIT = 512,
  FAT5_V_FWD64_KSPLIT_ON = 1024, FAT5_V_FWD64_KSPLIT_OFF = 2048,
  FAT5_V_KV64_HALF_ON = 4096, FAT5_V_KV64_HALF_OFF = 8192,
  FAT5_V_KV64_MIX_ON = 16384, FAT5_V_KV64_MIX_OFF = 32768,
  FAT5_V_FWD64_MIX_ON = 524288, FAT5_V_FWD64_MIX_OFF = 1048576,
  FAT5_V_DBIAS_NOSPLIT = 262144,
  FAT5_V_QDB64_ON = 2097152, FAT5_V_QDB64_OFF = 4194304,
  FAT5_V_QDIAG_ON = 8388608, FAT5_V_QDIAG_OFF = 16777216,
  FAT5_V_DTABLE_RUNS_ON = 33554432, FAT5_V_DTABLE_RUNS_OFF = 67108864,
  FAT5_V_FUSED64_ON = 65536, FAT5_V_FUSED64_OFF = 131072
};

enum fat5_bias_mode {
  FAT5_BIAS_NONE = 0,
  FAT5_BIAS_DENSE = 1,
  FAT5_BIAS_RPE1D = 2
};

typedef struct fat5_attn_params {
  int32_t B, H, M, N, D;
  int32_t dtype;
  int32_t causal;
  int32_t bias_mode;
  float sm_scale;
  int32_t rpe_radius;
  const void* q;
  const void* k;
  const void* v;
  void* o;
  float* lse;
  int64_t q_stride[3], k_stride[3], v_stride[3], o_stride[3];
  const void* bias;
  int64_t bias_stride[3];
  const float* rpe1d;
  const int32_t* cu_seqlens_q;
  const int32_t* cu_seqlens_k;
  int32_t total_q, total_k;
  const void* dout;
  void* dq;
  void* dk;
  void* dv;
  int64_t do_stride[3], dq_stride[3], dk_stride[3], dv_stride[3];
  void* dbias;
  int32_t dbias_batch, dbias_heads;
  float* drpe1d;
  const int32_t* rpe_bucket;
  float* drpe_table;
  int32_t rpe_num_buckets;
  int32_t unit_begin;
  int32_t unit_count;
  int32_t variant;
  void* workspace;
  size_t workspace_bytes;
  const int32_t* rpe_bucket_host;
} fat5_attn_params;

int fat5_version(void);
int fat5_chip_cus(void);
const char* fat5_last_error(void);
size_t fat5_sizeof_attn_params(void);

int fat5_attn_fwd(const fat5_attn_params* p, void* hip_stream);
size_t fat5_attn_bwd_workspace_bytes(const fat5_attn_params* p);
int fat5_attn_bwd(const fat5_attn_params* p, void* hip_stream);
int fat5_attn_bwd_launches(const fat5_attn_params* p);
int fat5_attn_describe(const fat5_attn_params* p, char* out, size_t n);
enum fat5_bwd_stage { FAT5_BWD_DQ = 1, FAT5_BWD_DKDV = 2, FAT5_BWD_REDUCE = 4, FAT5_BWD_ALL = 7 };
int fat5_attn_bwd_stages(const fat5_attn_params* p, int stages, void* hip_stream);

int fat5_rpe1d_from_table(const void* table, int table_dtype, const int32_t* rpe_bucket, float* rpe1d, int32_t H,
                          int32_t rpe_radius, int32_t num_buckets, void* hip_stream);

int fat5_rmsnorm_fwd(const void* x, const void* w, void* y, float* rstd, int64_t rows, int64_t n,
                     int64_t x_row_stride, int64_t y_row_stride, float eps, int x_dtype, int w_dtype,
                     void* hip_stream);
int fat5_add_rmsnorm_fwd(const void* x, const void* r, const void* w, void* h, void* y, float* rstd, int64_t rows, int64_t n,
                         int64_t x_row_stride, int64_t r_row_stride, int64_t h_row_stride, int64_t y_row_stride, float eps,
                         int x_dtype, int w_dtype, void* hip_stream);
int fat5_add_rmsnorm_bwd(const void* dy, const void* h, const void* w, const float* rstd, const void* dres, void* dx, void* dw,
                         int64_t rows, int64_t n, int64_t dy_row_stride, int64_t h_row_stride, int64_t dres_row_stride,
                         int64_t dx_row_stride, int x_dtype, int w_dtype, void* workspace, size_t workspace_bytes,
                         void* hip_stream);
size_t fat5_rmsnorm_bwd_workspace_bytes(int64_t rows, int64_t n);
int fat5_rmsnorm_bwd(const void* dy, const void* x, const void* w, const float* rstd, void* dx, void* dw,
                     int64_t rows, int64_t n, int64_t dy_row_stride, int64_t x_row_stride,
                     int64_t dx_row_stride, int x_dtype, int w_dtype, void* workspace,
                     size_t workspace_bytes, void* hip_stream);

typedef struct fat5_dropout_desc {
  uint64_t seed;
  const int64_t* step;
  uint64_t elem_offset;
  uint32_t site;
  float p;
} fat5_dropout_desc;
size_t fat5_sizeof_dropout_desc(void);
int fat5_dropout(const void* x, const void* r, void* y, int64_t rows, int64_t n, int64_t x_row_stride, int64_t r_row_stride,
                 int64_t y_row_stride, const fat5_dropout_desc* desc, int dtype, void* hip_stream);
int fat5_dropout_add_rmsnorm_fwd(const void* x, const void* delta, const void* w, void* h, void* y, float* rstd, int64_t rows,
                                 int64_t n, int64_t x_row_stride, int64_t delta_row_stride, int64_t h_row_stride,
                                 int64_t y_row_stride, float eps, const fat5_dropout_desc* desc, int x_dtype, int w_dtype,
                                 void* hip_stream);
int fat5_dropout_add_rmsnorm_bwd(const void* dy, const void* h, const void* w, const float* rstd, const void* dres, void* dx,
                                 void* ddelta, void* dw, int64_t rows, int64_t n, int64_t dy_row_stride, int64_t h_row_stride,
                                 int64_t dres_row_stride, int64_t dx_row_stride, int64_t ddelta_row_stride,
                                 const fat5_dropout_desc* desc, int x_dtype, int w_dtype, void* workspace, size_t workspace_bytes,
                                 void* hip_stream);

int fat5_fold_weights(const void* w0, const void* w1, const void* w2, int64_t n0, int64_t n1, int64_t n2, int64_t ld0, int64_t ld1,
                      int64_t ld2, const void* g, void* out, int64_t K, int dtype, void* hip_stream);
int fat5_rmsnorm_unit_bwd(const void* gy, const void* x, const float* rstd, void* dx, void* xhat, int64_t rows, int64_t n,
                          int64_t gy_row_stride, int64_t x_row_stride, int64_t dx_row_stride, int64_t xhat_row_stride,
                          const void* dres, int64_t dres_row_stride, int dtype, void* hip_stream);
int fat5_fold_weights_bwd(const void* dwg, const void* w0, const void* w1, const void* w2, int64_t n0, int64_t n1, int64_t n2, int64_t ld0,
                          int64_t ld1, int64_t ld2, const void* g, void* dw0, void* dw1, void* dw2, void* dg, int64_t K, int dtype,
                          void* scratch, size_t scratch_bytes, void* hip_stream);
size_t fat5_fold_weights_bwd_scratch_bytes(int64_t n_total, int64_t K);

enum fat5_act { FAT5_ACT_GELU_TANH = 0, FAT5_ACT_RELU = 1 };
int fat5_gated_act_fwd(const void* h0, const void* h1, void* out, int64_t rows, int64_t F, int64_t h0_row_stride, int64_t h1_row_stride,
                       int64_t out_row_stride, int act, int dtype, void* hip_stream);
int fat5_gated_act_bwd(const void* dout, const void* h0, const void* h1, void* dh0, void* dh1, int64_t rows, int64_t F,
                       int64_t dout_row_stride, int64_t h0_row_stride, int64_t h1_row_stride, int64_t dh0_row_stride,
                       int64_t dh1_row_stride, int act, int dtype, void* hip_stream);

typedef struct fat5_rope_params {
  int32_t B;
  int32_t S;
  int32_t S_k;
  int32_t H, D;
  int32_t rd;
  int32_t dtype;
  int32_t interleaved;
  int32_t conjugate;
  int32_t n_tensors;
  int32_t n_q;
  int32_t table_rows;
  const void* cos;
  const void* sin;
  const void* cos_k;
  const void* sin_k;
  const void* x[3];
  void* y[3];
  int64_t x_stride[3][3];
  int64_t y_stride[3][3];
  const int32_t* cu_seqlens;
  const int32_t* cu_seqlens_k;
} fat5_rope_params;
size_t fat5_sizeof_rope_params(void);
int fat5_rope_apply(const fat5_rope_params* p, void* hip_stream);

typedef struct fat5_fire_params {
  int64_t M, N;
  int32_t H, W;
  int32_t dtype;
  float eps;
  const float* w1;
  const float* b1;
  const float* w2;
  const float* b2;
  const float* c;
  const float* L_multiplier;
  const float* init_L;
  void* bias;
  const void* dbias;
  int64_t bias_stride[2];
  float* dw1;
  float* db1;
  float* dw2;
  float* db2;
  float* dc;
  float* dL_multiplier;
} fat5_fire_params;
size_t fat5_sizeof_fire_params(void);
int fat5_fire_fwd(const fat5_fire_params* p, void* hip_stream);
size_t fat5_fire_bwd_workspace_bytes(const fat5_fire_params* p);
int fat5_fire_bwd(const fat5_fire_params* p, void* workspace, size_t workspace_bytes, void* hip_stream);

enum fat5_kv_cache_dtype { FAT5_KV_NATIVE = 0, FAT5_KV_FP8_E4M3 = 1 };

typedef struct fat5_kv_quant_params {
  int32_t B, L, H, D;
  int32_t dtype;
  const void* x;
  void* out;
  float* scale;
  int64_t x_stride[3], out_stride[3], scale_stride[3];
} fat5_kv_quant_params;
size_t fat5_sizeof_kv_quant_params(void);
int fat5_kv_quantize(const fat5_kv_quant_params* p, void* hip_stream);

typedef struct fat5_decode_params {
  int32_t B, H, D;
  int32_t dtype;
  int32_t capacity;
  int32_t N;
  const int32_t* cache_seqlens;
  float sm_scale;
  int32_t bias_mode;
  int32_t rpe_radius;
  const float* rpe1d;
  const void* q;
  void* k_cache;
  void* v_cache;
  const void* k_new;
  const void* v_new;
  void* o;
  float* lse;
  int64_t q_stride[2], k_cache_stride[3], v_cache_stride[3], k_new_stride[2], v_new_stride[2], o_stride[2];
  int32_t num_splits;
  void* workspace;
  size_t workspace_bytes;
  const int32_t* cache_batch_idx;
  const int32_t* cache_row_batch;
  int32_t cache_B;
} fat5_decode_params;
size_t fat5_sizeof_decode_params(void);
size_t fat5_attn_decode_workspace_bytes(const fat5_decode_params* p);
int fat5_attn_decode(const fat5_decode_params* p, void* hip_stream);
// ... 394 lines not shown
```

Baseline: 298.5 TFLOP/s.

## Keep all K/V tiles resident in LDS for the dQ backward kernel

Adds a KVRES mode to the D=64 dQ backward body, and to the fused backward body. When the key length fits in 16 steps of 32 keys, every K/V tile is DMA'd into LDS up front, reusing the ring and staging space, instead of cycling through a 4-slot ring. The per-iteration DMA issue and ring sync are replaced by a single wait-and-barrier after step 3, with LDS base pointers rebased as the loop advances. The aim is to remove per-step synchronisation and refill overhead from the dQ loop. In exchange it needs more dynamic LDS, adds a longer upfront load before compute can overlap, and makes the address bookkeeping more complex.

```diff
diff --git a/flasht5_amd/_lib.py b/flasht5_amd/_lib.py
--- a/flasht5_amd/_lib.py
+++ b/flasht5_amd/_lib.py
@@ -258,7 +258,7 @@
 
 
 EXPORTS = (
-    "fat5_version", "fat5_chip_cus", "fat5_last_error", "fat5_sizeof_attn_params", "fat5_attn_fwd", "fat5_attn_bwd_workspace_bytes", "fat5_attn_bwd", "fat5_attn_bwd_launches",
+    "fat5_version", "fat5_chip_cus", "fat5_last_error", "fat5_sizeof_attn_params", "fat5_attn_fwd", "fat5_attn_bwd_workspace_bytes", "fat5_attn_bwd", "fat5_attn_bwd_launches", "fat5_attn_bwd_kvres",
     "fat5_attn_bwd_stages", "fat5_attn_describe", "fat5_rpe1d_from_table",
     "fat5_rmsnorm_fwd", "fat5_rmsnorm_bwd_workspace_bytes", "fat5_rmsnorm_bwd", "fat5_add_rmsnorm_fwd", "fat5_add_rmsnorm_bwd",
     "fat5_ce_fwd", "fat5_ce_bwd", "fat5_ce_fwd_bwd", "fat5_fold_weights", "fat5_fold_weights_bwd", "fat5_fold_weights_bwd_scratch_bytes", "fat5_rmsnorm_unit_bwd", "fat5_gated_act_fwd", "fat5_gated_act_bwd",
@@ -305,6 +305,8 @@
     lib.fat5_attn_bwd_stages.argtypes = [ctypes.POINTER(AttnParams), ctypes.c_int, ctypes.c_void_p]
     lib.fat5_attn_bwd_launches.restype = ctypes.c_int
     lib.fat5_attn_bwd_launches.argtypes = [ctypes.POINTER(AttnParams)]
+    lib.fat5_attn_bwd_kvres.restype = ctypes.c_int
+    lib.fat5_attn_bwd_kvres.argtypes = [ctypes.POINTER(AttnParams)]
     lib.fat5_attn_describe.restype = ctypes.c_int
     lib.fat5_attn_describe.argtypes = [ctypes.POINTER(AttnParams), ctypes.c_char_p, ctypes.c_size_t]
     lib.fat5_attn_bwd_workspace_bytes.restype = ctypes.c_size_t
@@ -499,6 +501,7 @@
 V_FUSED64_ON, V_FUSED64_OFF = 65536, 131072
 V_DBIAS_NOSPLIT = 262144
 V_QDB64_ON, V_QDB64_OFF = 2097152, 4194304
+V_KVRES_ON, V_KVRES_OFF = 134217728, 268435456
 V_QDIAG_ON, V_QDIAG_OFF = 8388608, 16777216
 V_DTABLE_RUNS_ON, V_DTABLE_RUNS_OFF = 33554432, 67108864
 _variant = 0
@@ -617,4 +620,6 @@
             p.drpe1d = 16
     buf = ctypes.create_string_buffer(256)
     check(load().fat5_attn_describe(ctypes.byref(p), buf, 256), "fat5_attn_describe")
-    return dict(kv.split("=") for kv in buf.value.decode().split())
+    d = dict(kv.split("=") for kv in buf.value.decode().split())
+    d["kvres"] = str(load().fat5_attn_bwd_kvres(ctypes.byref(p)))
+    return d
diff --git a/flasht5_amd/csrc/api_attn.hip b/flasht5_amd/csrc/api_attn.hip
--- a/flasht5_amd/csrc/api_attn.hip
+++ b/flasht5_amd/csrc/api_attn.hip
@@ -126,6 +126,13 @@
   BwdLayout L;
   bwd_layout(key_of(p), L);
   return L.form == kSeparate ? 2 : 1;
+}
+
+int fat5_attn_bwd_kvres(const fat5_attn_params* p) {
+  if (check_common(p)) return 0;
+  BwdLayout L;
+  bwd_layout(key_of(p), L);
+  return L.kvres ? 1 : 0;
 }
 
 int fat5_attn_describe(const fat5_attn_params* p, char* out, size_t n) {
@@ -235,6 +242,7 @@
   a.n_nblk = L.n_nblk;
   a.n_kv_blocks = 0;
   a.diag_q = L.diag_q ? 1 : 0;
+  a.kvres = L.kvres ? 1 : 0;
   a.part_stride = L.part_rows;
   const long grid_q = n_units(p) * a.n_mblk, grid_kv = n_units(p) * a.n_nblk;
   const BwdForm form = ((stages & FAT5_BWD_DQ) && (stages & FAT5_BWD_DKDV)) ? L.form : kSeparate;
diff --git a/flasht5_amd/csrc/attn_bwd64.h b/flasht5_amd/csrc/attn_bwd64.h
--- a/flasht5_amd/csrc/attn_bwd64.h
+++ b/flasht5_amd/csrc/attn_bwd64.h
@@ -936,13 +936,14 @@
   static constexpr int RING = NS * SLOT;
   static constexpr int STG_T = 64 * 2 * D;
   static constexpr int STG = NW * 3 * STG_T;
+  static constexpr int RES_STEPS = 16;
   static size_t smem(int R, int bias_mode, bool stage = false, bool qdg = false) {
     return RING + (stage ? STG : 0) + (bias_mode == FAT5_BIAS_RPE1D ? rpe_table_bytes(R) + 16 : 0) +
            (qdg && bias_mode == FAT5_BIAS_RPE1D ? ((size_t)(2 * R + 1) * 4 * 2 * NW + NT * 4 + 63) / 64 * 64 : 0);
   }
 };
 
-template <int D, bool BF16, int BIAS, bool QDG = false>
+template <int D, bool BF16, int BIAS, bool QDG = false, bool KVRES = false>
 FAT5_DEV void attn_bwd_q64_body(const AttnArgs& a, const int bid) {
   static_assert(D == 64 && BIAS != FAT5_BIAS_DENSE, "gap schedule written for D = 64, bias none / rpe1d");
   static_assert(!QDG || BIAS == FAT5_BIAS_RPE1D, "the diagonal sums belong to the T5 bias");
@@ -950,8 +951,9 @@
   using Cfg = BwdQ64Cfg<D>;
   constexpr int BM = Cfg::BM, NT = Cfg::NT, IMG = Cfg::IMG, SLOT = Cfg::SLOT;
   constexpr int KK = D / 16, DB = D / 32;
+  static_assert(!KVRES || Cfg::RES_STEPS * SLOT == Cfg::RING + Cfg::STG, "the resident slots are the ring and the staging images, nothing more");
   extern __shared__ __attribute__((aligned(16))) char smem[];
-  const bool stg = a.lds_stage != 0;
+  const bool stg = KVRES || a.lds_stage != 0;
   float* sT = reinterpret_cast<float*>(smem + Cfg::RING + (stg ? Cfg::STG : 0)) + kRpePad;
 
   const int tid = threadIdx.x, w = __builtin_amdgcn_readfirstlane(tid >> 6), l = tid & 63, lq = l & 31, hi = l >> 5;
@@ -1150,9 +1152,10 @@
     if (t + 3 < nt) dma_step(t + 3, slot3_off);
   };
 #pragma unroll
-  for (int i = 0; i < 3; ++i)
+  for (int i = 0; i < (KVRES ? 4 : 3); ++i)
     if (i < nt) dma_step(i, (uint32_t)(i * SLOT));
-  for (int i = tid; i < SLOT / 16; i += NT) reinterpret_cast<u32x4*>(smem + 3 * SLOT)[i] = u32x4{0u, 0u, 0u, 0u};
+  if (!KVRES || nt < 4)
+    for (int i = tid; i < SLOT / 16; i += NT) reinterpret_cast<u32x4*>(smem + 3 * SLOT)[i] = u32x4{0u, 0u, 0u, 0u};
   FAT5_STAMP(7);
   if constexpr (BIAS == FAT5_BIAS_RPE1D) rpe_table_fill_rest(sT - kRpePad, a.rpe1d + (int64_t)h * (2 * a.R + 1), a.R, tid, NT, tabr, ctab ? P : 0x7fffffff);
   FAT5_STAMP(8);
@@ -1172,6 +1175,15 @@
         off_[qb][kk] = lds_rd128(ad + (uint32_t)(2 * Cfg::STG_T));
       }
     derive_rows();
+    if constexpr (KVRES) {
+      if (nt > 4) {
+        asm volatile("s_waitcnt lgkmcnt(0)" ::: "memory");
+        __builtin_amdgcn_s_barrier();
+#pragma unroll
+        for (int i = 4; i < Cfg::RES_STEPS; ++i)
+          if (i < nt) dma_step(i, (uint32_t)(i * SLOT));
+      }
+    }
   }
   FAT5_STAMP(1);
 #pragma unroll
@@ -1187,6 +1199,26 @@
   for (int j2 = 0; j2 < 2; ++j2)
 #pragma unroll
     for (int db = 0; db < DB; ++db) trA[j2][db] = lds0 + (uint32_t)fa.tr[j2][db];
+  [[maybe_unused]] int rm_base = 0, tr_base = 0;
+  [[maybe_unused]] auto res_rebase = [&](const int t) {
+    const int tr_to = t >= 4 ? t - 4 : 0;
+    const uint32_t drm = (uint32_t)((t - rm_base) * SLOT), dtr = (uint32_t)((tr_to - tr_base) * SLOT);
+#pragma unroll
+    for (int kk = 0; kk < KK; ++kk) rmA[kk] += drm;
+#pragma unroll
+    for (int j2 = 0; j2 < 2; ++j2)
+#pragma unroll
+      for (int db = 0; db < DB; ++db) trA[j2][db] += dtr;
+    rm_base = t;
+    tr_base = tr_to;
+  };
+  [[maybe_unused]] auto res_visible = [&](const int t) {
+    if (t == 3 && nt > 4) {
+      wait_dma_all();
+      __syncthreads();
+      FAT5_STAMP(14);
+    }
+  };
 
   const float c2 = a.scale * kLog2e;
   float cst_neg = 0.f, cst_pos = 0.f;
@@ -1289,9 +1321,12 @@
     if constexpr (QDG) diag_step_end(gst, nb);
   };
   auto generic_iter = [&](const int t) {
-    const uint32_t o_prev = (uint32_t)(((t + 3) & 3) * SLOT), o_cur = (uint32_t)((t & 3) * SLOT), o_next = (uint32_t)(((t + 1) & 3) * SLOT);
+    const uint32_t o_prev = KVRES ? (uint32_t)(((t ? t - 1 : 3) - tr_base) * SLOT) : (uint32_t)(((t + 3) & 3) * SLOT);
+    const uint32_t o_cur = KVRES ? (uint32_t)((t - tr_base) * SLOT) : (uint32_t)((t & 3) * SLOT);
+    const uint32_t o_next = KVRES ? (uint32_t)((t + 1 - rm_base) * SLOT) : (uint32_t)(((t + 1) & 3) * SLOT);
     product_step(o_prev);
-    sync_step(t, o_prev);
+    if constexpr (KVRES) res_visible(t);
+    else sync_step(t, o_prev);
     f32x16 Sn[2], DPn[2];
     score_step(o_next, Sn, DPn);
     softmax_generic(t * 32);
@@ -1306,7 +1341,7 @@
 
   constexpr int NG = 24, G_DP = 16;
   auto fast_iter = [&]<int SL, bool BAND>(const int t, const float ad0, const float ad1) {
-    constexpr uint32_t o_prev = (uint32_t)(((SL + 3) & 3) * SLOT), o_cur = (uint32_t)(SL * SLOT), o_next = (uint32_t)(((SL + 1) & 3) * SLOT);
+    constexpr uint32_t o_prev = (uint32_t)(((SL + 3) & 3) * SLOT), o_cur = (uint32_t)(SL * SLOT), o_next = (uint32_t)((KVRES ? SL + 1 : ((SL + 1) & 3)) * SLOT);
     f32x16 Sn[2], DPn[2];
     u32x4 DSn[2][2], kf[KK], vf[KK];
     u32x2 th[2][2], tn[2][2];
@@ -1359,11 +1394,21 @@
         else DPn[qb] = mfma32<BF16>(vf[kk], dof[qb][kk], DPn[qb]);
       }
       __builtin_amdgcn_sched_barrier(0);
-      if constexpr (g == 4) {
+      if constexpr (KVRES) {
+        if constexpr (g == 4 && SL == 3) res_visible(t);
+        if constexpr (g == 4 && SL == 0) {
+          const uint32_t dtr = (uint32_t)((t - tr_base) * SLOT);
+#pragma unroll
+          for (int j2 = 0; j2 < 2; ++j2)
+#pragma unroll
+            for (int db = 0; db < DB; ++db) trA[j2][db] += dtr;
+          tr_base = t;
+        }
+      } else if constexpr (g == 4) {
         if constexpr (FAT5_DMA_SPREAD) sync_wait(t);
         else sync_step(t, o_prev);
       }
-      if constexpr (FAT5_DMA_SPREAD && (g == 5 || g == 6)) {
+      if constexpr (!KVRES && FAT5_DMA_SPREAD && (g == 5 || g == 6)) {
         if (t + 3 < nt) {
           const uint32_t tt = (uint32_t)__builtin_amdgcn_readfirstlane(t + 3);
           const uint32_t dst = (uint32_t)__builtin_amdgcn_readfirstlane((int)(wave_lds + o_prev));
@@ -1434,6 +1479,11 @@
     }
 #pragma unroll
     for (int db = 0; db < DB; ++db) TRK[db] = u32x4{tn[db][0][0], tn[db][0][1], tn[db][1][0], tn[db][1][1]};
+    if constexpr (KVRES && SL == 3) {
+#pragma unroll
+      for (int kk = 0; kk < KK; ++kk) rmA[kk] += (uint32_t)(4 * SLOT);
+      rm_base += 4;
+    }
     if constexpr (BAND && QDG) {
       asm volatile("s_nop 1" : "+v"(dst[1].u1), "+v"(dst[1].b1));
       diag_step_end(dst, t * 32);
@@ -1464,6 +1514,7 @@
     int t = 0;
     while (t < nt) {
       int side, side3;
+      if constexpr (KVRES) res_rebase(t);
       while (t + 4 <= nt && (t & 3) == 0 && classify(t, side) && classify(t + 3, side3) && side3 == side) {
         const float cst = BIAS == FAT5_BIAS_RPE1D ? (side > 0 ? cst_pos : cst_neg) : 0.f;
         const float ad0 = cst + nL2[0], ad1 = cst + nL2[1];
@@ -1496,10 +1547,16 @@
       }
     }
     FAT5_STAMP(3);
-    product_step((uint32_t)(((nt - 1) & 3) * SLOT));
-  }
-  asm volatile("s_nop 15\n\ts_nop 15" ::: "memory");
+    product_step(KVRES ? (uint32_t)((nt - 1 - tr_base) * SLOT) : (uint32_t)(((nt - 1) & 3) * SLOT));
+    asm volatile("s_nop 15\n\ts_nop 15" : "+a"(dq[0][0]), "+a"(dq[0][1]), "+a"(dq[1][0]), "+a"(dq[1][1]) : : "memory");
+  }
   FAT5_STAMP(4);
+  if constexpr (KVRES) {
+    if (nt > 4) {
+      asm volatile("s_waitcnt lgkmcnt(0)" ::: "memory");
+      __builtin_amdgcn_s_barrier();
+    }
+  }
 
   const float scale = a.scale;
   if (stg) {
@@ -1566,13 +1623,13 @@
   FAT5_STAMP(6);
 }
 
-template <int D, bool BF16, int BIAS, bool QDG = false>
+template <int D, bool BF16, int BIAS, bool QDG = false, bool KVRES = false>
 __global__ __launch_bounds__(256) __attribute__((amdgpu_waves_per_eu(1, 1)))
 void attn_bwd_q64_kernel(const AttnArgs a) {
-  attn_bwd_q64_body<D, BF16, BIAS, QDG>(a, blockIdx.x);
+  attn_bwd_q64_body<D, BF16, BIAS, QDG, KVRES>(a, blockIdx.x);
 }
 
-template <int D, bool BF16, int BIAS, bool QDG = false>
+template <int D, bool BF16, int BIAS, bool QDG = false, bool KVRES = false>
 __global__ __launch_bounds__(256) __attribute__((amdgpu_waves_per_eu(1, 1)))
 void attn_bwd_fused64_kernel(const AttnArgs a) {
   if ((int)blockIdx.x < a.n_kv_blocks) {
@@ -1580,7 +1637,7 @@
     decode_unit(a, blockIdx.x, a.n_nblk, b, h, nblk, (FAT5_CAUSAL_ORDER && a.causal) ? 2 : 0);
     attn_bwd_kv64_body<D, BF16, BIAS, false, true, false, QDG>(a, b, h, nblk, nblk, false);
   } else {
-    attn_bwd_q64_body<D, BF16, BIAS, QDG>(a, blockIdx.x - a.n_kv_blocks);
+    attn_bwd_q64_body<D, BF16, BIAS, QDG, KVRES>(a, blockIdx.x - a.n_kv_blocks);
   }
 }
 
diff --git a/flasht5_amd/csrc/attn_bwd64_inst.hip b/flasht5_amd/csrc/attn_bwd64_inst.hip
--- a/flasht5_amd/csrc/attn_bwd64_inst.hip
+++ b/flasht5_amd/csrc/attn_bwd64_inst.hip
@@ -28,19 +28,29 @@
   return hipGetLastError();
 }
 
+template <int D>
+static size_t kvres_smem(size_t smem) { return std::max(smem, (size_t)(BwdQ64Cfg<D>::RES_STEPS + 1) * BwdQ64Cfg<D>::SLOT); }
+template <int D>
+static bool kvres_ok(const AttnArgs& a, bool staged) { return a.kvres && staged && (a.N + 31) / 32 <= BwdQ64Cfg<D>::RES_STEPS; }
+
+template <int D, bool BF16, int BIAS, bool QDG, bool KVRES>
+static hipError_t launch_q64_form(const AttnArgs& as, size_t smem, int grid, hipStream_t s) {
+  auto kern = attn_bwd_q64_kernel<D, BF16, BIAS, QDG, KVRES>;
+  if (smem > 48 * 1024) {
+    hipError_t e = hipFuncSetAttribute(reinterpret_cast<const void*>(kern), hipFuncAttributeMaxDynamicSharedMemorySize, (int)smem);
+    if (e != hipSuccess) return e;
+  }
+  hipLaunchKernelGGL(kern, dim3(grid), dim3(256), smem, s, as);
+  return hipGetLastError();
+}
 template <int D, bool BF16, int BIAS, bool QDG = false>
 static hipError_t launch_q64(const AttnArgs& a, int grid, hipStream_t s) {
   AttnArgs as = a;
   fill_div_magic(as, grid);
   as.lds_stage = BwdQ64Cfg<D>::smem(a.R, BIAS, true, QDG) <= 160 * 1024;
   const size_t smem = BwdQ64Cfg<D>::smem(a.R, BIAS, as.lds_stage != 0, QDG);
-  auto kern = attn_bwd_q64_kernel<D, BF16, BIAS, QDG>;
-  if (smem > 48 * 1024) {
-    hipError_t e = hipFuncSetAttribute(reinterpret_cast<const void*>(kern), hipFuncAttributeMaxDynamicSharedMemorySize, (int)smem);
-    if (e != hipSuccess) return e;
-  }
-  hipLaunchKernelGGL(kern, dim3(grid), dim3(256), smem, s, as);
-  return hipGetLastError();
+  if (kvres_ok<D>(a, as.lds_stage != 0)) return launch_q64_form<D, BF16, BIAS, QDG, true>(as, kvres_smem<D>(smem), grid, s);
+  return launch_q64_form<D, BF16, BIAS, QDG, false>(as, smem, grid, s);
 }
 hipError_t CAT(launch_bwd_q64_d, FAT5_INST_D)(const AttnArgs& a, int bf16, int bias, int , int grid, hipStream_t s) {
   if (bias == FAT5_BIAS_RPE1D) {
@@ -91,6 +101,16 @@
   }
   return nw == kKv64Half ? launch_kv64_bias<true>(a, bf16, bias, grid, s) : launch_kv64_bias<false>(a, bf16, bias, grid, s);
 }
+template <int D, bool BF16, int BIAS, bool QDG, bool KVRES>
+static hipError_t launch_fused64_form(const AttnArgs& as, size_t smem, int grid, hipStream_t s) {
+  auto kern = attn_bwd_fused64_kernel<D, BF16, BIAS, QDG, KVRES>;
+  if (smem > 48 * 1024) {
+    hipError_t e = hipFuncSetAttribute(reinterpret_cast<const void*>(kern), hipFuncAttributeMaxDynamicSharedMemorySize, (int)smem);
+    if (e != hipSuccess) return e;
+  }
+  hipLaunchKernelGGL(kern, dim3(grid), dim3(256), smem, s, as);
+  return hipGetLastError();
+}
 template <int D, bool BF16, int BIAS, bool QDG = false>
 static hipError_t launch_fused64(const AttnArgs& a, int grid, hipStream_t s) {
   AttnArgs as = a;
@@ -98,13 +118,8 @@
   as.lds_stage = std::max(Bwd64Cfg<D, false, true>::smem(a.R, BIAS, true), BwdQ64Cfg<D>::smem(a.R, BIAS, true, QDG)) <= 160 * 1024;
   const bool st = as.lds_stage != 0;
   const size_t smem = std::max(Bwd64Cfg<D, false, true>::smem(a.R, BIAS, st), BwdQ64Cfg<D>::smem(a.R, BIAS, st, QDG));
-  auto kern = attn_bwd_fused64_kernel<D, BF16, BIAS, QDG>;
-  if (smem > 48 * 1024) {
-    hipError_t e = hipFuncSetAttribute(reinterpret_cast<const void*>(kern), hipFuncAttributeMaxDynamicSharedMemorySize, (int)smem);
-    if (e != hipSuccess) return e;
-  }
-  hipLaunchKernelGGL(kern, dim3(grid), dim3(256), smem, s, as);
-  return hipGetLastError();
+  if (kvres_ok<D>(a, st)) return launch_fused64_form<D, BF16, BIAS, QDG, true>(as, kvres_smem<D>(smem), grid, s);
+  return launch_fused64_form<D, BF16, BIAS, QDG, false>(as, smem, grid, s);
 }
 hipError_t CAT(launch_bwd_fused64_d, FAT5_INST_D)(const AttnArgs& a, int bf16, int bias, int , int grid, hipStream_t s) {
   if (bias == FAT5_BIAS_RPE1D) {
@@ -117,6 +132,11 @@
 size_t CAT(smem_bwd_fused64_d, FAT5_INST_D)(int R, int bias) {
   return std::max(Bwd64Cfg<FAT5_INST_D, false, true>::smem(R, bias), BwdQ64Cfg<FAT5_INST_D>::smem(R, bias, false, true));
 }
+bool CAT(stage_bwd_q64_d, FAT5_INST_D)(int R, int bias, bool qdg, bool one_launch) {
+  const size_t q = BwdQ64Cfg<FAT5_INST_D>::smem(R, bias, true, qdg);
+  return (one_launch ? std::max(Bwd64Cfg<FAT5_INST_D, false, true>::smem(R, bias, true), q) : q) <= 160 * 1024;
+}
+int CAT(res_steps_bwd_q64_d, FAT5_INST_D)() { return BwdQ64Cfg<FAT5_INST_D>::RES_STEPS; }
 size_t CAT(smem_bwd_kv64_d, FAT5_INST_D)(int R, int bias) {
   return bias == FAT5_BIAS_DENSE ? Bwd64Cfg<FAT5_INST_D, false, false, true>::smem(R, bias) : Bwd64Cfg<FAT5_INST_D>::smem(R, bias);
 }
diff --git a/flasht5_amd/csrc/attn_common.h b/flasht5_amd/csrc/attn_common.h
--- a/flasht5_amd/csrc/attn_common.h
+++ b/flasht5_amd/csrc/attn_common.h
@@ -327,6 +327,7 @@
   int32_t dvalid;
   int32_t ref_first;
   int32_t lds_stage;
+  int32_t kvres;
   float scale;
 };
 
diff --git a/flasht5_amd/csrc/attn_dispatch.h b/flasht5_amd/csrc/attn_dispatch.h
--- a/flasht5_amd/csrc/attn_dispatch.h
+++ b/flasht5_amd/csrc/attn_dispatch.h
@@ -41,7 +41,7 @@
 
 struct Overrides {
   int fwd64, fwd64_ksplit, fwd64_mix;
-  int kv64, kv64_half, kv64_mix, q64, fused64, qdb64, qdiag;
+  int kv64, kv64_half, kv64_mix, q64, fused64, qdb64, qdiag, kvres;
   bool dbias_staged, dbias_inkernel;
   bool no_split, no_fuse;
   explicit Overrides(int v)
@@ -49,7 +49,7 @@
         fwd64_mix(vsel(v, FAT5_V_FWD64_MIX_ON, FAT5_V_FWD64_MIX_OFF)), kv64(vsel(v, FAT5_V_KV64_ON, FAT5_V_KV64_OFF)),
         kv64_half(vsel(v, FAT5_V_KV64_HALF_ON, FAT5_V_KV64_HALF_OFF)), kv64_mix(vsel(v, FAT5_V_KV64_MIX_ON, FAT5_V_KV64_MIX_OFF)),
         q64(vsel(v, FAT5_V_Q64_ON, FAT5_V_Q64_OFF)), fused64(vsel(v, FAT5_V_FUSED64_ON, FAT5_V_FUSED64_OFF)),
-        qdb64(vsel(v, FAT5_V_QDB64_ON, FAT5_V_QDB64_OFF)), qdiag(vsel(v, FAT5_V_QDIAG_ON, FAT5_V_QDIAG_OFF)),
+        qdb64(vsel(v, FAT5_V_QDB64_ON, FAT5_V_QDB64_OFF)), qdiag(vsel(v, FAT5_V_QDIAG_ON, FAT5_V_QDIAG_OFF)), kvres(vsel(v, FAT5_V_KVRES_ON, FAT5_V_KVRES_OFF)),
         dbias_staged(v & FAT5_V_DBIAS_STAGED), dbias_inkernel(v & FAT5_V_DBIAS_INKERNEL), no_split(v & FAT5_V_NO_SPLIT),
         no_fuse(v & FAT5_V_NO_FUSE) {}
 };
@@ -99,6 +99,7 @@
   int nw_q, nw_kv;
   bool diag_q;
   int part_rows;
+  bool kvres;
   long grid_q, grid_kv;
   BwdForm form;
 };
@@ -354,6 +355,8 @@
   L.grid_q = bh * L.n_mblk;
   L.grid_kv = bh * L.n_nblk;
   L.form = bwd_fusable(L, ov, k) ? kFused32 : (L.fused64 ? kFused64 : (L.dfused64 ? kDenseFused64 : kSeparate));
+  L.kvres = L.q64 && k.D == 64 && k.bias_mode != FAT5_BIAS_DENSE && ov.kvres != 0 && (k.N + 31) / 32 <= res_steps_bwd_q64_d64() &&
+            stage_bwd_q64_d64(k.rpe_radius, k.bias_mode, L.diag_q, L.form == kFused64);
   return FAT5_OK;
 }
 
diff --git a/flasht5_amd/csrc/attn_launch.h b/flasht5_amd/csrc/attn_launch.h
--- a/flasht5_amd/csrc/attn_launch.h
+++ b/flasht5_amd/csrc/attn_launch.h
@@ -41,6 +41,8 @@
 size_t smem_bwd_kv64_d64(int R, int bias);
 size_t smem_bwd_kv64h_d64(int R, int bias);
 hipError_t launch_bwd_q64_d64(const AttnArgs& a, int bf16, int bias, int nw, int grid, hipStream_t s);
+bool stage_bwd_q64_d64(int R, int bias, bool qdg, bool one_launch);
+int res_steps_bwd_q64_d64();
 hipError_t launch_bwd_fused64_d64(const AttnArgs& a, int bf16, int bias, int nw, int grid, hipStream_t s);
 size_t smem_bwd_fused64_d64(int R, int bias);
 hipError_t launch_bwd_qdb64_d64(const AttnArgs& a, int bf16, void* dbias_out, int partial, int grid, hipStream_t s);
diff --git a/flasht5_amd/flash_attention_v2_bias.py b/flasht5_amd/flash_attention_v2_bias.py
--- a/flasht5_amd/flash_attention_v2_bias.py
+++ b/flasht5_amd/flash_attention_v2_bias.py
@@ -640,7 +640,9 @@
     def describe(self):
         buf = ctypes.create_string_buffer(256)
         _lib.check(self.lib.fat5_attn_describe(ctypes.byref(self.p), buf, 256), "fat5_attn_describe")
-        return dict(kv.split("=") for kv in buf.value.decode().split())
+        d = dict(kv.split("=") for kv in buf.value.decode().split())
+        d["kvres"] = str(int(self.lib.fat5_attn_bwd_kvres(ctypes.byref(self.p))))
+        return d
 
     def bwd_launches(self):
         return int(self.lib.fat5_attn_bwd_launches(ctypes.byref(self.p)))
diff --git a/include/fat5.h b/include/fat5.h
--- a/include/fat5.h
+++ b/include/fat5.h
@@ -34,6 +34,7 @@
   FAT5_V_QDB64_ON = 2097152, FAT5_V_QDB64_OFF = 4194304,
   FAT5_V_QDIAG_ON = 8388608, FAT5_V_QDIAG_OFF = 16777216,
   FAT5_V_DTABLE_RUNS_ON = 33554432, FAT5_V_DTABLE_RUNS_OFF = 67108864,
+  FAT5_V_KVRES_ON = 134217728, FAT5_V_KVRES_OFF = 268435456,
   FAT5_V_FUSED64_ON = 65536, FAT5_V_FUSED64_OFF = 131072
 };
 
@@ -91,6 +92,7 @@
 int fat5_attn_bwd(const fat5_attn_params* p, void* hip_stream);
 int fat5_attn_bwd_launches(const fat5_attn_params* p);
 int fat5_attn_describe(const fat5_attn_params* p, char* out, size_t n);
+int fat5_attn_bwd_kvres(const fat5_attn_params* p);
 enum fat5_bwd_stage { FAT5_BWD_DQ = 1, FAT5_BWD_DKDV = 2, FAT5_BWD_REDUCE = 4, FAT5_BWD_ALL = 7 };
 int fat5_attn_bwd_stages(const fat5_attn_params* p, int stages, void* hip_stream);
 
```

After: 307.8 TFLOP/s, median of 6. 1.03x the previous value.
